# xinjuezou-whi/Open_Duck_Playground

Measured on AMD Instinct MI355X. Metric: env steps/sec (all envs) open_duck_mini_v2 flat, 4096 envs, 1/2/4/8 GPUs, higher is better.
Workload: dtype f32; 1 GPU; C2: flat_terrain, no imitation, 4096 envs per GPU, episode_length 1000 + auto-reset; envs_per_gpu=4096, total_envs=4096, substeps=10, parallelism=env-shard x1, step_kernel=throughput

## Files before the change

open_duck_playground_amd/csrc/duck_env_kernels.h:

```cpp
#pragma once
#include "duck_common.h"
#include "duck_physics.h"
#include "duck_team.h"

enum { SLOT_ACTION_DELAY = 0, SLOT_PUSH_THETA = 1, SLOT_PUSH_MAG = 2, SLOT_GYRO = 3, SLOT_ACCEL = 6,
       SLOT_GRAVITY = 9, SLOT_IMU_IDX = 12, SLOT_QPOS = 13, SLOT_QVEL = 29, SLOT_CMD = 45 };
enum { RSLOT_DXY = 0, RSLOT_YAW = 2, RSLOT_QSCALE = 3, RSLOT_QVEL = 19, RSLOT_CMD = 25, RSLOT_PUSH = 33,
       RSLOT_OBS = 64 };
#define KEY_TAG_ENV 0x5EEDu
#define KEY_TAG_DR 0xD0D0u
#define PI_F 3.14159265358979323846f

struct KArgs {
  int n;
  float* fs;
  int32_t* is;
  const float* dr;
  const float* action;
  float* obs;
  float* priv;
  float* reward;
  float* done;
  float* scratch;
  const uint8_t* mask;
  uint64_t seed;
  int64_t env_offset;
  const float* frames;
  const float* hfield;
  RefMeta ref;
  duck_env_config cfg;
  duck_layout lay;
  duck_dr_layout drl;
  unsigned* err;
};


DK int local_env(int& lane) {
  lane = threadIdx.x % TEAM;
  return threadIdx.x / TEAM;
}

template <class Md, int LAT = 0>
DK lds_float* env_slice(float* lds, int t) {
  return (lds_float*)(lds + t * TLay<Md, LAT>::STRIDE);
}

template <class Md>
DK void phys_step(lds_float* L, int lane, bool integrate, bool want_out, float* aux, int aux_stride, float* scratch,
                  int sstride, const float* hfield) {
  TPhys<Md>::step(L, lane, integrate, want_out, aux, aux_stride, scratch, sstride, hfield);
}

template <class Md>
__device__ __noinline__ void phys_step_dni(lds_float* L, int lane, bool integrate, bool want_out, float* aux,
                                           int aux_stride, float* scratch, int sstride, const float* hfield) {
  phys_step<Md>(L, lane, integrate, want_out, aux, aux_stride, scratch, sstride, hfield);
}

struct Col {
  float* p;
  int n;
  DK float& operator[](int k) const { return p[(size_t)k * n]; }
};
struct LCol {
  lds_float* p;
  DK lds_float& operator[](int k) const { return p[k]; }
};

DK int nearest(const float* g, int n, float v) {
  int best = 0;
  float bd = fabsf(g[0] - v);
  for (int i = 1; i < 16; i++) {
    if (i >= n) break;
    const float d = fabsf(g[i] - v);
    if (d < bd) { bd = d; best = i; }
  }
  return best;
}
DK void reference_motion(const KArgs& A, float dx, float dy, float dth, int i, float* out) {
  const RefMeta& R = A.ref;
  dx = fminf(fmaxf(dx, R.dx_range[0]), R.dx_range[1]);
  dy = fminf(fmaxf(dy, R.dy_range[0]), R.dy_range[1]);
  dth = fminf(fmaxf(dth, R.dtheta_range[0]), R.dtheta_range[1]);
  const int ix = nearest(R.dxs, R.n_dx, dx), iy = nearest(R.dys, R.n_dy, dy), it = nearest(R.dthetas, R.n_dtheta, dth);
  const int nb = R.nb;
  const int ph = ((i % nb) + nb) % nb;
  const float4* f = reinterpret_cast<const float4*>(
      A.frames + ((size_t)((ix * R.n_dy + iy) * R.n_dtheta + it) * nb + ph) * 40);
#pragma unroll
  for (int d = 0; d < 10; d++) {
    const float4 v = f[d];
    out[4 * d] = v.x; out[4 * d + 1] = v.y; out[4 * d + 2] = v.z; out[4 * d + 3] = v.w;
  }
}

DK float nan_to_num(float x) {
  if (isnan(x)) return 0.0f;
  if (isinf(x)) return x > 0 ? 3.4028234663852886e38f : -3.4028234663852886e38f;
  return x;
}

template <class RT>
DK void sample_command(const duck_env_config& c, const RT& r, int slot, float* cmd) {
  const float f = c.head_range_factor;
  cmd[0] = r.uniform(slot + 0, c.lin_vel_x[0], c.lin_vel_x[1]);
  cmd[1] = r.uniform(slot + 1, c.lin_vel_y[0], c.lin_vel_y[1]);
  cmd[2] = r.uniform(slot + 2, c.ang_vel_yaw[0], c.ang_vel_yaw[1]);
  cmd[3] = r.uniform(slot + 3, c.neck_pitch_range[0] * f, c.neck_pitch_range[1] * f);
  cmd[4] = r.uniform(slot + 4, c.head_pitch_range[0] * f, c.head_pitch_range[1] * f);
  cmd[5] = r.uniform(slot + 5, c.head_yaw_range[0] * f, c.head_yaw_range[1] * f);
  cmd[6] = r.uniform(slot + 6, c.head_roll_range[0] * f, c.head_roll_range[1] * f);
  if (r.u(slot + 7) < 0.1f)
    for (int k = 0; k < 7; k++) cmd[k] = 0.0f;
}

template <class Md>
DK void load_dyn(const KArgs& A, int e, lds_float* L) {
  using Ly = Lay<Md>;
  Phys<Md>::set_nominal(L);
  if (A.dr) {
    const duck_dr_layout& D = A.drl;
    const int n = A.n;
#pragma unroll
    for (int k = 0; k < 3; k++) L[Ly::DIPOS + k] = A.dr[(size_t)(D.base_ipos + k) * n + e];
#pragma unroll
    for (int b = 0; b < Md::NB; b++) L[Ly::DMASS + b] = A.dr[(size_t)(D.body_mass + b) * n + e];
#pragma unroll
    for (int a = 0; a < Md::NU; a++) {
      L[Ly::DFRIC + Md::actuator_dof[a]] = A.dr[(size_t)(D.frictionloss + a) * n + e];
      L[Ly::DARM + Md::actuator_dof[a]] = A.dr[(size_t)(D.armature + a) * n + e];
      L[Ly::DQ0 + Md::actuator_qadr[a]] = A.dr[(size_t)(D.qpos0 + a) * n + e];
      L[Ly::DKP + a] = A.dr[(size_t)(D.kp + a) * n + e];
    }
  }
}

template <class Md, int LAT = 0>
DK void load_dyn_team(const KArgs& A, int e, lds_float* L, int lane) {
  using Ly = Lay<Md>;
  using TP = TPhys<Md, LAT>;
  constexpr int NDYN = Md::NB + 3 + 2 * Md::NV + Md::NQ + Md::NU;
  static_assert(Ly::DKP + Md::NU - Ly::DMASS == NDYN, "contiguous per-env model block");
  for (int k = lane; k < NDYN; k += TEAM) L[Ly::DMASS + k] = TP::tf(Md::B_NOM + k);
  if (A.dr) {
    TSYNC();
    const duck_dr_layout& D = A.drl;
    const int n = A.n;
    if (lane < 3) L[Ly::DIPOS + lane] = A.dr[(size_t)(D.base_ipos + lane) * n + e];
    for (int b = lane; b < Md::NB; b += TEAM) L[Ly::DMASS + b] = A.dr[(size_t)(D.body_mass + b) * n + e];
    if (lane < Md::NU) {
      const int a = lane, o = Md::B_ACT + 12 * a, dof = TP::ti(o + 5), qadr = TP::ti(o + 4);
      L[Ly::DFRIC + dof] = A.dr[(size_t)(D.frictionloss + a) * n + e];
      L[Ly::DARM + dof] = A.dr[(size_t)(D.armature + a) * n + e];
      L[Ly::DQ0 + qadr] = A.dr[(size_t)(D.qpos0 + a) * n + e];
      L[Ly::DKP + a] = A.dr[(size_t)(D.kp + a) * n + e];
    }
  }
}

struct SObs {
  lds_float* row;
  DK void operator()(int k, float v) const { row[k] = v; }
};

template <class Md, class FA, class OS, class RT>
DK void write_obs_team(const KArgs& A, int lane, lds_float* L, const FA& F, const OS& out, const RT& r,
                       int slot_base, int imitation_i) {
  using Ly = Lay<Md>;
  const duck_env_config& c = A.cfg;
  const duck_layout& Lo = A.lay;
  constexpr int NU = Md::NU;
  static_assert(NU <= TEAM, "an actuator per lane");
  static_assert(priv_row_max(NU) <= Ly::HSZ + 4 * Ly::NROW, "privileged row must fit in the H/row storage (SObs)");
  const bool joystick = Lo.task == DUCK_TASK_JOYSTICK;
  const float nl = c.noise_level;
  const int OQ = 13, OV = OQ + NU, O1 = OV + NU, O2 = O1 + NU, O3 = O2 + NU, OM = O3 + NU;
  const int OC = joystick ? OM + NU : OM;
  const int P = OC + 2 + (joystick ? 2 : 0);
  const int PQ = P + 15, PV = PQ + NU, PZ = PV + NU, PA = PZ + 1, PC = PA + NU, PF = PC + 2, PT = PF + 6, PR = PT + 2;
  const int PI = PR + (Lo.imitation ? 40 : 0);
  if (lane < 3) {
    const int k = lane;
    const float gyro = L[Ly::SENS + c.sens_gyro + k], acc = L[Ly::SENS + c.sens_accelerometer + k];
    const float grav = -L[Ly::IMUR + k];
    const float ngrav = grav + (2.0f * r.u(slot_base + SLOT_GRAVITY + k) - 1.0f) * nl * c.noise_gravity;
    const float h0 = F[Lo.imu_history + k], h1 = F[Lo.imu_history + 3 + k];
    F[Lo.imu_history + 6 + k] = h1;
    F[Lo.imu_history + 3 + k] = h0;
    F[Lo.imu_history + k] = ngrav;
    out(k, gyro + (2.0f * r.u(slot_base + SLOT_GYRO + k) - 1.0f) * nl * c.noise_gyro);
    out(3 + k, acc + (2.0f * r.u(slot_base + SLOT_ACCEL + k) - 1.0f) * nl * c.noise_accelerometer);
    out(P + k, gyro);
    out(P + 3 + k, acc);
    out(P + 6 + k, grav);
    out(P + 9 + k, L[Ly::SENS + c.sens_local_linvel + k]);
    out(P + 12 + k, L[Ly::SENS + c.sens_global_angvel + k]);
    out(PF + k, L[Ly::SENS + c.sens_left_foot_linvel + k]);
    out(PF + 3 + k, L[Ly::SENS + c.sens_right_foot_linvel + k]);
  }
  if (lane < 7) out(6 + lane, F[Lo.command + lane]);
  if (lane < NU) {
    const int a = lane;
    float ja = L[Ly::QPOS + c.actuator_qposadr[a]];
    if (c.backlash_qposadr[a] >= 0) ja += L[Ly::QPOS + c.backlash_qposadr[a]];
    const float jv = L[Ly::QVEL + c.actuator_qveladr[a]];
    out(OQ + a, ja + (2.0f * r.u(slot_base + SLOT_QPOS + a) - 1.0f) * nl * c.qpos_noise_scale[a] - c.default_actuator[a]);
    out(OV + a, (jv + (2.0f * r.u(slot_base + SLOT_QVEL + a) - 1.0f) * nl * c.noise_joint_vel) * c.dof_vel_scale);
    out(O1 + a, F[Lo.last_act + a]);
    out(O2 + a, F[Lo.last_last_act + a]);
    out(O3 + a, F[Lo.last_last_last_act + a]);
    if (joystick) out(OM + a, F[Lo.motor_targets + a]);
    out(PQ + a, ja - c.default_actuator[a]);
    out(PV + a, jv);
    out(PA + a, L[Ly::AF + a]);
  }
  if (lane < 2) {
    const float con = L[Ly::OCON + lane];
    out(OC + lane, con);
    out(PC + lane, con);
    out(PT + lane, F[Lo.feet_air_time + lane]);
    if (joystick) {
      const float ph = F[Lo.imitation_phase + lane];
      out(OC + 2 + lane, ph);
      out(PI + 1 + lane, ph);
    }
  }
  if (lane == 0) {
    out(PZ, L[Ly::QPOS + 2]);
    if (joystick) out(PI, (float)imitation_i);
  }
  if (Lo.imitation)
    for (int k = lane; k < 40; k += TEAM) out(PR + k, F[Lo.ref_motion + k]);
}

template <class Md>
__global__ void __launch_bounds__(TPB) reset_kernel(KArgs A) {
  using Ly = Lay<Md>;
  {
    extern __shared__ float lds_t[];
    load_model_tables<Md>(lds_t);
  }
  int lane;
  const int t = local_env(lane);
  const int e = blockIdx.x * TEAM_WG + t;
  if (e >= A.n) return;
  if (A.mask && !A.mask[e]) return;
  extern __shared__ float lds[];
  lds_float* const L = env_slice<Md>(lds, t);
  const duck_env_config& c = A.cfg;
  const duck_layout& Lo = A.lay;
  constexpr int NQ = Md::NQ, NV = Md::NV, NU = Md::NU;
  const Col F{A.fs + e, A.n};
  auto iset = [&](int k, int32_t v) { A.is[(size_t)k * A.n + e] = v; };
  for (int k = 0; k < Lo.nfloat; k++) F[k] = 0.0f;
  for (int k = 0; k < Lo.nint; k++) iset(k, 0);
  Rng r;
  derive_key(A.seed, A.env_offset + e, KEY_TAG_ENV, r.k0, r.k1);
  r.ctr = 0;
  load_dyn<Md>(A, e, L);
  for (int i = 0; i < NQ; i++) L[Ly::QPOS + i] = c.init_qpos[i];
  for (int i = 0; i < NV; i++) { L[Ly::QVEL + i] = 0.0f; L[Ly::WARM + i] = 0.0f; }
  L[Ly::QPOS + 0] += r.uniform(RSLOT_DXY + 0, -0.05f, 0.05f);
  L[Ly::QPOS + 1] += r.uniform(RSLOT_DXY + 1, -0.05f, 0.05f);
  {
    const float yaw = r.uniform(RSLOT_YAW, -3.14f, 3.14f);
    float s, co;
    sincosf(0.5f * yaw, &s, &co);
    const float qy[4] = {co, 0.0f, 0.0f, s};
    float q[4] = {L[Ly::QPOS + 3], L[Ly::QPOS + 4], L[Ly::QPOS + 5], L[Ly::QPOS + 6]};
    qmul(q, q, qy);
    for (int k = 0; k < 4; k++) L[Ly::QPOS + 3 + k] = q[k];
  }
  for (int a = 0; a < NU; a++) L[Ly::QPOS + c.actuator_qposadr[a]] *= r.uniform(RSLOT_QSCALE + a, 0.5f, 1.5f);
  const float vr = Lo.task == DUCK_TASK_STANDING ? 0.5f : 0.05f;
  for (int k = 0; k < 6; k++) L[Ly::QVEL + k] = r.uniform(RSLOT_QVEL + k, -vr, vr);
  for (int a = 0; a < NU; a++) L[Ly::CTRL + a] = L[Ly::QPOS + c.actuator_qposadr[a]];
  phys_step<Md>(L, lane, false, true, nullptr, 0, A.scratch ? A.scratch + e : nullptr, A.n, A.hfield);
  float cmd[7];
  sample_command(c, r, RSLOT_CMD, cmd);
  const float push_interval = r.uniform(RSLOT_PUSH, c.push_interval_range[0], c.push_interval_range[1]);
  iset(Lo.push_interval, (int32_t)rintf(push_interval / c.ctrl_dt));
  iset(Lo.rng_key, (int32_t)r.k0);
  iset(Lo.rng_key + 1, (int32_t)r.k1);
  iset(Lo.rng_ctr, 1);
  for (int k = 0; k < 7; k++) F[Lo.command + k] = cmd[k];
  for (int a = 0; a < NU; a++) F[Lo.motor_targets + a] = Lo.task == DUCK_TASK_STANDING ? 0.0f : c.default_actuator[a];
  if (Lo.imitation) {
    float ref[40];
    reference_motion(A, cmd[0], cmd[1], cmd[2], 0, ref);
    for (int k = 0; k < 40; k++) F[Lo.ref_motion + k] = ref[k];
  }
  write_obs_team<Md>(A, lane, L, F, SObs{L + Ly::H}, r, RSLOT_OBS, 0);
  TSYNC();
  float* priv = A.priv + (size_t)e * Lo.priv_size;
  float* obs = A.obs + (size_t)e * Lo.obs_size;
  for (int k = lane; k < Lo.priv_size; k += TEAM) {
    const float v = L[Ly::H + k];
    priv[k] = v;
    F[Lo.first_priv + k] = v;
    if (k < Lo.obs_size) {
      obs[k] = v;
      F[Lo.first_obs + k] = v;
    }
  }
  for (int i = 0; i < NQ; i++) { F[Lo.qpos + i] = L[Ly::QPOS + i]; F[Lo.first_qpos + i] = L[Ly::QPOS + i]; }
  for (int i = 0; i < NV; i++) {
    F[Lo.qvel + i] = L[Ly::QVEL + i]; F[Lo.first_qvel + i] = L[Ly::QVEL + i];
    F[Lo.qacc_warmstart + i] = L[Ly::WARM + i]; F[Lo.first_qacc_warmstart + i] = L[Ly::WARM + i];
  }
  for (int a = 0; a < NU; a++) { F[Lo.ctrl + a] = L[Ly::CTRL + a]; F[Lo.first_ctrl + a] = L[Ly::CTRL + a]; }
}

struct StepPre {
  int32_t step, push_step, push_interval, ep_steps, imitation_i;
  uint32_t k0, k1, ctr;
  float act;
};
template <class Md>
DK StepPre step_prefetch(const KArgs& A, int e, int lane) {
  static_assert(Md::NU <= TEAM, "an actuator per lane");
  const duck_layout& Lo = A.lay;
  const int n = A.n, ec = e < n ? e : 0;
  auto ig = [&](int k) { return A.is[(size_t)k * n + ec]; };
  StepPre P;
  P.step = ig(Lo.step);
  P.push_step = ig(Lo.push_step);
  P.push_interval = ig(Lo.push_interval);
  P.ep_steps = ig(Lo.ep_steps);
  P.imitation_i = ig(Lo.imitation_i);
  P.k0 = (uint32_t)ig(Lo.rng_key);
  P.k1 = (uint32_t)ig(Lo.rng_key + 1);
  P.ctr = (uint32_t)ig(Lo.rng_ctr);
  P.act = A.action[(size_t)ec * Md::NU + (lane < Md::NU ? lane : 0)];
  return P;
}

template <class Md, class FA, class RT, int LAT = 0>
DK void step_env(const KArgs& A, int e, int lane, lds_float* L, const FA& F, const Col& G, const RT& r,
                 const StepPre& P) {
  using Ly = Lay<Md>;
  const duck_env_config& c = A.cfg;
  const duck_layout& Lo = A.lay;
  constexpr int NQ = Md::NQ, NV = Md::NV, NU = Md::NU;
  const int n = A.n;
  STAGE_T0();
  auto iset = [&](int k, int32_t v) { A.is[(size_t)k * n + e] = v; };
  const float dt = c.ctrl_dt;
  const int step_prev = P.step, push_step = P.push_step, push_interval = P.push_interval;
  int ep_steps = P.ep_steps;
  if (c.auto_reset && F[Lo.done] != 0.0f) ep_steps = 0;
  int imitation_i = P.imitation_i;
  if (Lo.imitation) {
    const int nb = A.ref.nb;
    imitation_i = (imitation_i + 1) % nb;
    const float ph = ((float)imitation_i / (float)nb) * 2.0f * PI_F;
    F[Lo.imitation_phase] = cosf(ph);
    F[Lo.imitation_phase + 1] = sinf(ph);
    float ref[40];
    reference_motion(A, F[Lo.command], F[Lo.command + 1], F[Lo.command + 2], imitation_i, ref);
    for (int k = 0; k < 40; k++) F[Lo.ref_motion + k] = ref[k];
  } else {
    imitation_i = 0;
  }
  const int didx = r.randint(SLOT_ACTION_DELAY, c.action_min_delay, c.action_max_delay);
  float arate = 0.0f;
  for (int a = lane; a < NU; a += TEAM) {
    const float act = P.act;
    const float h1 = F[Lo.action_history + a], h2 = F[Lo.action_history + NU + a];
    F[Lo.action_history + a] = act;
    F[Lo.action_history + NU + a] = h1;
    F[Lo.action_history + 2 * NU + a] = h2;
    const float ad = didx == 0 ? act : (didx == 1 ? h1 : h2);
    float mt = c.default_actuator[a] + ad * c.action_scale;
    if (c.use_motor_speed_limits) {
      const float prev = F[Lo.motor_targets + a], lim = c.max_motor_velocity * dt;
      mt = fminf(fmaxf(mt, prev - lim), prev + lim);
    }
    L[Ly::CTRL + a] = mt;
    const float la = F[Lo.last_act + a];
    arate += (act - la) * (act - la);
  }
  const float theta = r.uniform(SLOT_PUSH_THETA, 0.0f, 2.0f * PI_F);
  const float mag = r.uniform(SLOT_PUSH_MAG, c.push_magnitude_range[0], c.push_magnitude_range[1]);
  const float gate = (push_interval != 0 && (push_step + 1) % push_interval == 0) ? 1.0f : 0.0f;
  const float push[2] = {cosf(theta) * gate * (float)c.push_enable, sinf(theta) * gate * (float)c.push_enable};
  arate = tsum(arate);
  team_for<NQ>(lane, [&](int i) { L[Ly::QPOS + i] = F[Lo.qpos + i]; });
  team_for<NV>(lane, [&](int i) {
    L[Ly::QVEL + i] = F[Lo.qvel + i] + (i == 0 ? push[0] * mag : (i == 1 ? push[1] * mag : 0.0f));
    L[Ly::WARM + i] = F[Lo.qacc_warmstart + i];
  });
  load_dyn_team<Md, LAT>(A, e, L, lane);
  TSYNC();
  float* scr = A.scratch ? A.scratch + e : nullptr;
  STAGE_MARK(29);
  if constexpr (LAT) {
    using TPL = TPhys<Md, LAT>;
    (void)scr;
    LAT_T(43, 5);
    for (int s = 0; s < c.n_substeps; s++) {
// ... 59 lines not shown
  const float r_still = nan_to_num(pc + vc) * (cn < 0.01f ? 1.0f : 0.0f);
  float imit = 0.0f;
  if (Lo.imitation) {
    const int R0 = Lo.ref_motion;
    float lxy = 0.0f, axy = 0.0f;
    for (int k = 0; k < 2; k++) {
      const float dv = L[Ly::QVEL + k] - F[R0 + 34 + k], dw = L[Ly::QVEL + 3 + k] - F[R0 + 37 + k];
      lxy += dv * dv;
      axy += dw * dw;
    }
    const float dz = L[Ly::QVEL + 2] - F[R0 + 36], dwz = L[Ly::QVEL + 5] - F[R0 + 39];
    const float lin_xy = expf(-8.0f * lxy), lin_z = expf(-8.0f * dz * dz);
    const float ang_xy = expf(-2.0f * axy) * 0.5f, ang_z = expf(-2.0f * dwz * dwz) * 0.5f;
    float jp = 0.0f, jv = 0.0f;
    for (int k = lane; k < 5; k += TEAM) {
      const float q1 = L[Ly::QPOS + c.actuator_qposadr[k]] - F[R0 + k];
      const float q2 = L[Ly::QPOS + c.actuator_qposadr[NU - 5 + k]] - F[R0 + 11 + k];
      const float v1 = L[Ly::QVEL + c.actuator_qveladr[k]] - F[R0 + 16 + k];
      const float v2 = L[Ly::QVEL + c.actuator_qveladr[NU - 5 + k]] - F[R0 + 27 + k];
      jp += q1 * q1 + q2 * q2;
      jv += v1 * v1 + v2 * v2;
    }
    jp = tsum(jp);
    jv = tsum(jv);
    float contact_r = 0.0f;
    for (int k = 0; k < 2; k++) contact_r += (con[k] == (F[R0 + 32 + k] > 0.5f ? 1.0f : 0.0f)) ? 1.0f : 0.0f;
    float rr = lin_xy + lin_z + ang_xy + ang_z + (-jp * 15.0f) + (-jv * 1e-3f) + contact_r;
    rr *= cn > 0.01f ? 1.0f : 0.0f;
    imit = nan_to_num(rr);
  }
  float terms[7];
  if (standing) {
    lpc = tsum(lpc);
    lvc = tsum(lvc);
    hp = tsum(hp);
    const float ux = L[Ly::SENS + c.sens_upvector], uy = L[Ly::SENS + c.sens_upvector + 1];
    terms[0] = nan_to_num(ux * ux + uy * uy) * c.scale_orientation;
    terms[1] = nan_to_num(torq) * c.scale_torques;
    terms[2] = nan_to_num(arate) * c.scale_action_rate;
    terms[3] = 1.0f * c.scale_alive;
    terms[4] = nan_to_num(lpc + lvc) * (cn < 0.01f ? 1.0f : 0.0f) * c.scale_stand_still;
    terms[5] = nan_to_num(hp) * (cn > 0.01f ? 1.0f : 0.0f) * c.scale_head_pos;
    terms[6] = 0.0f;
  } else {
    terms[0] = r_lin * c.scale_tracking_lin_vel;
    terms[1] = r_ang * c.scale_tracking_ang_vel;
    terms[2] = nan_to_num(torq) * c.scale_torques;
    terms[3] = nan_to_num(arate) * c.scale_action_rate;
    terms[4] = 1.0f * c.scale_alive;
    terms[5] = imit * c.scale_imitation;
    terms[6] = r_still * c.scale_stand_still;
  }
  float sum = 0.0f;
  for (int k = 0; k < 7; k++) sum += terms[k];
  const float reward = fminf(fmaxf(sum * dt, 0.0f), 10000.0f);
  F[Lo.push] = push[0];
  F[Lo.push + 1] = push[1];
  int step = step_prev + 1;
  iset(Lo.push_step, push_step + 1);
  team_for<NU>(lane, [&](int a) {
    F[Lo.last_last_last_act + a] = F[Lo.last_last_act + a];
    F[Lo.last_last_act + a] = F[Lo.last_act + a];
    F[Lo.last_act + a] = F[Lo.action_history + a];
  });
  if (step > 500) {
    float nc[7];
    sample_command(c, r, SLOT_CMD, nc);
    for (int k = 0; k < 7; k++) F[Lo.command + k] = nc[k];
  }
  if (done != 0.0f || step > 500) step = 0;
  iset(Lo.step, step);
  iset(Lo.imitation_i, imitation_i);
  for (int k = 0; k < 2; k++) {
    F[Lo.feet_air_time + k] = F[Lo.feet_air_time + k] * (con[k] != 0.0f ? 0.0f : 1.0f);
    F[Lo.last_contact + k] = con[k];
    F[Lo.swing_peak + k] = F[Lo.swing_peak + k] * (con[k] != 0.0f ? 0.0f : 1.0f);
  }
  const float scales[7] = {standing ? c.scale_orientation : c.scale_tracking_lin_vel,
                           standing ? c.scale_torques : c.scale_tracking_ang_vel,
                           standing ? c.scale_action_rate : c.scale_torques,
                           standing ? c.scale_alive : c.scale_action_rate,
                           standing ? c.scale_stand_still : c.scale_alive,
                           standing ? c.scale_head_pos : c.scale_imitation,
                           standing ? 0.0f : c.scale_stand_still};
  for (int k = 0; k < 7; k++) F[Lo.metrics + k] = scales[k] > 0.0f ? terms[k] : -terms[k];
  F[Lo.metrics + DUCK_M_SWING_PEAK] = 0.5f * (F[Lo.swing_peak] + F[Lo.swing_peak + 1]);
  iset(Lo.rng_ctr, (int32_t)(r.ctr + 1));
  float trunc = 0.0f;
  bool restore = false;
  if (c.auto_reset) {
    ep_steps += 1;
    if (ep_steps >= c.episode_length) { trunc = 1.0f - done; done = 1.0f; }
    restore = done != 0.0f;
    iset(Lo.ep_steps, ep_steps);
  }
  if (restore) {
    for (int i = lane; i < NQ; i += TEAM) F[Lo.qpos + i] = G[Lo.first_qpos + i];
    for (int i = lane; i < NV; i += TEAM) { F[Lo.qvel + i] = G[Lo.first_qvel + i]; F[Lo.qacc_warmstart + i] = G[Lo.first_qacc_warmstart + i]; }
    for (int a = lane; a < NU; a += TEAM) F[Lo.ctrl + a] = G[Lo.first_ctrl + a];
    TSYNC();
    for (int k = lane; k < Lo.priv_size; k += TEAM) L[Ly::H + k] = G[Lo.first_priv + k];
  } else {
    team_for<NQ>(lane, [&](int i) { F[Lo.qpos + i] = L[Ly::QPOS + i]; });
    team_for<NV>(lane, [&](int i) { F[Lo.qvel + i] = L[Ly::QVEL + i]; F[Lo.qacc_warmstart + i] = L[Ly::WARM + i]; });
  }
  F[Lo.reward] = reward;
  F[Lo.done] = done;
  F[Lo.truncation] = trunc;
  A.reward[e] = reward;
  A.done[e] = done;
  STAGE_MARK(31);
  TSYNC();
  float* priv = A.priv + (size_t)e * Lo.priv_size;
  float* obs = A.obs + (size_t)e * Lo.obs_size;
  constexpr int PMAX = priv_row_max(NU);
  constexpr int NKP = (PMAX + TEAM - 1) / TEAM, NKO = (DUCK_OBS_SIZE(NU) + TEAM - 1) / TEAM;
  float pv[NKP];
#pragma unroll
  for (int kk = 0; kk < NKP; kk++) {
    const int k = lane + TEAM * kk;
    pv[kk] = L[Ly::H + (k < PMAX ? k : PMAX - 1)];
  }
#pragma unroll
  for (int kk = 0; kk < NKP; kk++) {
    const int k = lane + TEAM * kk;
    if (k < Lo.priv_size) priv[k] = pv[kk];
  }
#pragma unroll
  for (int kk = 0; kk < NKO; kk++) {
    const int k = lane + TEAM * kk;
    if (k < Lo.obs_size) obs[k] = pv[kk];
  }
  STAGE_MARK(34);
}

DK RngTab step_rng(const StepPre& P, lds_float* tab, int lane) {
  RngTab rt;
  rt.k0 = P.k0;
  rt.k1 = P.k1;
  rt.ctr = P.ctr;
  rt.tab = tab;
  rt.fill(tab, lane);
  return rt;
}

template <class Md>
__global__ void __launch_bounds__(TPB) step_kernel(KArgs A) {
  STAGE_T0();
#ifdef DUCK_ANY_PROF
  const unsigned long long kstart = clock64(), kwall = wall_clock64();
#endif
  using TL = TLay<Md>;
  {
    extern __shared__ float lds_t[];
    load_model_tables<Md>(lds_t);
  }
  STAGE_MARK(14);
  int lane;
  const int t = local_env(lane);
  const int e = blockIdx.x * TEAM_WG + t;
  const int n = A.n;
  extern __shared__ float lds[];
  if constexpr (TL::ES_LDS) {
    const int j = threadIdx.x % TEAM_WG, ej = blockIdx.x * TEAM_WG + j;
    lds_float* esj = (lds_float*)(lds + TL::ES + j * TL::ESTRIDE);
    const StepPre P = step_prefetch<Md>(A, e, lane);
    {
      constexpr int NK = (TL::HOT + TPB / TEAM_WG - 1) / (TPB / TEAM_WG);
      const int ejc = ej < n ? ej : 0;
      float hv[NK];
#pragma unroll
      for (int kk = 0; kk < NK; kk++) {
        const int k = (int)threadIdx.x / TEAM_WG + (TPB / TEAM_WG) * kk;
        hv[kk] = A.fs[(size_t)(k < TL::HOT ? k : TL::HOT - 1) * n + ejc];
      }
#pragma unroll
      for (int kk = 0; kk < NK; kk++) {
        const int k = (int)threadIdx.x / TEAM_WG + (TPB / TEAM_WG) * kk;
        if (ej < n && k < TL::HOT) esj[k] = hv[kk];
      }
    }
    __syncthreads();
    STAGE_MARK(32);
    if (e < n) {
      lds_float* const L = env_slice<Md>(lds, t);
      const Col G{A.fs + e, n};
      lds_float* esp = (lds_float*)(lds + TL::ES + t * TL::ESTRIDE);
      const RngTab rt = step_rng(P, esp + TL::HOT, lane);
      TSYNC();
      STAGE_MARK(33);
      step_env<Md>(A, e, lane, L, LCol{esp}, G, rt, P);
      STAGE_RESET();
    }
    __syncthreads();
    {
      constexpr int NK = (TL::HOT + TPB / TEAM_WG - 1) / (TPB / TEAM_WG);
      float hv[NK];
#pragma unroll
      for (int kk = 0; kk < NK; kk++) {
        const int k = (int)threadIdx.x / TEAM_WG + (TPB / TEAM_WG) * kk;
        hv[kk] = esj[k < TL::HOT ? k : TL::HOT - 1];
      }
#pragma unroll
      for (int kk = 0; kk < NK; kk++) {
        const int k = (int)threadIdx.x / TEAM_WG + (TPB / TEAM_WG) * kk;
        if (ej < n && k < TL::HOT) A.fs[(size_t)k * n + ej] = hv[kk];
      }
    }
  } else {
    if (e >= n) return;
    lds_float* const L = env_slice<Md>(lds, t);
    const Col G{A.fs + e, n};
    const duck_layout& Lo = A.lay;
    Rng r;
    r.k0 = (uint32_t)A.is[(size_t)Lo.rng_key * n + e];
    r.k1 = (uint32_t)A.is[(size_t)(Lo.rng_key + 1) * n + e];
    r.ctr = (uint32_t)A.is[(size_t)Lo.rng_ctr * n + e];
    step_env<Md>(A, e, lane, L, G, G, r, step_prefetch<Md>(A, e, lane));
    STAGE_RESET();
  }
  STAGE_MARK(15);
#ifdef DUCK_ANY_PROF
  if ((threadIdx.x & 63) == 0 && blockIdx.x < 256) {
    const int w = 4 * blockIdx.x + threadIdx.x / 64;
    g_stage_cycles[DUCK_NSTAGE + w] = clock64() - kstart;
    g_stage_cycles[DUCK_NSTAGE + 1024 + w] = kwall;
    g_stage_cycles[DUCK_NSTAGE + 2048 + w] = wall_clock64();
  }
#endif
}

template <class Md, int LAT>
__device__ __forceinline__ void step_lat_body(KArgs A) {
  using TL = TLay<Md, LAT>;
  using TPL = TPhys<Md, LAT>;
  constexpr int WGL = TL::NWG;
  static_assert(TL::TAB_LDS && TL::ES_LDS, "latency mode: the model blob and the hot state in LDS");
  static_assert(TPB == 4 * 64 && WGL * TEAM == 64 * (LAT == 2 ? 2 : 1),
                "latency modes: 4 waves, one set of 4 teams per wave (paired: per pair of waves)");
  extern __shared__ float lds[];
  LAT_T(40, 5);
  TPL::ev_init((int)threadIdx.x);
  load_model_tables<Md, LAT>(lds);
  LAT_T(41, 5);
  const int wave = __builtin_amdgcn_readfirstlane((int)threadIdx.x >> 6);
  const int t = (LAT == 2 ? 4 * (wave >> 1) : 0) + ((int)threadIdx.x & 63) / TEAM, lane = (int)threadIdx.x % TEAM;
  const int e = blockIdx.x * WGL + t;
  const int n = A.n;
  const int j = threadIdx.x % WGL, ej = blockIdx.x * WGL + j;
  lds_float* esj = (lds_float*)(lds + TL::ES + j * TL::ESTRIDE);
  const StepPre P = step_prefetch<Md>(A, e, lane);
  constexpr int NK = (TL::HOT + TPB / WGL - 1) / (TPB / WGL);
  {
    const int ejc = ej < n ? ej : 0;
    float hv[NK];
#pragma unroll
    for (int kk = 0; kk < NK; kk++) {
      const int k = (int)threadIdx.x / WGL + (TPB / WGL) * kk;
      hv[kk] = A.fs[(size_t)(k < TL::HOT ? k : TL::HOT - 1) * n + ejc];
    }
#pragma unroll
    for (int kk = 0; kk < NK; kk++) {
      const int k = (int)threadIdx.x / WGL + (TPB / WGL) * kk;
      if (ej < n && k < TL::HOT) esj[k] = hv[kk];
    }
  }
  __syncthreads();
  LAT_T(42, 5);
  if (e < n) {
    lds_float* const L = env_slice<Md, LAT>(lds, t);
    const int ns = A.cfg.n_substeps;
    float* scr = A.scratch ? A.scratch + e : nullptr;
    auto env_code = [&]() {
      const Col G{A.fs + e, n};
      lds_float* esp = (lds_float*)(lds + TL::ES + t * TL::ESTRIDE);
      const RngTab rt = step_rng(P, esp + TL::HOT, lane);
      TSYNC();
      step_env<Md, LCol, RngTab, LAT>(A, e, lane, L, LCol{esp}, G, rt, P);
      LAT_T(45, 5);
    };
    if constexpr (LAT == 2) {
      if ((wave & 1) == 0) {
        env_code();
      } else {
        for (int s = 0; s < ns; s++) TPL::lat2_b(L, lane, s, true, s == ns - 1, scr, n);
      }
    } else {
      if (wave == 0) {
        env_code();
      } else if (wave == 1) {
        for (int s = 0; s < ns; s++) TPL::lat_r1(L, lane, s, true, s == ns - 1, scr, n);
      } else if (wave == 2) {
        for (int s = 0; s < ns; s++) TPL::lat_r2(L, lane, s, A.hfield);
      } else {
        for (int s = 0; s < ns; s++) TPL::lat_r3(L, lane, s);
      }
    }
  }
  __syncthreads();
  LAT_T(46, 5);
  const bool timed_out = TPL::ev_timed_out(LAT == 2 ? j / LAT_WG : 0);
  if (threadIdx.x == 0 && A.err && (TPL::ev_timed_out(0) || (LAT == 2 && TPL::ev_timed_out(1))))
    __hip_atomic_fetch_or(A.err, (unsigned)DUCK_DEVERR_LAT_TIMEOUT, __ATOMIC_RELAXED, __HIP_MEMORY_SCOPE_SYSTEM);
  {
    float hv[NK];
#pragma unroll
    for (int kk = 0; kk < NK; kk++) {
      const int k = (int)threadIdx.x / WGL + (TPB / WGL) * kk;
      hv[kk] = esj[k < TL::HOT ? k : TL::HOT - 1];
      if (timed_out && k >= A.lay.qpos && k < A.lay.qpos + Md::NQ) hv[kk] = __builtin_nanf("");
    }
#pragma unroll
    for (int kk = 0; kk < NK; kk++) {
      const int k = (int)threadIdx.x / WGL + (TPB / WGL) * kk;
      if (ej < n && k < TL::HOT) A.fs[(size_t)k * n + ej] = hv[kk];
    }
  }
}

template <class Md, int LAT>
__global__ void __launch_bounds__(TPB) step_kernel_lat(KArgs A) {
  step_lat_body<Md, LAT>(A);
}

constexpr int LAT_X2 = 5;
template <class Md>
struct LatX2 {
  static_assert(TLay<Md, LAT_X2>::LDS_FLOATS == TLay<Md, 1>::LDS_FLOATS && TLay<Md, LAT_X2>::NWG == LAT_WG,
                "LAT_X2 is the LAT = 1 layout");
  static constexpr bool PAYS = TLay<Md, 1>::FITS && 2 * (size_t)TLay<Md, 1>::LDS_FLOATS * 4 <= 160 * 1024 &&
                               Md::FLOOR_TYPE == 0 && Md::NV <= 20;
};
template <class Md>
__global__ void __launch_bounds__(TPB) __attribute__((amdgpu_waves_per_eu(2, 2))) step_kernel_lat_x2(KArgs A) {
  if constexpr (LatX2<Md>::PAYS) step_lat_body<Md, LAT_X2>(A);
}

template <class Md>
__global__ void __launch_bounds__(TPB) physics_kernel(KArgs A, float* qpos_g, float* qvel_g, float* warm_g,
                                                     const float* ctrl_g, int nsub, float* aux) {
  using Ly = Lay<Md>;
  {
    extern __shared__ float lds_t[];
    load_model_tables<Md>(lds_t);
  }
  int lane;
  const int t = local_env(lane);
  const int e = blockIdx.x * TEAM_WG + t;
  const int n = A.n;
  if (e >= n) return;
  extern __shared__ float lds[];
  lds_float* const L = env_slice<Md>(lds, t);
  for (int i = 0; i < Md::NQ; i++) L[Ly::QPOS + i] = qpos_g[(size_t)i * n + e];
  for (int i = 0; i < Md::NV; i++) { L[Ly::QVEL + i] = qvel_g[(size_t)i * n + e]; L[Ly::WARM + i] = warm_g[(size_t)i * n + e]; }
  for (int a = 0; a < Md::NU; a++) L[Ly::CTRL + a] = ctrl_g[(size_t)a * n + e];
  load_dyn<Md>(A, e, L);
  float* ax = aux ? aux + e : nullptr;
  float* scr = A.scratch ? A.scratch + e : nullptr;
  const int ns = nsub > 0 ? nsub : 1;
  for (int s = 0; s < ns; s++) phys_step_dni<Md>(L, lane, nsub > 0, s == ns - 1, ax, n, scr, n, A.hfield);
  for (int i = 0; i < Md::NQ; i++) qpos_g[(size_t)i * n + e] = L[Ly::QPOS + i];
  for (int i = 0; i < Md::NV; i++) { qvel_g[(size_t)i * n + e] = L[Ly::QVEL + i]; warm_g[(size_t)i * n + e] = L[Ly::WARM + i]; }
}

template <class Md>
__global__ void randomize_kernel(int n, float* dr, duck_dr_layout D, uint64_t seed, int64_t env_offset) {
  const int e = blockIdx.x * blockDim.x + threadIdx.x;
  if (e >= n) return;
  Rng r;
  derive_key(seed, env_offset + e, KEY_TAG_DR, r.k0, r.k1);
  r.ctr = 0;
  int slot = 0;
  auto W = [&](int k, float v) { dr[(size_t)k * n + e] = v; };
  W(D.floor_friction, r.uniform(slot++, 0.5f, 1.0f));
  float fl[Md::NU], arm[Md::NU], ip[3], ms[Md::NB], q0[Md::NU], kp[Md::NU];
  for (int a = 0; a < Md::NU; a++) fl[a] = r.uniform(slot++, 0.9f, 1.1f);
  for (int a = 0; a < Md::NU; a++) arm[a] = r.uniform(slot++, 1.0f, 1.05f);
  for (int k = 0; k < 3; k++) ip[k] = r.uniform(slot++, -0.05f, 0.05f);
  for (int b = 0; b < Md::NB; b++) ms[b] = r.uniform(slot++, 0.9f, 1.1f);
  const float dmass = r.uniform(slot++, -0.1f, 0.1f);
  for (int a = 0; a < Md::NU; a++) q0[a] = r.uniform(slot++, -0.03f, 0.03f);
  for (int a = 0; a < Md::NU; a++) kp[a] = r.uniform(slot++, 0.9f, 1.1f);
  for (int a = 0; a < Md::NU; a++) {
    W(D.frictionloss + a, fl[a] * Md::dof_frictionloss[Md::actuator_dof[a]]);
    W(D.armature + a, arm[a] * Md::dof_armature[Md::actuator_dof[a]]);
    W(D.qpos0 + a, q0[a] + Md::qpos0[Md::actuator_qadr[a]]);
    W(D.kp + a, kp[a] * Md::actuator_kp[a]);
  }
  for (int k = 0; k < 3; k++) W(D.base_ipos + k, ip[k] + Md::body_ipos[1][k]);
  for (int b = 0; b < Md::NB; b++) W(D.body_mass + b, ms[b] * Md::body_mass[b] + (b == 1 ? dmass : 0.0f));
}

template <class Md>
static bool matches(const duck_model_desc* m) {
  return duck_model_fingerprint(m) == Md::FINGERPRINT;
}

template <class Md>
static size_t lds_bytes() {
  return (size_t)TLay<Md>::LDS_FLOATS * sizeof(float);
}
template <class Md>
static size_t lds_bytes_lat() {
  return TLay<Md, 1>::FITS ? (size_t)TLay<Md, 1>::LDS_FLOATS * sizeof(float) : 0;
}
template <class Md>
static size_t lds_bytes_lat2() {
  return TLay<Md, 2>::FITS ? (size_t)TLay<Md, 2>::LDS_FLOATS * sizeof(float) : 0;
}
template <class Md>
static size_t lds_bytes_lat_x2() {
  return LatX2<Md>::PAYS ? (size_t)TLay<Md, 1>::LDS_FLOATS * sizeof(float) : 0;
}

template <class Md>
static int aux_size_of() {
  return aux_size<Md>();
}

static KArgs make_args(duck_sim* s, int n) {
  KArgs A;
  memset(&A, 0, sizeof(A));
  A.n = n;
  A.cfg = s->cfg;
  A.lay = s->lay;
  A.drl = s->drl;
  A.ref = s->ref;
  A.frames = s->frames_d;
  A.hfield = s->hfield_d;
  A.err = s->err_d;
  return A;
}

template <class Md>
static int launch_reset(duck_sim* s, int n, float* fs, int32_t* is, const uint8_t* mask, uint64_t seed,
                        int64_t env_offset, const float* dr, float* obs, float* priv, hipStream_t st) {
  KArgs A = make_args(s, n);
  A.fs = fs; A.is = is; A.mask = mask; A.seed = seed; A.env_offset = env_offset; A.dr = dr;
  A.obs = obs; A.priv = priv;
  const dim3 grid((A.n + TEAM_WG - 1) / TEAM_WG), block(TPB);
  hipLaunchKernelGGL((reset_kernel<Md>), grid, block, lds_bytes<Md>(), st, A);
  HIPCHECK(hipGetLastError());
  return DUCK_OK;
}

template <class Md>
static int launch_step(duck_sim* s, int n, float* fs, int32_t* is, const float* dr, const float* action, float* obs,
                       float* priv, float* reward, float* done, float* scratch, hipStream_t st) {
  KArgs A = make_args(s, n);
  A.fs = fs; A.is = is; A.dr = dr; A.action = action; A.obs = obs; A.priv = priv;
  A.reward = reward; A.done = done; A.scratch = scratch;
  if (s->lay.first_qpos != TLay<Md>::HOT) return duck_fail(DUCK_EINVAL, "state layout does not match the kernel's hot-state size");
  static_assert(LAT_WG == LAT_WG_HOST, "latency workgroup size");
  const int k = step_kernel_choice(s, n);
  if (k == DUCK_STEP_LATENCY || k == DUCK_STEP_PAIRED || k == DUCK_STEP_LATENCY_X2) {
    const int wgl = k == DUCK_STEP_PAIRED ? 2 * LAT_WG : LAT_WG;
    const dim3 grid((A.n + wgl - 1) / wgl), block(TPB);
    if (k == DUCK_STEP_LATENCY_X2) {
      if constexpr (LatX2<Md>::PAYS)
        hipLaunchKernelGGL((step_kernel_lat_x2<Md>), grid, block, lds_bytes_lat_x2<Md>(), st, A);
      else
        return duck_fail(DUCK_EUNSUPPORTED, "the two-workgroups-per-CU latency kernel is not compiled for this model");
    } else if (k == DUCK_STEP_PAIRED) {
      if constexpr (TLay<Md, 2>::FITS)
        hipLaunchKernelGGL((step_kernel_lat<Md, 2>), grid, block, lds_bytes_lat2<Md>(), st, A);
      else
        return duck_fail(DUCK_EUNSUPPORTED, "the paired latency kernel does not fit this model in LDS");
    } else {
      if constexpr (TLay<Md, 1>::FITS)
        hipLaunchKernelGGL((step_kernel_lat<Md, 1>), grid, block, lds_bytes_lat<Md>(), st, A);
      else
        return duck_fail(DUCK_EUNSUPPORTED, "the latency kernel does not fit this model in LDS");
    }
    HIPCHECK(hipGetLastError());
    return DUCK_OK;
  }
  const dim3 grid((A.n + TEAM_WG - 1) / TEAM_WG), block(TPB);
  hipLaunchKernelGGL((step_kernel<Md>), grid, block, lds_bytes<Md>(), st, A);
  HIPCHECK(hipGetLastError());
  return DUCK_OK;
}

template <class Md>
static int launch_randomize(duck_sim* s, int n, float* dr, uint64_t seed, int64_t env_offset, hipStream_t st) {
  const dim3 grid((n + 255) / 256), block(256);
  hipLaunchKernelGGL((randomize_kernel<Md>), grid, block, 0, st, n, dr, s->drl, seed, env_offset);
  HIPCHECK(hipGetLastError());
  return DUCK_OK;
}

template <class Md>
static int launch_physics(duck_sim* s, int n, float* qpos, float* qvel, float* warm, const float* ctrl, const float* dr,
                          int nsub, float* aux, float* scratch, hipStream_t st) {
  const dim3 grid((n + TEAM_WG - 1) / TEAM_WG), block(TPB);
  KArgs A = make_args(s, n);
  A.dr = dr;
  A.scratch = scratch;
  hipLaunchKernelGGL((physics_kernel<Md>), grid, block, lds_bytes<Md>(), st, A, qpos, qvel, warm, ctrl, nsub, aux);
  HIPCHECK(hipGetLastError());
  return DUCK_OK;
}

static int lat_timeouts_of(unsigned* out, int reset) {
  hipError_t e = hipMemcpyFromSymbol(out, HIP_SYMBOL(g_lat_timeouts), sizeof(unsigned));
  if (e == hipSuccess && reset) {
    const unsigned z = 0;
    e = hipMemcpyToSymbol(HIP_SYMBOL(g_lat_timeouts), &z, sizeof(unsigned));
  }
  return e == hipSuccess ? DUCK_OK : duck_fail(DUCK_EHIP, hipGetErrorString(e));
}

static int stage_cycles_of(unsigned long long* out, int reset) {
#ifdef DUCK_ANY_PROF
  hipError_t e = hipMemcpyFromSymbol(out, HIP_SYMBOL(g_stage_cycles), sizeof(unsigned long long) * (DUCK_NSTAGE + 3 * 1024));
  static unsigned long long wg[DUCK_NSTAGE * 256];
  if (e == hipSuccess) e = hipMemcpyFromSymbol(wg, HIP_SYMBOL(g_stage_wg), sizeof(wg));
  for (int k = 0; k < DUCK_NSTAGE && e == hipSuccess; k++)
    for (int b = 0; b < 256; b++) out[k] += wg[k * 256 + b];
  if (e == hipSuccess && reset) {
    static unsigned long long z[DUCK_NSTAGE * 256 > DUCK_NSTAGE + 3 * 1024 ? DUCK_NSTAGE * 256 : DUCK_NSTAGE + 3 * 1024] = {0};
    e = hipMemcpyToSymbol(HIP_SYMBOL(g_stage_cycles), z, sizeof(unsigned long long) * (DUCK_NSTAGE + 3 * 1024));
    if (e == hipSuccess) e = hipMemcpyToSymbol(HIP_SYMBOL(g_stage_wg), z, sizeof(wg));
  }
  return e == hipSuccess ? 0 : DUCK_EHIP;
#else
  (void)out;
  (void)reset;
  return DUCK_EUNSUPPORTED;
#endif
}

#define DUCK_DEFINE_VARIANT(NAME, MODEL)                                                        \
  const VariantOps* duck_variant_##NAME() {                                                     \
    static const VariantOps ops = {#NAME,               matches<MODEL>,         aux_size_of<MODEL>, \
                                   lds_bytes<MODEL>,    MODEL::FLOOR_TYPE,      launch_reset<MODEL>, \
                                   launch_step<MODEL>,  launch_randomize<MODEL>, launch_physics<MODEL>, \
                                   stage_cycles_of,     lat_timeouts_of,        lds_bytes_lat<MODEL>, \
                                   lds_bytes_lat2<MODEL>, lds_bytes_lat_x2<MODEL>};                     \
    return &ops;                                                                                \
  }
```

open_duck_playground_amd/csrc/duck_physics.h:

```cpp
#pragma once
#include "../../include/duck_env.h"
#include "duck_math.h"

#define DNI __device__ __noinline__
#define SCHED_FENCE() asm volatile("" ::: "memory")

typedef __attribute__((address_space(3))) float lds_float;

#if defined(DUCK_STAGE_PROF) || defined(DUCK_WAVE_PROF) || defined(DUCK_LAT_PROF)
#define DUCK_ANY_PROF 1
#endif
#ifdef DUCK_ANY_PROF
#define DUCK_NSTAGE 60
static __device__ unsigned long long g_stage_cycles[DUCK_NSTAGE + 3 * 1024];
static __device__ unsigned long long g_stage_wg[DUCK_NSTAGE * 256];
#define STAGE_ADD(k, v) atomicAdd(&g_stage_wg[(k) * 256 + (blockIdx.x & 255)], (v))
#endif
#ifdef DUCK_STAGE_PROF
#define STAGE_T0() unsigned long long _t0 = wall_clock64(), _c0 = clock64()
#define STAGE_RESET() (_c0 = clock64())
#define STAGE_MARK(k)                                                             \
  do {                                                                            \
    asm volatile("s_waitcnt lgkmcnt(0)" ::: "memory");                            \
    const unsigned long long _c1 = clock64();                                     \
    if (threadIdx.x == 0) STAGE_ADD(k, _c1 - _c0);                                \
    _c0 = _c1;                                                                    \
    (void)_t0;                                                                    \
  } while (0)
#elif defined(DUCK_LAT_PROF)
#define STAGE_T0() unsigned long long _c0 = clock64()
#define STAGE_RESET() (_c0 = clock64())
#define STAGE_MARK(k)                                                                  \
  do {                                                                                 \
    asm volatile("s_waitcnt lgkmcnt(0)" ::: "memory");                                 \
    const unsigned long long _c1 = clock64();                                          \
    if (blockIdx.x == 0 && ((int)threadIdx.x & 63) == 0) g_stage_cycles[DUCK_NSTAGE + 64 + (k)] += _c1 - _c0; \
    _c0 = _c1;                                                                         \
  } while (0)
#elif defined(DUCK_ASM_MARKS)
#define STAGE_T0() \
  do {             \
  } while (0)
#define STAGE_MARK(k) asm volatile("; STAGE_MARK " #k ::: "memory")
#define STAGE_RESET() \
  do {                \
  } while (0)
#else
#define STAGE_T0() \
  do {             \
  } while (0)
#define STAGE_MARK(k) \
  do {                \
  } while (0)
#define STAGE_RESET() \
  do {                \
  } while (0)
#endif

constexpr int priv_row_max(int nu) { return DUCK_OBS_SIZE(nu) + 15 + 3 * nu + 1 + 2 + 6 + 2 + 40 + 1 + 2; }

template <class Md>
struct Lay {
  static constexpr int NB = Md::NB, NV = Md::NV, NQ = Md::NQ, NU = Md::NU;
  static constexpr int NCON = 4 * Md::NPAIR;
  static constexpr int R_LIM = Md::NFRIC, R_CON = Md::NFRIC + Md::NLIM;
  static constexpr int NROW = R_CON + 4 * NCON;
  static constexpr int QPOS = 0, QVEL = QPOS + NQ, WARM = QVEL + NV, CTRL = WARM + NV, QACC = CTRL + NU;
  static constexpr int QSM = QACC + NV, FSM = QSM + NV, SRCH = FSM + NV, GRAD = SRCH + NV, MA = GRAD + NV;
  static constexpr int DMASS = MA + NV, DIPOS = DMASS + NB, DARM = DIPOS + 3, DFRIC = DARM + NV;
  static constexpr int DQ0 = DFRIC + NV, DKP = DQ0 + NQ;
  static constexpr int XPOS = DKP + NU, XQ = XPOS + 3 * NB, XMAT = XQ + 4 * NB, CIN = XMAT + 9 * NB;
  static constexpr int CVEL = CIN + 10 * NB, COM = CVEL + 6 * NB;
  static constexpr int CDOF = COM + 3, CDD1 = CDOF + 6 * NV;
  static constexpr int M = CDD1 + 18, MZERO = M + Md::NM, H = MZERO + 1;
  static constexpr int SCR_TREE = 12 * NB + 6 * NV, SCR_SAT = 6 * (Md::NHE + Md::NHF);
  static constexpr int SCR_HF = Md::FLOOR_TYPE == 1 ? 3 + 28 * 16 : 0, SCR_OBS = priv_row_max(NU);
  static constexpr int cmax(int a, int b) { return a > b ? a : b; }
  static constexpr int SCR_NEED = cmax(cmax(SCR_TREE, SCR_SAT), cmax(SCR_HF, SCR_OBS));
  static constexpr int HSZ = ((cmax(SCR_NEED - 4 * NROW - Md::NLIM, 0) + 3) / 4) * 4;
  static constexpr int JA = H + HSZ, JV = JA + NROW, RD = JV + NROW, AREF = RD + NROW;
  static constexpr int LSGN = AREF + NROW;
  static constexpr int CR = LSGN + Md::NLIM, CFR = CR + 3 * NCON, CDIST = CFR + 9 * NCON;
  static constexpr int KL = CIN, KR = KL + 21, KLR = KR + 21, FL = KLR + 36, FR = FL + 6;
  static_assert(FR + 6 <= CIN + 10 * NB, "Newton blocks must fit in CIN");
  static constexpr int AF = CDIST + NCON, SENS = AF + NU, OCON = SENS + Md::NSENSORDATA, IMUR = OCON + 2,
                       FOOTZ = IMUR + 3, FLAGS = FOOTZ + 2;
  static constexpr int TOTAL = FLAGS + 2;
};

DK void kbi(const float* solref, const float* solimp, float pos, float dt, float& k, float& b, float& imp) {
  const float timeconst = fmaxf(solref[0], 2.0f * dt);
  const float dampratio = solref[1];
  const float dmin = fminf(fmaxf(solimp[0], 0.0001f), 0.9999f), dmax = fminf(fmaxf(solimp[1], 0.0001f), 0.9999f);
  const float width = fmaxf(1e-15f, solimp[2]), mid = fminf(fmaxf(solimp[3], 0.0001f), 0.9999f);
  const float power = fmaxf(1.0f, solimp[4]);
  k = 1.0f / (dmax * dmax * timeconst * timeconst * dampratio * dampratio);
  b = 2.0f / (dmax * timeconst);
  const float x = fabsf(pos) / width;
  float y;
  if (power == 2.0f) {
    const float ya = (1.0f / mid) * x * x;
    const float yb = 1.0f - (1.0f / (1.0f - mid)) * (1.0f - x) * (1.0f - x);
    y = x < mid ? ya : yb;
  } else {
    const float ya = (1.0f / powf(mid, power - 1.0f)) * powf(x, power);
    const float yb = 1.0f - (1.0f / powf(1.0f - mid, power - 1.0f)) * powf(1.0f - x, power);
    y = x < mid ? ya : yb;
  }
  float im = dmin + y * (dmax - dmin);
  im = fminf(fmaxf(im, dmin), dmax);
  imp = x > 1.0f ? dmax : im;
}

template <int N>
DK int argmax_tol(const float* v, float tol) {
  float mx = v[0];
#pragma unroll
  for (int i = 1; i < N; i++) mx = fmaxf(mx, v[i]);
  int r = N - 1;
#pragma unroll
  for (int i = N - 1; i >= 0; i--) r = (v[i] >= mx - tol) ? i : r;
  return r;
}
#define MANIFOLD_TOL 2e-8f

template <int N>
DK void pick3(const float (*P)[3], int k, float* out) {
  out[0] = P[0][0]; out[1] = P[0][1]; out[2] = P[0][2];
#pragma unroll
  for (int i = 1; i < N; i++) {
    const bool s = (i == k);
    out[0] = s ? P[i][0] : out[0];
    out[1] = s ? P[i][1] : out[1];
    out[2] = s ? P[i][2] : out[2];
  }
}
template <int N>
DK float pick1(const float* P, int k) {
  float o = P[0];
#pragma unroll
  for (int i = 1; i < N; i++) o = (i == k) ? P[i] : o;
  return o;
}

template <int N>
DK void manifold_points(const float (*poly)[3], const bool* mask, const float* nrm, int idx[4]) {
  float dm[N], s[N], s2[2 * N];
#pragma unroll
  for (int k = 0; k < N; k++) dm[k] = mask[k] ? 0.0f : -1e6f;
  const int a = argmax_tol<N>(dm, 0.0f);
  float pa[3];
  pick3<N>(poly, a, pa);
#pragma unroll
  for (int k = 0; k < N; k++) {
    const float dx = pa[0] - poly[k][0], dy = pa[1] - poly[k][1], dz = pa[2] - poly[k][2];
    s[k] = dx * dx + dy * dy + dz * dz + dm[k];
  }
  const int b = argmax_tol<N>(s, MANIFOLD_TOL);
  float pb[3];
  pick3<N>(poly, b, pb);
  float amb[3] = {pa[0] - pb[0], pa[1] - pb[1], pa[2] - pb[2]}, ab[3];
  cross3(ab, nrm, amb);
#pragma unroll
  for (int k = 0; k < N; k++) {
    const float ap[3] = {pa[0] - poly[k][0], pa[1] - poly[k][1], pa[2] - poly[k][2]};
    s[k] = fabsf(dot3(ap, ab)) + dm[k];
  }
  const int c = argmax_tol<N>(s, MANIFOLD_TOL);
  float pc[3];
  pick3<N>(poly, c, pc);
  float amc[3] = {pa[0] - pc[0], pa[1] - pc[1], pa[2] - pc[2]};
  float bmc[3] = {pb[0] - pc[0], pb[1] - pc[1], pb[2] - pc[2]};
  float ac[3], bc[3];
  cross3(ac, nrm, amc);
  cross3(bc, nrm, bmc);
#pragma unroll
  for (int k = 0; k < N; k++) {
    const float bp[3] = {pb[0] - poly[k][0], pb[1] - poly[k][1], pb[2] - poly[k][2]};
    const float ap[3] = {pa[0] - poly[k][0], pa[1] - poly[k][1], pa[2] - poly[k][2]};
    s2[k] = fabsf(dot3(bp, bc)) + dm[k];
    s2[N + k] = fabsf(dot3(ap, ac)) + dm[k];
  }
  int d = argmax_tol<2 * N>(s2, MANIFOLD_TOL);
  d = d >= N ? d - N : d;
  idx[0] = a; idx[1] = b; idx[2] = c; idx[3] = d;
}

DK void make_frame(float* fr, const float* nin) {
  float n[3] = {nin[0], nin[1], nin[2]};
  const float nn = sqrtf(dot3(n, n));
  if (nn > 1e-15f) { n[0] /= nn; n[1] /= nn; n[2] /= nn; }
  float b[3];
  const bool y = (-0.5f < n[1]) && (n[1] < 0.5f);
  b[0] = 0.0f; b[1] = y ? 1.0f : 0.0f; b[2] = y ? 0.0f : 1.0f;
  const float nb = dot3(n, b);
  b[0] -= n[0] * nb; b[1] -= n[1] * nb; b[2] -= n[2] * nb;
  const float bn = sqrtf(dot3(b, b));
  if (bn > 1e-15f) { b[0] /= bn; b[1] /= bn; b[2] /= bn; }
  float c[3];
  cross3(c, n, b);
  fr[0] = n[0]; fr[1] = n[1]; fr[2] = n[2];
  fr[3] = b[0]; fr[4] = b[1]; fr[5] = b[2];
  fr[6] = c[0]; fr[7] = c[1]; fr[8] = c[2];
}

template <class Md>
DK constexpr int cgeom_slot(int g) {
  return g == Md::FLOOR_GEOM ? 0 : (g == Md::LFOOT_GEOM ? 1 : 2);
}

template <class Md>
struct Phys {
  using Ly = Lay<Md>;
  static constexpr int NV = Md::NV, NB = Md::NB, NQ = Md::NQ, NU = Md::NU;
  static constexpr int NCON = Ly::NCON;

  static DK void set_nominal(lds_float* L) {
#pragma unroll
    for (int b = 0; b < NB; b++) L[Ly::DMASS + b] = Md::body_mass[b];
#pragma unroll
    for (int k = 0; k < 3; k++) L[Ly::DIPOS + k] = Md::body_ipos[1][k];
#pragma unroll
    for (int i = 0; i < NV; i++) { L[Ly::DARM + i] = Md::dof_armature[i]; L[Ly::DFRIC + i] = Md::dof_frictionloss[i]; }
#pragma unroll
    for (int i = 0; i < NQ; i++) L[Ly::DQ0 + i] = Md::qpos0[i];
#pragma unroll
    for (int a = 0; a < NU; a++) L[Ly::DKP + a] = Md::actuator_kp[a];
  }

  static DK void geom_frame(lds_float* L, int g, float* gp, float* gR) {
    const int b = Md::cgeom_body[g];
    if (Md::body_weldid[b] == 0) {
      float bq[4] = {Md::body_quat[b][0], Md::body_quat[b][1], Md::body_quat[b][2], Md::body_quat[b][3]}, BR[9], t[3];
      q2m(BR, bq);
      mulmv3(t, BR, Md::geom_pos[g]);
#pragma unroll
      for (int k = 0; k < 3; k++) gp[k] = Md::body_pos[b][k] + t[k];
      mulmm3(gR, BR, Md::geom_mat[g]);
    } else {
      float R[9], t[3];
#pragma unroll
      for (int k = 0; k < 9; k++) R[k] = L[Ly::XMAT + 9 * b + k];
      mulmv3(t, R, Md::geom_pos[g]);
#pragma unroll
      for (int k = 0; k < 3; k++) gp[k] = L[Ly::XPOS + 3 * b + k] + t[k];
      mulmm3(gR, R, Md::geom_mat[g]);
    }
  }

  static DK void store_contact(lds_float* L, int slot, float dist, const float* pos, const float* fr) {
    L[Ly::CDIST + slot] = dist;
#pragma unroll
    for (int a = 0; a < 3; a++) L[Ly::CR + 3 * slot + a] = pos[a] - L[Ly::COM + a];
#pragma unroll
    for (int a = 0; a < 9; a++) L[Ly::CFR + 9 * slot + a] = fr[a];
  }

  static DK void contact_vel(const float* Sp, const float* r, float* v) {
    float t[3];
    cross3(t, Sp, r);
    v[0] = Sp[3] + t[0]; v[1] = Sp[4] + t[1]; v[2] = Sp[5] + t[2];
  }

  static DNI void write_aux(lds_float* L, float* aux, int stride) {
    int o = 0;
    for (int i = 0; i < NV; i++) aux[(o++) * stride] = L[Ly::QACC + i];
    for (int i = 0; i < NV; i++) aux[(o++) * stride] = L[Ly::QSM + i];
    for (int i = 0; i < NV; i++) aux[(o++) * stride] = L[Ly::QVEL + i];
    for (int i = 0; i < NV; i++) aux[(o++) * stride] = L[Ly::FSM + i];
    for (int a = 0; a < NU; a++) aux[(o++) * stride] = L[Ly::AF + a];
    for (int k = 0; k < Md::NSENSORDATA; k++) aux[(o++) * stride] = L[Ly::SENS + k];
    for (int s = 0; s < NCON; s++) aux[(o++) * stride] = L[Ly::CDIST + s];
    for (int s = 0; s < NCON; s++)
      for (int a = 0; a < 3; a++) aux[(o++) * stride] = L[Ly::CR + 3 * s + a] + L[Ly::COM + a];
    for (int s = 0; s < NCON; s++)
      for (int a = 0; a < 3; a++) aux[(o++) * stride] = L[Ly::CFR + 9 * s + a];
    for (int k = 0; k < Md::NM; k++) aux[(o++) * stride] = L[Ly::M + k];
#ifdef DUCK_AUX_LDS
    for (int k = 0; k < Ly::TOTAL + 12 * Md::MAXCHAIN + 24; k++) aux[(o++) * stride] = L[k];
#endif
  }
};

template <class Md>
constexpr int aux_size() {
  return 4 * Md::NV + Md::NU + Md::NSENSORDATA + 7 * Lay<Md>::NCON + Md::NM
#ifdef DUCK_AUX_LDS
         + Lay<Md>::TOTAL + 12 * Md::MAXCHAIN + 24
#endif
      ;
}
```

open_duck_playground_amd/csrc/duck_team.h:

```cpp
#pragma once
#include <utility>

#include "duck_physics.h"

constexpr int TEAM = 16;
constexpr int TEAM_WG = 16;
constexpr int TPB = TEAM * TEAM_WG;
typedef __attribute__((address_space(3))) int lds_int;
typedef float f4v __attribute__((ext_vector_type(4)));
typedef __attribute__((address_space(3))) f4v lds_f4;

DK float frcp(float x) { return __builtin_amdgcn_rcpf(x); }
DK float vsel(unsigned long long m, float t, float f) {
  float r;
  asm("v_cndmask_b32_e64 %0, %1, %2, %3" : "=v"(r) : "v"(f), "v"(t), "s"(m));
  return r;
}

DK float imp_of(const float* solimp, float pos) {
  const float dmin = fminf(fmaxf(solimp[0], 0.0001f), 0.9999f), dmax = fminf(fmaxf(solimp[1], 0.0001f), 0.9999f);
  const float width = fmaxf(1e-15f, solimp[2]), mid = fminf(fmaxf(solimp[3], 0.0001f), 0.9999f);
  const float power = fmaxf(1.0f, solimp[4]);
  const float x = fabsf(pos) * frcp(width);
  float y;
// ... 45 lines not shown
  for (int s = 0; s < (N - B0 + TEAM - 1) / TEAM; s++) {
    const int i = B0 + lane + TEAM * s;
    if (B0 + TEAM * (s + 1) <= N || i < N) f(i);
  }
}
DK float tmaxf(float v) {
  v = fmaxf(v, dppf<0xB1>(v));
  v = fmaxf(v, dppf<0x4E>(v));
  v = fmaxf(v, dppf<0x141>(v));
  v = fmaxf(v, dppf<0x140>(v));
  return v;
}
DK int tmini(int v) {
  v = min(v, dppi<0xB1>(v));
  v = min(v, dppi<0x4E>(v));
  v = min(v, dppi<0x141>(v));
  v = min(v, dppi<0x140>(v));
  return v;
}
DK float hsum8(float v) {
  v += dppf<0xB1>(v);
  v += dppf<0x4E>(v);
  v += dppf<0x141>(v);
  return v;
}
DK float hmax8(float v) {
  v = fmaxf(v, dppf<0xB1>(v));
  v = fmaxf(v, dppf<0x4E>(v));
  v = fmaxf(v, dppf<0x141>(v));
  return v;
}
DK float hmax8_nc(float v) {
  v = fmax_nc(v, dppf<0xB1>(v));
  v = fmax_nc(v, dppf<0x4E>(v));
  v = fmax_nc(v, dppf<0x141>(v));
  return v;
}
DK int hmin8i(int v) {
  v = min(v, dppi<0xB1>(v));
  v = min(v, dppi<0x4E>(v));
  v = min(v, dppi<0x141>(v));
  return v;
}

template <int B, int E, class F>
DK void static_for(F&& f) {
  if constexpr (B < E) {
    f(std::integral_constant<int, B>{});
    static_for<B + 1, E>(f);
  }
}
constexpr int fbits(float v) { return __builtin_bit_cast(int, v); }
template <int C0, int C1, int C2>
DK float cdot(const float* x) {
  float r;
  asm("v_mul_f32_e32 %0, %1, %2" : "=v"(r) : "i"(C0), "v"(x[0]));
  asm("v_fmac_f32_e32 %0, %1, %2" : "+v"(r) : "i"(C1), "v"(x[1]));
  asm("v_fmac_f32_e32 %0, %1, %2" : "+v"(r) : "i"(C2), "v"(x[2]));
  return r;
}
template <int C0, int C1, int C2, int OFF>
DK void cdot3v_off(const float* x, const float* y, const float* z, float* r) {
  asm("v_mul_f32_e32 %0, %3, %7\n\tv_mul_f32_e32 %1, %3, %10\n\tv_mul_f32_e32 %2, %3, %13\n\t"
      "v_fmac_f32_e32 %0, %4, %8\n\tv_fmac_f32_e32 %1, %4, %11\n\tv_fmac_f32_e32 %2, %4, %14\n\t"
      "v_fmac_f32_e32 %0, %5, %9\n\tv_fmac_f32_e32 %1, %5, %12\n\tv_fmac_f32_e32 %2, %5, %15\n\t"
      "v_sub_f32_e32 %0, %6, %0\n\tv_sub_f32_e32 %1, %6, %1\n\tv_sub_f32_e32 %2, %6, %2"
      : "=&v"(r[0]), "=&v"(r[1]), "=&v"(r[2])
      : "i"(C0), "i"(C1), "i"(C2), "i"(OFF), "v"(x[0]), "v"(x[1]), "v"(x[2]), "v"(y[0]), "v"(y[1]), "v"(y[2]),
        "v"(z[0]), "v"(z[1]), "v"(z[2]));
}
template <int C0, int C1, int C2>
DK void cdot4v(const float* x, const float* y, const float* z, const float* u, float* r) {
  asm("v_mul_f32_e32 %0, %4, %7\n\tv_mul_f32_e32 %1, %4, %10\n\tv_mul_f32_e32 %2, %4, %13\n\t"
      "v_mul_f32_e32 %3, %4, %16\n\t"
      "v_fmac_f32_e32 %0, %5, %8\n\tv_fmac_f32_e32 %1, %5, %11\n\tv_fmac_f32_e32 %2, %5, %14\n\t"
      "v_fmac_f32_e32 %3, %5, %17\n\t"
      "v_fmac_f32_e32 %0, %6, %9\n\tv_fmac_f32_e32 %1, %6, %12\n\tv_fmac_f32_e32 %2, %6, %15\n\t"
      "v_fmac_f32_e32 %3, %6, %18"
      : "=&v"(r[0]), "=&v"(r[1]), "=&v"(r[2]), "=&v"(r[3])
      : "i"(C0), "i"(C1), "i"(C2), "v"(x[0]), "v"(x[1]), "v"(x[2]), "v"(y[0]), "v"(y[1]), "v"(y[2]),
        "v"(z[0]), "v"(z[1]), "v"(z[2]), "v"(u[0]), "v"(u[1]), "v"(u[2]));
}
template <int C0, int C1, int C2>
DK void cdot5v(const float* x, const float* y, const float* z, const float* u, const float* w, float* r) {
  asm("v_mul_f32_e32 %0, %5, %8\n\tv_mul_f32_e32 %1, %5, %11\n\tv_mul_f32_e32 %2, %5, %14\n\t"
      "v_mul_f32_e32 %3, %5, %17\n\tv_mul_f32_e32 %4, %5, %20\n\t"
      "v_fmac_f32_e32 %0, %6, %9\n\tv_fmac_f32_e32 %1, %6, %12\n\tv_fmac_f32_e32 %2, %6, %15\n\t"
      "v_fmac_f32_e32 %3, %6, %18\n\tv_fmac_f32_e32 %4, %6, %21\n\t"
      "v_fmac_f32_e32 %0, %7, %10\n\tv_fmac_f32_e32 %1, %7, %13\n\tv_fmac_f32_e32 %2, %7, %16\n\t"
      "v_fmac_f32_e32 %3, %7, %19\n\tv_fmac_f32_e32 %4, %7, %22"
      : "=&v"(r[0]), "=&v"(r[1]), "=&v"(r[2]), "=&v"(r[3]), "=&v"(r[4])
      : "i"(C0), "i"(C1), "i"(C2), "v"(x[0]), "v"(x[1]), "v"(x[2]), "v"(y[0]), "v"(y[1]), "v"(y[2]),
        "v"(z[0]), "v"(z[1]), "v"(z[2]), "v"(u[0]), "v"(u[1]), "v"(u[2]), "v"(w[0]), "v"(w[1]), "v"(w[2]));
}
template <int C0, int C1, int C2>
DK void cdot5v_noff(const float* x, const float* y, const float* z, const float* u, const float* w, const float* o,
                    float* r) {
  asm("v_fmamk_f32 %0, %8, %5, %23\n\tv_fmamk_f32 %1, %11, %5, %24\n\tv_fmamk_f32 %2, %14, %5, %25\n\t"
      "v_fmamk_f32 %3, %17, %5, %26\n\tv_fmamk_f32 %4, %20, %5, %27\n\t"
      "v_fmac_f32_e32 %0, %6, %9\n\tv_fmac_f32_e32 %1, %6, %12\n\tv_fmac_f32_e32 %2, %6, %15\n\t"
      "v_fmac_f32_e32 %3, %6, %18\n\tv_fmac_f32_e32 %4, %6, %21\n\t"
      "v_fmac_f32_e32 %0, %7, %10\n\tv_fmac_f32_e32 %1, %7, %13\n\tv_fmac_f32_e32 %2, %7, %16\n\t"
      "v_fmac_f32_e32 %3, %7, %19\n\tv_fmac_f32_e32 %4, %7, %22"
      : "=&v"(r[0]), "=&v"(r[1]), "=&v"(r[2]), "=&v"(r[3]), "=&v"(r[4])
      : "i"(C0 ^ (int)0x80000000), "i"(C1 ^ (int)0x80000000), "i"(C2 ^ (int)0x80000000), "v"(x[0]), "v"(x[1]),
        "v"(x[2]), "v"(y[0]), "v"(y[1]), "v"(y[2]), "v"(z[0]), "v"(z[1]), "v"(z[2]), "v"(u[0]), "v"(u[1]), "v"(u[2]),
        "v"(w[0]), "v"(w[1]), "v"(w[2]), "v"(o[0]), "v"(o[1]), "v"(o[2]), "v"(o[3]), "v"(o[4]));
}
template <int A0, int A1, int A2, int B0, int B1, int B2>
DK void cdot2c(const float* x, float& ra, float& rb) {
  asm("v_mul_f32_e32 %0, %2, %8\n\tv_mul_f32_e32 %1, %5, %8\n\t"
      "v_fmac_f32_e32 %0, %3, %9\n\tv_fmac_f32_e32 %1, %6, %9\n\t"
      "v_fmac_f32_e32 %0, %4, %10\n\tv_fmac_f32_e32 %1, %7, %10"
      : "=&v"(ra), "=&v"(rb)
      : "i"(A0), "i"(A1), "i"(A2), "i"(B0), "i"(B1), "i"(B2), "v"(x[0]), "v"(x[1]), "v"(x[2]));
}
template <int C>
DK float cfma(float x, float a) {
  asm("v_fmac_f32_e32 %0, %1, %2" : "+v"(a) : "i"(C), "v"(x));
  return a;
}

constexpr float HF_WITNESS_BAND = 1e-3f;
constexpr float HF_DEPTH_TIE = 1e-6f;

#ifndef DUCK_LS_DFLOOR
#define DUCK_LS_DFLOOR 1e-6f
#endif

constexpr int LAT_WG = 4;
static __device__ unsigned int g_lat_timeouts;
#ifdef DUCK_LAT_PROF
#define LAT_T(k, s)                                                                                         \
  do {                                                                                                      \
    if (blockIdx.x == 0 && ((int)threadIdx.x & 63) == 0 && (s) == 5) g_stage_cycles[DUCK_NSTAGE + (k)] = clock64(); \
  } while (0)
#define LAT2_T(k, s)               \
  do {                             \
    if (threadIdx.x < 128) LAT_T(k, s); \
  } while (0)
#else
#define LAT_T(k, s) \
  do {              \
  } while (0)
#define LAT2_T(k, s) \
  do {               \
  } while (0)
#endif

template <class Md, int LAT = 0>
struct TLay {
  using Ly = Lay<Md>;
  static constexpr int KC = Ly::TOTAL;
#ifdef DUCK_LS_DUMP
  static constexpr int USED0 = KC + 136;
#else
  static constexpr int USED0 = KC + 2 * TEAM;
#endif
  static constexpr int HF_SLF = (1 + Md::HF_SILCAP + 3) & ~3;
  static constexpr int HF_SLSZ = HF_SLF + 4 * Md::HF_SILCAP;
  static constexpr int XRNE = LAT ? ((USED0 + 3) & ~3) : Ly::H;
  static constexpr int RCA = XRNE, CFRC = XRNE + 6 * Md::NB, RFB = XRNE + 12 * Md::NB;
  static constexpr int XCIN = LAT ? XRNE + 18 * Md::NB : Ly::CIN;
  static constexpr int XDUM0 = LAT ? XCIN + 10 * Md::NB : 0, XDUM1 = LAT ? XDUM0 + 10 * Md::NB : 0;
  static constexpr int XSIL = LAT ? ((XDUM1 + 6 * Md::NB + 3) & ~3) : ((Ly::CIN + 3) & ~3);
  static constexpr int XDIR = LAT ? ((XSIL + (Md::FLOOR_TYPE == 1 ? 2 * HF_SLSZ : 0) + 3) & ~3) : 0;
  static constexpr int USED = LAT ? XDIR + Md::NV + 4 : USED0;
  static constexpr int STRIDE = ((USED + 15) / 32) * 32 + 16;
  static constexpr int NWG = LAT == 2 ? 2 * LAT_WG : (LAT ? LAT_WG : TEAM_WG);
  static_assert(STRIDE >= USED && STRIDE % 32 == 16, "stride");
  static constexpr int SINK = KC;
  static constexpr int TMP = Ly::H;
  static constexpr int KLOC = TMP;
  static_assert(7 * Md::NB <= Ly::HSZ + 4 * Ly::NROW, "tree scratch must fit in H + rows");
  static constexpr int TAB = STRIDE * NWG;
  static constexpr int HOT = Md::NQ + 2 * Md::NV + 8 * Md::NU + 77;
  static constexpr int ESTRIDE = (HOT + 64) | 1;
  static constexpr int ES_FLOATS = ESTRIDE * NWG;
  static constexpr int NEV_G = LAT ? 10 : 0;
  static constexpr int NEV = LAT == 2 ? 2 * NEV_G : NEV_G;
  static constexpr size_t LDS_MAX = 160 * 1024 / 4 - 4 * NEV;
  static constexpr bool TAB_LDS = (size_t)(TAB + Md::NBLOB) <= LDS_MAX;
  static constexpr int NHT = Md::B_HEND > Md::B_HFACE ? Md::B_HEND - Md::B_HFACE : 0;
  static constexpr bool HT_LDS = !TAB_LDS && NHT > 0 && (size_t)(TAB + NHT) <= LDS_MAX;
  static constexpr int ES = TAB + (TAB_LDS ? Md::NBLOB : (HT_LDS ? NHT : 0));
  static constexpr bool ES_LDS = (size_t)(ES + ES_FLOATS) <= LDS_MAX;
  static constexpr int EV = ES + (ES_LDS ? ES_FLOATS : 0);
  static constexpr int LDS_FLOATS = EV + 4 * NEV;
  static constexpr bool FITS = (size_t)LDS_FLOATS * 4 <= 160 * 1024 && (LAT == 0 || (TAB_LDS && ES_LDS));
  static_assert(LAT || FITS, "LDS budget");
  static_assert(6 * Md::NV <= 4 * Ly::NROW, "crb scratch must fit in the row storage");
  static_assert(LAT || 18 * Md::NB <= Ly::HSZ + 4 * Ly::NROW, "rne scratch must fit in H + rows");
  static_assert(LAT || Md::FLOOR_TYPE != 1 || XSIL + 2 * HF_SLSZ <= Ly::CIN + 10 * Md::NB,
                "the silhouette lists must fit in the composite inertias' storage");
};

template <class Md, int LAT = 0>
DK void load_model_tables(float* lds) {
  using TLy = TLay<Md, LAT>;
  if constexpr (TLy::TAB_LDS) {
    int* dst = (int*)(lds + TLy::TAB);
    constexpr int NK = (Md::NBLOB + TPB - 1) / TPB;
    int w[NK];
#pragma unroll
    for (int kk = 0; kk < NK; kk++) {
      const int i = (int)threadIdx.x + TPB * kk;
      w[kk] = Md::t_blob()[i < Md::NBLOB ? i : Md::NBLOB - 1];
    }
#pragma unroll
    for (int kk = 0; kk < NK; kk++) {
      const int i = (int)threadIdx.x + TPB * kk;
      if (i < Md::NBLOB) dst[i] = w[kk];
    }
    __syncthreads();
  } else if constexpr (TLy::HT_LDS) {
    int* dst = (int*)(lds + TLy::TAB);
    constexpr int N = TLy::NHT, NK = (N + TPB - 1) / TPB;
    int w[NK];
#pragma unroll
    for (int kk = 0; kk < NK; kk++) {
      const int i = (int)threadIdx.x + TPB * kk;
      w[kk] = Md::t_blob()[Md::B_HFACE + (i < N ? i : N - 1)];
    }
#pragma unroll
    for (int kk = 0; kk < NK; kk++) {
      const int i = (int)threadIdx.x + TPB * kk;
      if (i < N) dst[i] = w[kk];
    }
    __syncthreads();
  }
}

template <class Md>
struct HullFaceOrder {
  int f[Md::NHF];
  constexpr HullFaceOrder() : f{} {
    bool used[Md::NHF] = {};
    int n = 0;
    for (int c = 0; c < 6 && c < Md::NHF; c++) {
      const int ax = c < 2 ? 2 : (c < 4 ? 0 : 1);
      const float sg = (c == 0 || c == 3 || c == 5) ? -1.0f : 1.0f;
      int best = -1;
      for (int i = 0; i < Md::NHF; i++)
        if (!used[i] && (best < 0 || sg * Md::hull_face_normal[i][ax] > sg * Md::hull_face_normal[best][ax])) best = i;
      used[best] = true;
      f[n++] = best;
    }
    for (int i = 0; i < Md::NHF; i++)
      if (!used[i]) f[n++] = i;
  }
};

template <class Md, int LAT = 0>
struct TPhys {
  using Ly = Lay<Md>;
  using TL = TLay<Md, LAT>;
  using Ph = Phys<Md>;
  typedef lds_float* LP;
  static constexpr int NV = Md::NV, NB = Md::NB, NQ = Md::NQ, NU = Md::NU, NJ = Md::NJ;
  static constexpr int NCON = Ly::NCON, NFRIC = Md::NFRIC, NLIM = Md::NLIM, NROW = Ly::NROW;
  static constexpr int R_LIM = Ly::R_LIM, R_CON = Ly::R_CON;
  static DK int ti(int off) {
    if constexpr (TL::TAB_LDS) {
      extern __shared__ float lds_dyn[];
      return ((lds_int*)(lds_dyn + TL::TAB))[off];
    } else {
      return Md::t_blob()[off];
    }
  }
  static DK float tf(int off) { return __int_as_float(ti(off)); }
  static DK float th(int off) {
    if constexpr (!TL::TAB_LDS && TL::HT_LDS) {
      extern __shared__ float lds_dyn[];
      return ((lds_float*)(lds_dyn + TL::TAB))[off - Md::B_HFACE];
    } else {
      return tf(off);
    }
  }
  static DK f4v ht4(int off) {
    extern __shared__ __attribute__((aligned(16))) float lds_dyn[];
    static_assert(Md::FLOOR_TYPE != 1 || TL::TAB_LDS || TL::HT_LDS, "the hull SAT tables must be in LDS");
    return *(const lds_f4*)((lds_float*)lds_dyn + TL::TAB + (TL::TAB_LDS ? off : off - Md::B_HFACE));
  }
  static constexpr int LIMW = 13, PAIRW = 13;
  static DK int fric_dof(int r) {
    if constexpr (Md::B_FRIC0 >= 0) return Md::B_FRIC0 + r;
    else return ti(Md::B_FRIC + 3 * r);
  }
  static DK int lim_dof(int r) {
    if constexpr (Md::B_LIM0 >= 0) return Md::B_LIM0 + r;
    else return ti(Md::B_LIM + LIMW * r);
  }
  static DK int dof_fric(int c) {
    if constexpr (Md::B_FRIC0 >= 0) return (c >= Md::B_FRIC0 && c < Md::B_FRIC0 + NFRIC) ? c - Md::B_FRIC0 : -1;
    else return ti(Md::B_DOF2FRIC + c);
  }
  static DK int dof_lim(int c) {
    if constexpr (Md::B_LIM0 >= 0) return (c >= Md::B_LIM0 && c < Md::B_LIM0 + NLIM) ? c - Md::B_LIM0 : -1;
    else return ti(Md::B_DOF2LIM + c);
  }
  static DK int madr(int i, int j) { return ti(Md::B_MADR + NV * i + j); }
  static constexpr bool FREE0 = Md::jnt_type[0] == 0 && Md::body_dofadr[1] == 0 && Md::body_dofnum[1] == 6;
  static constexpr unsigned long long moving_mask() {
    unsigned long long msk = 0;
    for (int b = 0; b < Md::NB; b++)
      if (Md::body_weldid[b] != 0) msk |= 1ull << b;
    return msk;
  }
  static DK bool moving(int b) { return (moving_mask() >> b) & 1ull; }
  static DK int limb_body(int lane, int d) { return ti(Md::B_BR + Md::T_BRLEN * (lane < Md::T_NBR ? lane : 0) + d); }
  static DK int limb_dof(int lane, int k) { return ti(Md::B_BRDOF + 2 * Md::T_BRLEN * (lane < Md::T_NBR ? lane : 0) + k); }
  static DK int dof_body(int i) {
    if constexpr (Md::B_DBD > -1000) return i < Md::B_DBN ? Md::B_DB0 : i + Md::B_DBD;
    else return ti(Md::B_DOFREC + 4 * i);
  }
  static DK int act_dof(int a) {
    if constexpr (Md::B_ACTD0 >= 0) return Md::B_ACTD0 + a;
    else return ti(Md::B_ACT + 12 * a + 5);
  }
  static DK int act_qadr(int a) {
    if constexpr (Md::B_ACTQ0 >= 0) return Md::B_ACTQ0 + a;
    else return ti(Md::B_ACT + 12 * a + 4);
  }
  static DK int lim_qadr(int r) {
    if constexpr (Md::B_LIMQ0 >= 0) return Md::B_LIMQ0 + r;
    else return ti(Md::B_LIM + LIMW * r + 1);
  }

  static_assert(NFRIC <= TEAM, "one friction row per lane");
  static_assert(NCON <= TEAM, "one contact slot per lane");
  static_assert(NU <= TEAM, "one actuator per lane");

  static DK void body_pose(LP L, int b, const float* pp, const float* pR, const float* pq, float* p, float* q,
                           float* R) {
    const float bq[4] = {Md::body_quat[b][0], Md::body_quat[b][1], Md::body_quat[b][2], Md::body_quat[b][3]};
    const float bp[3] = {Md::body_pos[b][0], Md::body_pos[b][1], Md::body_pos[b][2]};
    float t[3];
    mulmv3(t, pR, bp);
    for (int k = 0; k < 3; k++) p[k] = pp[k] + t[k];
    qmul(q, pq, bq);
    const int nj = Md::body_jntnum[b], j0 = Md::body_jntadr[b];
#pragma unroll
    for (int jj = 0; jj < 2; jj++) {
      if (jj < nj) {
        const int j = j0 + jj, a = Md::jnt_qposadr[j];
        float sn, cs;
        sincosf(0.5f * (L[Ly::QPOS + a] - L[Ly::DQ0 + a]), &sn, &cs);
        const float ql[4] = {cs, Md::jnt_axis[j][0] * sn, Md::jnt_axis[j][1] * sn, Md::jnt_axis[j][2] * sn};
        qmul(q, q, ql);
      }
    }
    qnormalize(q);
    q2m(R, q);
  }
  static DK void store_pose(LP L, int b, const float* p, const float* q, const float* R) {
    for (int k = 0; k < 3; k++) L[Ly::XPOS + 3 * b + k] = p[k];
    for (int k = 0; k < 4; k++) L[Ly::XQ + 4 * b + k] = q[k];
    for (int k = 0; k < 9; k++) L[Ly::XMAT + 9 * b + k] = R[k];
  }

  static DK void kinematics(LP L, int lane) {
#pragma clang fp reassociate(on)
    STAGE_T0();
    team_for<NB, 2>(lane, [&](int b) {
      if (!moving(b)) return;
      const int o = Md::B_BKIN + 17 * b;
      float q[4] = {tf(o), tf(o + 1), tf(o + 2), tf(o + 3)};
      const int nj = ti(o + 7);
#pragma unroll
      for (int jj = 0; jj < 2; jj++) {
        if (jj < nj) {
          const int oj = o + 8 + 4 * jj, a = ti(oj);
          float sn, cs;
          __sincosf(0.5f * (L[Ly::QPOS + a] - L[Ly::DQ0 + a]), &sn, &cs);
          const float ql[4] = {cs, tf(oj + 1) * sn, tf(oj + 2) * sn, tf(oj + 3) * sn};
          qmul(q, q, ql);
        }
      }
      for (int k = 0; k < 4; k++) L[TL::KLOC + 7 * b + k] = q[k];
      for (int k = 0; k < 3; k++) L[TL::KLOC + 7 * b + 4 + k] = tf(o + 4 + k);
    });
    TSYNC();
    STAGE_MARK(24);
    float p[3], q[4], R[9];
    for (int k = 0; k < 3; k++) p[k] = L[Ly::QPOS + k];
    for (int k = 0; k < 4; k++) q[k] = L[Ly::QPOS + 3 + k];
    qnormalize(q);
    q2m(R, q);
    if (lane == 0) store_pose(L, 1, p, q, R);
    auto compose = [&](int b) {
      float ql[4], pl[3], t[3], qn[4];
      for (int k = 0; k < 4; k++) ql[k] = L[TL::KLOC + 7 * b + k];
      for (int k = 0; k < 3; k++) pl[k] = L[TL::KLOC + 7 * b + 4 + k];
      mulmv3(t, R, pl);
      for (int k = 0; k < 3; k++) p[k] += t[k];
      qmul(qn, q, ql);
      qnormalize(qn);
      for (int k = 0; k < 4; k++) q[k] = qn[k];
      q2m(R, q);
    };
#pragma unroll
    for (int r = 1; r < Md::T_NROOT; r++) {
      compose(Md::T_ROOT[r]);
      if (lane == 0) store_pose(L, Md::T_ROOT[r], p, q, R);
    }
    if (lane < Md::T_NBR) {
      constexpr int BL = Md::T_BRLEN;
      int bb[BL];
      float kl[BL][7];
#pragma unroll
      for (int d = 0; d < BL; d++) bb[d] = limb_body(lane, d);
#pragma unroll
      for (int d = 0; d < BL; d++) {
        const int bc = bb[d] >= 0 ? bb[d] : 1;
        for (int k = 0; k < 7; k++) kl[d][k] = L[TL::KLOC + 7 * bc + k];
      }
#pragma unroll
      for (int d = 0; d < BL; d++) {
        if (bb[d] < 0) break;
        float t[3], qn[4];
        mulmv3(t, R, &kl[d][4]);
        for (int k = 0; k < 3; k++) p[k] += t[k];
        qmul(qn, q, kl[d]);
        qnormalize(qn);
        for (int k = 0; k < 4; k++) q[k] = qn[k];
        q2m(R, q);
        store_pose(L, bb[d], p, q, R);
      }
    }
    TSYNC();
  }

  static DK void com_pos(LP L, int lane) {
#pragma clang fp reassociate(on)
    static_assert((moving_mask() >> (1 + TEAM)) == 0, "a moving body per lane");
    float xi[3] = {0, 0, 0}, rot[9] = {0, 0, 0, 0, 0, 0, 0, 0, 0}, m = 0.0f;
    const int b = 1 + lane;
    const bool mv = b < NB && moving(b);
    if (mv) {
      const int ob = Md::B_BINERT + 17 * b;
      float R[9], t[3], ip[3], Ri[9], Bi[9];
      for (int k = 0; k < 9; k++) R[k] = L[Ly::XMAT + 9 * b + k];
      for (int k = 0; k < 3; k++) ip[k] = (b == 1) ? L[Ly::DIPOS + k] : tf(ob + k);
      for (int k = 0; k < 9; k++) Bi[k] = tf(ob + 3 + k);
      mulmv3(t, R, ip);
      mulmm3(Ri, R, Bi);
      const float I[3] = {tf(ob + 12), tf(ob + 13), tf(ob + 14)};
      for (int a = 0; a < 3; a++)
        for (int c = 0; c < 3; c++)
          rot[3 * a + c] = Ri[3 * a] * I[0] * Ri[3 * c] + Ri[3 * a + 1] * I[1] * Ri[3 * c + 1] + Ri[3 * a + 2] * I[2] * Ri[3 * c + 2];
      for (int k = 0; k < 3; k++) xi[k] = L[Ly::XPOS + 3 * b + k] + t[k];
      m = L[Ly::DMASS + b];
    }
    const float ms = tsum(m);
    const float inv = frcp(ms);
    const float com[3] = {tsum(m * xi[0]) * inv, tsum(m * xi[1]) * inv, tsum(m * xi[2]) * inv};
    if (lane == 0)
      for (int k = 0; k < 3; k++) L[Ly::COM + k] = com[k];
    if (mv) {
      const float d[3] = {xi[0] - com[0], xi[1] - com[1], xi[2] - com[2]};
      const float dd = dot3(d, d);
      const int o = Ly::CIN + 10 * b;
      L[o + 0] = rot[0] + m * (dd - d[0] * d[0]);
      L[o + 1] = rot[4] + m * (dd - d[1] * d[1]);
      L[o + 2] = rot[8] + m * (dd - d[2] * d[2]);
      L[o + 3] = rot[1] - m * d[0] * d[1];
      L[o + 4] = rot[2] - m * d[0] * d[2];
      L[o + 5] = rot[5] - m * d[1] * d[2];
      L[o + 6] = m * d[0]; L[o + 7] = m * d[1]; L[o + 8] = m * d[2];
      L[o + 9] = m;
    }
    team_for<NJ>(lane, [&](int j) {
      const int oj = Md::B_JREC + 9 * j;
      const bool jh = Md::B_JAFF && j >= Md::B_JN0;
      const int b = jh ? j + Md::B_JBD : ti(oj), da = jh ? j + Md::B_JDD : ti(oj + 1);
      const float off[3] = {com[0] - L[Ly::XPOS + 3 * b], com[1] - L[Ly::XPOS + 3 * b + 1], com[2] - L[Ly::XPOS + 3 * b + 2]};
      if (!jh && ti(oj + 3) == 0) {
        for (int k = 0; k < 3; k++)
          for (int q = 0; q < 6; q++) L[Ly::CDOF + 6 * (da + k) + q] = (q == 3 + k) ? 1.0f : 0.0f;
        for (int k = 0; k < 3; k++) {
          const float ax[3] = {L[Ly::XMAT + 9 * b + k], L[Ly::XMAT + 9 * b + 3 + k], L[Ly::XMAT + 9 * b + 6 + k]};
          float t[3];
          cross3(t, ax, off);
          const int o = Ly::CDOF + 6 * (da + 3 + k);
          L[o] = ax[0]; L[o + 1] = ax[1]; L[o + 2] = ax[2]; L[o + 3] = t[0]; L[o + 4] = t[1]; L[o + 5] = t[2];
        }
      } else {
        float R[9], ax[3], t[3];
        const float ja[3] = {tf(oj + 4), tf(oj + 5), tf(oj + 6)};
        for (int k = 0; k < 9; k++) R[k] = L[Ly::XMAT + 9 * b + k];
        mulmv3(ax, R, ja);
        cross3(t, ax, off);
        const int o = Ly::CDOF + 6 * da;
        L[o] = ax[0]; L[o + 1] = ax[1]; L[o + 2] = ax[2]; L[o + 3] = t[0]; L[o + 4] = t[1]; L[o + 5] = t[2];
      }
    });
    TSYNC();
  }

  static constexpr int RCA = TL::RCA, RFB = TL::RFB;

  static DK void root_motion(LP L, int lane, int b, float* cv, float* ca) {
    const int da = Md::body_dofadr[b], nd = Md::body_dofnum[b];
    if (nd == 6) {
      for (int i = 0; i < 3; i++) cv[3 + i] += L[Ly::QVEL + da + i];
      float cvt[6];
      for (int k = 0; k < 6; k++) cvt[k] = cv[k];
      for (int i = 3; i < 6; i++) {
        float cd[6], cdd[6];
        for (int k = 0; k < 6; k++) cd[k] = L[Ly::CDOF + 6 * (da + i) + k];
        cross_motion(cdd, cvt, cd);
        if (lane == i - 3)
          for (int k = 0; k < 6; k++) L[Ly::CDD1 + 6 * (i - 3) + k] = cdd[k];
        const float v = L[Ly::QVEL + da + i];
        for (int k = 0; k < 6; k++) { ca[k] += cdd[k] * v; cv[k] += cd[k] * v; }
      }
    } else {
      for (int jj = 0; jj < nd; jj++) {
        float cd[6], cdd[6];
        for (int k = 0; k < 6; k++) cd[k] = L[Ly::CDOF + 6 * (da + jj) + k];
        cross_motion(cdd, cv, cd);
        const float v = L[Ly::QVEL + da + jj];
        for (int k = 0; k < 6; k++) { ca[k] += cdd[k] * v; cv[k] += cd[k] * v; }
      }
    }
  }

  static DK void rne(LP L, int lane) {
    rne_vel(L, lane);
    rne_rest<0>(L, lane);
  }
  static DK void rne_vel(LP L, int lane) {
#pragma clang fp reassociate(on)
    STAGE_T0();
    constexpr int NR = Md::T_NROOT, BL = Md::T_BRLEN, MD = Md::T_BRMD;
    static_assert(Md::T_NBR <= TEAM, "a limb per lane");
    float cv[6], ca[6];
    for (int k = 0; k < 6; k++) { cv[k] = 0.0f; ca[k] = (k >= 3) ? -Md::gravity[k - 3] : 0.0f; }
#pragma unroll
    for (int r = 0; r < NR; r++) {
      const int b = Md::T_ROOT[r];
      root_motion(L, lane, b, cv, ca);
      if (lane == 0)
        for (int k = 0; k < 6; k++) { L[Ly::CVEL + 6 * b + k] = cv[k]; L[RCA + 6 * b + k] = ca[k]; }
    }
    const bool limb = lane < Md::T_NBR;
    int bb[BL];
#pragma unroll
    for (int d = 0; d < BL; d++) bb[d] = limb_body(lane, d);
    {
      float cd[BL][MD][6], qv[BL][MD];
      int dof[BL][MD];
#pragma unroll
      for (int d = 0; d < BL; d++)
#pragma unroll
        for (int jj = 0; jj < MD; jj++) dof[d][jj] = limb_dof(lane, 2 * d + jj);
#pragma unroll
      for (int d = 0; d < BL; d++)
#pragma unroll
        for (int jj = 0; jj < MD; jj++) {
          const int i = dof[d][jj] >= 0 ? dof[d][jj] : 0;
          for (int k = 0; k < 6; k++) cd[d][jj][k] = L[Ly::CDOF + 6 * i + k];
          const float q = L[Ly::QVEL + i];
          qv[d][jj] = dof[d][jj] >= 0 ? q : 0.0f;
        }
#pragma unroll
      for (int d = 0; d < BL; d++) {
#pragma unroll
        for (int jj = 0; jj < MD; jj++) {
          float cdd[6];
          cross_motion(cdd, cv, cd[d][jj]);
          const float v = qv[d][jj];
          for (int k = 0; k < 6; k++) { ca[k] += cdd[k] * v; cv[k] += cd[d][jj][k] * v; }
        }
        if (limb && bb[d] >= 0)
          for (int k = 0; k < 6; k++) { L[Ly::CVEL + 6 * bb[d] + k] = cv[k]; L[RCA + 6 * bb[d] + k] = ca[k]; }
      }
    }
    TSYNC();
    STAGE_MARK(21);
  }
  template <int PART>
  static DK void rne_rest(LP L, int lane) {
#pragma clang fp reassociate(on)
    STAGE_T0();
    team_for<NB, 1>(lane, [&](int b) {
      if (!moving(b)) return;
      float I[10], v6[6], a6[6], f[6], t1[6], t2[6];
      for (int k = 0; k < 10; k++) I[k] = L[Ly::CIN + 10 * b + k];
      for (int k = 0; k < 6; k++) { v6[k] = L[Ly::CVEL + 6 * b + k]; a6[k] = L[RCA + 6 * b + k]; }
      mul_inert_vec(f, I, a6);
      mul_inert_vec(t1, I, v6);
      cross_force(t2, v6, t1);
      for (int k = 0; k < 6; k++) L[RFB + 6 * b + k] = f[k] + t2[k];
    });
    TSYNC();
    STAGE_MARK(22);
    subtree_sums<PART>(L, lane);
    team_for<NV>(lane, [&](int i) {
      const int b = dof_body(i);
      float s = 0.0f;
      for (int k = 0; k < 6; k++) s += L[Ly::CDOF + 6 * i + k] * L[TL::CFRC + 6 * b + k];
      L[Ly::FSM + i] = -s;
    });
    TSYNC();
  }
  static constexpr bool bodies_distinct() {
    for (int m = 0; m < Md::T_NBR; m++)
      for (int d = 0; d < Md::T_BRLEN; d++) {
        const int b = Md::T_BRB[m][d];
        if (b < 0) continue;
        for (int m2 = 0; m2 < Md::T_NBR; m2++)
          for (int d2 = 0; d2 < Md::T_BRLEN; d2++)
            if ((m2 != m || d2 != d) && Md::T_BRB[m2][d2] == b) return false;
        for (int r = 0; r < Md::T_NROOT; r++)
          if (Md::T_ROOT[r] == b) return false;
      }
    for (int r = 0; r < Md::T_NROOT; r++)
      for (int r2 = r + 1; r2 < Md::T_NROOT; r2++)
        if (Md::T_ROOT[r] == Md::T_ROOT[r2]) return false;
    return true;
  }
  template <int PART>
  static DK void subtree_sums(LP L, int lane) {
#pragma clang fp reassociate(on)
    STAGE_T0();
    constexpr int NR = Md::T_NROOT, BL = Md::T_BRLEN;
    static_assert(TEAM == 6 + 10, "a force or inertia component per lane");
    {
      int lk = lane;
      asm volatile("" : "+v"(lk));
      const bool fk = lk < 6;
      const int fsrc = PART == 2 ? Ly::CIN + lk : RFB + lk, fdst = PART == 2 ? TL::XDUM1 + lk : TL::CFRC + lk;
      const int idst = PART == 1 ? TL::XDUM0 + (lk - 6) : TL::XCIN + (lk - 6);
      const int src = fk ? fsrc : Ly::CIN + (lk - 6), dst = fk ? fdst : idst;
      const int st = fk ? 6 : 10;
      static_assert(bodies_distinct(), "limb and root bodies must be distinct");
      float xb[Md::T_NBR][BL], xr[NR];
#pragma unroll
      for (int m = 0; m < Md::T_NBR; m++)
#pragma unroll
        for (int d = 0; d < BL; d++) {
          const int b = Md::T_BRB[m][d];
// ... 333 lines not shown
      }
    }
  }

  static DK void smooth_acc(LP L, int lane, const float (*Mc)[NV]) {
    Fac F;
#pragma unroll
    for (int s = 0; s < NC; s++)
#pragma unroll
      for (int r = 0; r < NV; r++) F.col[s][r] = Mc[s][r];
    float x[NC];
#pragma unroll
    for (int s = 0; s < NC; s++) {
      const int c = TEAM * s + lane;
      const float v = L[Ly::FSM + (c < NV ? c : 0)];
      x[s] = c < NV ? v : 0.0f;
    }
    factor_solve(F, x, lane);
#pragma unroll
    for (int s = 0; s < NC; s++) {
      const int c = TEAM * s + lane;
      if (c < NV) L[Ly::QSM + c] = x[s];
    }
    TSYNC();
  }
  static DK void smooth_factor(Fac& F, int lane, const float (*Mc)[NV]) {
#pragma unroll
    for (int s = 0; s < NC; s++)
#pragma unroll
      for (int r = 0; r < NV; r++) F.col[s][r] = Mc[s][r];
    factor(F, lane);
  }
  static DK void smooth_solve(LP L, int lane, const Fac& F) {
    float x[NC];
#pragma unroll
    for (int s = 0; s < NC; s++) {
      const int c = TEAM * s + lane;
      const float v = L[Ly::FSM + (c < NV ? c : 0)];
      x[s] = c < NV ? v : 0.0f;
    }
    solve_factored(F, x, lane);
#pragma unroll
    for (int s = 0; s < NC; s++) {
      const int c = TEAM * s + lane;
      if (c < NV) L[Ly::QSM + c] = x[s];
    }
    TSYNC();
  }

  template <int... R>
  static DK void mul_acc(const float (*Mc)[NV], const float* x, float* y, std::integer_sequence<int, R...>) {
#pragma unroll
    for (int s = 0; s < NC; s++) ((y[s] += Mc[s][R] * bc<R % TEAM>(x[R / TEAM])), ...);
  }
  static DK void mul_cols(LP L, int lane, const float (*Mc)[NV], const float* x, int Y) {
    float y[NC];
#pragma unroll
    for (int s = 0; s < NC; s++) y[s] = 0.0f;
    mul_acc(Mc, x, y, std::make_integer_sequence<int, NV>{});
#pragma unroll
    for (int s = 0; s < NC; s++) {
      const int c = TEAM * s + lane;
      if (c < NV) L[Y + c] = y[s];
    }
  }
  static DK void lane_vec(LP L, int lane, int X, float* x) {
#pragma unroll
    for (int s = 0; s < NC; s++) {
      const int c = TEAM * s + lane;
      x[s] = L[X + (c < NV ? c : 0)];
    }
  }

  static constexpr unsigned chain_mask(int b) {
    unsigned msk = 0;
    for (int q = 0; q < Md::chain_len[b]; q++) msk |= 1u << Md::chain[b][q];
    return msk;
  }

  template <int R>
  static DK void jdj_row(Fac& F, const float (*kc)[6], const float (*cdc)[6], const bool* in, unsigned msk) {
    if (!((msk >> R) & 1u)) return;
#pragma unroll
    for (int s = 0; s < NC; s++) {
      if (R < TEAM * s) continue;
      if (FREE0 && R < 3) { F.col[s][R] += kc[s][3 + R]; continue; }
      float h = 0.0f;
      for (int k = 0; k < 6; k++) h += bc<R % TEAM>(kc[R / TEAM][k]) * cdc[s][k];
      F.col[s][R] += in[s] ? h : 0.0f;
    }
  }
  template <int... R>
  static DK void jdj_rows(Fac& F, const float (*kc)[6], const float (*cdc)[6], const bool* in, unsigned msk,
                          std::integer_sequence<int, R...>) {
    (jdj_row<R>(F, kc, cdc, in, msk), ...);
  }

  template <bool FF, int OUT = Ly::SRCH>
  static DK bool newton_fused(LP L, int lane, const float (*Mc)[NV]) {
    STAGE_T0();
    if constexpr (!FF) {
      if (Md::FOOT_PAIR >= 0) {
        const int row = R_CON + 16 * Md::FOOT_PAIR + lane;
        const float act = (L[Ly::JA + row] < 0.0f && L[Ly::RD + row] != 0.0f) ? 1.0f : 0.0f;
        if (tsum(act) > 0.0f) return false;
      }
    }
    Fac F;
    float g[NC];
#pragma unroll
    for (int s = 0; s < NC; s++) {
      const int c = TEAM * s + lane, cc = c < NV ? c : 0;
      const bool valid = c < NV;
      float gr = L[Ly::MA + cc] - L[Ly::FSM + cc], diag = 0.0f;
      const int fr = dof_fric(cc), frc = fr >= 0 ? fr : 0;
      {
        const float D = L[Ly::RD + frc], x = L[Ly::JA + frc], f = L[Ly::DFRIC + cc], rf = f * frcp(D);
        const float force = x <= -rf ? f : (x >= rf ? -f : -D * x);
        const bool quad = x > -rf && x < rf;
        gr -= fr >= 0 ? force : 0.0f;
        diag += (fr >= 0 && quad) ? D : 0.0f;
      }
      const int lr = dof_lim(cc), lrc = lr >= 0 ? lr : 0;
      {
        const float D = L[Ly::RD + R_LIM + lrc], x = L[Ly::JA + R_LIM + lrc], sg = L[Ly::LSGN + lrc];
        const bool act = lr >= 0 && x < 0.0f;
        gr -= act ? sg * (-D * x) : 0.0f;
        diag += act ? D : 0.0f;
      }
      g[s] = valid ? gr : 0.0f;
#pragma unroll
      for (int r = 0; r < NV; r++) F.col[s][r] = r >= TEAM * s ? Mc[s][r] + (r == c ? diag : 0.0f) : 0.0f;
    }
    STAGE_MARK(16);
    float Kh[21], Fh[6];
    {
      const int hs = lane >> 3, l8 = lane & 7;
      const int p = hs == 0 ? Md::PLANE_PAIR[0] : Md::PLANE_PAIR[1];
      const float mu = tf(Md::B_PAIR + PAIRW * p + 2);
#pragma unroll
      for (int k = 0; k < 21; k++) Kh[k] = 0.0f;
#pragma unroll
      for (int k = 0; k < 6; k++) Fh[k] = 0.0f;
#pragma unroll
      for (int h2 = 0; h2 < 2; h2++) {
        const int j = l8 + 8 * h2, slot = 4 * p + (j >> 2), e = j & 3, row = R_CON + 4 * slot + e;
        const float D = L[Ly::RD + row], x = L[Ly::JA + row];
        const float w = (x < 0.0f && D != 0.0f) ? D : 0.0f;
        const float force = -w * x;
        const int t = 1 + (e >> 1);
        const float sg = (e & 1) ? -mu : mu;
        float u[3], r3[3], a[6];
        for (int q = 0; q < 3; q++) {
          u[q] = L[Ly::CFR + 9 * slot + q] + sg * L[Ly::CFR + 9 * slot + 3 * t + q];
          r3[q] = L[Ly::CR + 3 * slot + q];
        }
        cross3(a, r3, u);
        a[3] = u[0]; a[4] = u[1]; a[5] = u[2];
        int o = 0;
        for (int q = 0; q < 6; q++)
          for (int kk = q; kk < 6; kk++) { Kh[o] += w * a[q] * a[kk]; o++; }
        for (int q = 0; q < 6; q++) Fh[q] += force * a[q];
      }
#pragma unroll
      for (int k = 0; k < 21; k++) Kh[k] = hsum8(Kh[k]);
#pragma unroll
      for (int k = 0; k < 6; k++) Fh[k] = hsum8(Fh[k]);
    }
#pragma unroll
    for (int side = 0; side < 2; side++) {
      const int p = Md::PLANE_PAIR[side];
      const int foot = cgeom_slot<Md>(Md::pair_geom2[p]);
      float K[21], Fv[6];
#pragma unroll
      for (int k = 0; k < 21; k++) K[k] = side == 0 ? bc<0>(Kh[k]) : bc<8>(Kh[k]);
#pragma unroll
      for (int k = 0; k < 6; k++) Fv[k] = side == 0 ? bc<0>(Fh[k]) : bc<8>(Fh[k]);
      constexpr unsigned MASKL = chain_mask(Md::LFOOT_BODY), MASKR = chain_mask(Md::RFOOT_BODY);
      const unsigned msk = foot == 1 ? MASKL : MASKR;
      float cdc[NC][6], kc[NC][6];
      bool in[NC];
#pragma unroll
      for (int s = 0; s < NC; s++) {
        const int c = TEAM * s + lane, cc = c < NV ? c : 0;
        in[s] = c < NV && ((msk >> cc) & 1u);
        for (int k = 0; k < 6; k++) cdc[s][k] = L[Ly::CDOF + 6 * cc + k];
        float gf = 0.0f;
        for (int q = 0; q < 6; q++) {
          float sacc = 0.0f;
          for (int k = 0; k < 6; k++) sacc += K[kidx(q, k)] * cdc[s][k];
          kc[s][q] = in[s] ? sacc : 0.0f;
          gf += cdc[s][q] * Fv[q];
        }
        g[s] -= in[s] ? gf : 0.0f;
      }
      jdj_rows(F, kc, cdc, in, msk, std::make_integer_sequence<int, NV>{});
    }
    if constexpr (FF) {
      if constexpr (Md::FOOT_PAIR >= 0) {
        constexpr int p = Md::FOOT_PAIR;
        constexpr int g1 = cgeom_slot<Md>(Md::pair_geom1[p]), g2 = cgeom_slot<Md>(Md::pair_geom2[p]);
        constexpr unsigned M1 = chain_mask(g1 == 1 ? Md::LFOOT_BODY : Md::RFOOT_BODY);
        constexpr unsigned M2 = chain_mask(g2 == 1 ? Md::LFOOT_BODY : Md::RFOOT_BODY);
        const float mu = tf(Md::B_PAIR + PAIRW * p + 2);
        const int slot = 4 * p + (lane >> 2), e = lane & 3, row = R_CON + 4 * slot + e;
        const float D = L[Ly::RD + row], x = L[Ly::JA + row];
        const float w = (x < 0.0f && D != 0.0f) ? D : 0.0f;
        const float force = -w * x;
        const int t = 1 + (e >> 1);
        const float sg = (e & 1) ? -mu : mu;
        float u[3], r3[3], a[6];
        for (int q = 0; q < 3; q++) {
          u[q] = L[Ly::CFR + 9 * slot + q] + sg * L[Ly::CFR + 9 * slot + 3 * t + q];
          r3[q] = L[Ly::CR + 3 * slot + q];
        }
        cross3(a, r3, u);
        a[3] = u[0]; a[4] = u[1]; a[5] = u[2];
        float K[21], Fv[6];
        {
          int o = 0;
          for (int q = 0; q < 6; q++)
            for (int kk = q; kk < 6; kk++) { K[o] = tsum(w * a[q] * a[kk]); o++; }
          for (int q = 0; q < 6; q++) Fv[q] = tsum(force * a[q]);
        }
#pragma unroll
        for (int s = 0; s < NC; s++) {
          const int c = TEAM * s + lane, cc = c < NV ? c : 0;
          const float sc = c < NV ? (float)((int)((M2 >> cc) & 1u) - (int)((M1 >> cc) & 1u)) : 0.0f;
          float cdc[6], kc[6];
          for (int k = 0; k < 6; k++) cdc[k] = sc * L[Ly::CDOF + 6 * cc + k];
          float gf = 0.0f;
          for (int q = 0; q < 6; q++) {
            float sacc = 0.0f;
            for (int k = 0; k < 6; k++) sacc += K[kidx(q, k)] * cdc[k];
            kc[q] = sacc;
            gf += cdc[q] * Fv[q];
          }
          g[s] -= gf;
#pragma unroll
          for (int r = 0; r < NV; r++) {
            const int sr = (int)((M2 >> r) & 1u) - (int)((M1 >> r) & 1u);
            if (sr == 0 || r < TEAM * s) continue;
            float h = 0.0f;
            for (int k = 0; k < 6; k++) h += L[Ly::CDOF + 6 * r + k] * kc[k];
            F.col[s][r] += sr > 0 ? h : -h;
          }
        }
      }
    }
    STAGE_MARK(17);
    if constexpr (FF) factor_solve_dense(F, g, lane);
    else factor_solve(F, g, lane);
    STAGE_MARK(18);
#pragma unroll
    for (int s = 0; s < NC; s++) {
      const int c = TEAM * s + lane;
      if (c < NV) L[OUT + c] = -g[s];
    }
    TSYNC();
    return true;
  }

  static DK void cgeom_frame(LP L, int gs, float* gp, float* gR) {
    const int o = Md::B_CGEOM + 16 * gs, b = ti(o);
    float R[9], t[3], gpos[3], gm[9];
    for (int k = 0; k < 9; k++) { R[k] = L[Ly::XMAT + 9 * b + k]; gm[k] = tf(o + 4 + k); }
    for (int k = 0; k < 3; k++) gpos[k] = tf(o + 1 + k);
    mulmv3(t, R, gpos);
    for (int k = 0; k < 3; k++) gp[k] = L[Ly::XPOS + 3 * b + k] + t[k];
    mulmm3(gR, R, gm);
  }

  static DK void collide_planes(LP L, int lane) {
    constexpr int NH = Md::NHV;
    const int h = lane >> 3, sub = lane & 7;
    const int p = Md::PLANE_PAIR[0] * (1 - h) + Md::PLANE_PAIR[1] * h;
    const int gs = cgeom_slot<Md>(Md::pair_geom2[p]);
    float pp[3], PR[9], cp[3], CR[9];
    Ph::geom_frame(L, 0, pp, PR);
    cgeom_frame(L, gs, cp, CR);
    const float n[3] = {PR[2], PR[5], PR[8]};
    const float dif[3] = {pp[0] - cp[0], pp[1] - cp[1], pp[2] - cp[2]};
    float pl[3], nl[3];
    mulmtv3(pl, CR, dif);
    mulmtv3(nl, CR, n);
    auto HVf = [&](int k, int q) { return tf(Md::B_HULL + 3 * k + q); };
    constexpr int R = (NH + 7) / 8;
    float sup[R], vx[R], vy[R], vz[R];
    float smax = -1e30f;
    for (int r = 0; r < R; r++) {
      const int k = sub + 8 * r;
      const bool ok = k < NH;
      vx[r] = ok ? HVf(k, 0) : 0.0f; vy[r] = ok ? HVf(k, 1) : 0.0f; vz[r] = ok ? HVf(k, 2) : 0.0f;
      sup[r] = ok ? (pl[0] - vx[r]) * nl[0] + (pl[1] - vy[r]) * nl[1] + (pl[2] - vz[r]) * nl[2] : -1e30f;
      smax = fmaxf(smax, sup[r]);
    }
    smax = hmax8(smax);
    const float thr = fmaxf(smax - 1e-3f, 0.0f);
    float dm[R];
    for (int r = 0; r < R; r++) dm[r] = (sub + 8 * r < NH) ? (sup[r] > thr ? 0.0f : -1e6f) : -1e30f;
    auto argmax = [&](const float* v, float tol) -> int {
      float mx = -1e30f;
      for (int r = 0; r < R; r++) mx = fmaxf(mx, v[r]);
      mx = hmax8(mx);
      int best = 1 << 20;
      for (int r = 0; r < R; r++) {
        const int k = sub + 8 * r;
        if (k < NH && v[r] >= mx - tol) best = min(best, k);
      }
      best = hmin8i(best);
      return best < NH ? best : NH - 1;
    };
    auto vert = [&](int k, float* o) { o[0] = HVf(k, 0); o[1] = HVf(k, 1); o[2] = HVf(k, 2); };
    float s[R];
    const int a = argmax(dm, 0.0f);
    float pa[3];
    vert(a, pa);
    for (int r = 0; r < R; r++) {
      const float dx = pa[0] - vx[r], dy = pa[1] - vy[r], dz = pa[2] - vz[r];
      s[r] = dx * dx + dy * dy + dz * dz + dm[r];
    }
    const int b = argmax(s, MANIFOLD_TOL);
    float pb[3];
    vert(b, pb);
    float amb[3] = {pa[0] - pb[0], pa[1] - pb[1], pa[2] - pb[2]}, ab[3];
    cross3(ab, nl, amb);
    for (int r = 0; r < R; r++) {
      const float ap[3] = {pa[0] - vx[r], pa[1] - vy[r], pa[2] - vz[r]};
      s[r] = fabsf(dot3(ap, ab)) + dm[r];
    }
    const int c = argmax(s, MANIFOLD_TOL);
    float pc[3];
    vert(c, pc);
    float amc[3] = {pa[0] - pc[0], pa[1] - pc[1], pa[2] - pc[2]};
    float bmc[3] = {pb[0] - pc[0], pb[1] - pc[1], pb[2] - pc[2]};
    float ac[3], bc[3];
    cross3(ac, nl, amc);
    cross3(bc, nl, bmc);
    int d;
    {
      float s1[R], s2[R];
      float mx = -1e30f;
      for (int r = 0; r < R; r++) {
        const float bp[3] = {pb[0] - vx[r], pb[1] - vy[r], pb[2] - vz[r]};
        const float ap[3] = {pa[0] - vx[r], pa[1] - vy[r], pa[2] - vz[r]};
        s1[r] = fabsf(dot3(bp, bc)) + dm[r];
        s2[r] = fabsf(dot3(ap, ac)) + dm[r];
        mx = fmaxf(mx, fmaxf(s1[r], s2[r]));
      }
      mx = hmax8(mx);
      int best = 1 << 20;
      for (int r = 0; r < R; r++) {
        const int k = sub + 8 * r;
        if (k < NH && s1[r] >= mx - MANIFOLD_TOL) best = min(best, k);
        if (k < NH && s2[r] >= mx - MANIFOLD_TOL) best = min(best, NH + k);
      }
      d = hmin8i(best);
      d = d < 2 * NH ? d : 2 * NH - 1;
      d = d >= NH ? d - NH : d;
    }
    if (sub < 4) {
      const int idx[4] = {a, b, c, d};
      const int me = idx[sub];
      bool unique = true;
      for (int e = 0; e < 4; e++) unique = unique && !(e < sub && idx[e] == me);
      float v[3], vw[3], pos[3], nw[3], fr[9];
      vert(me, v);
      mulmv3(vw, CR, v);
      const float sp = (pl[0] - v[0]) * nl[0] + (pl[1] - v[1]) * nl[1] + (pl[2] - v[2]) * nl[2];
      nw[0] = n[0]; nw[1] = n[1]; nw[2] = n[2];
      for (int q = 0; q < 3; q++) vw[q] += cp[q];
      const float dist = unique ? -sp : 1.0f;
      for (int q = 0; q < 3; q++) pos[q] = vw[q] - 0.5f * dist * nw[q];
      make_frame(fr, nw);
      Ph::store_contact(L, 4 * p + sub, dist, pos, fr);
    }
  }

  static DK float hmin8f(float v) { return -hmax8_nc(-v); }
  static DK unsigned half_bits(unsigned long long b, int lane) {
    const int base = ((int)threadIdx.x & 63) & ~7;
    (void)lane;
    return (unsigned)(b >> base) & 0xFFu;
  }
  template <int F>
  static DK float nf_dot(const float* x) {
    return cdot<fbits(Md::hull_face_normal[F][0]), fbits(Md::hull_face_normal[F][1]), fbits(Md::hull_face_normal[F][2])>(x);
  }
  template <int K>
  static DK float hv_dot(const float* x) {
    return cdot<fbits(Md::hull_vert[K][0]), fbits(Md::hull_vert[K][1]), fbits(Md::hull_vert[K][2])>(x);
  }
  template <int E>
  static DK float dxc_dot(const float* x) {
    return cdot<fbits(Md::hull_edge_dxc[E][0]), fbits(Md::hull_edge_dxc[E][1]), fbits(Md::hull_edge_dxc[E][2])>(x);
  }
#define DUCK_C3(A) fbits(A[0]), fbits(A[1]), fbits(A[2])
  template <int F>
  static DK void nf_off_dot3(const float* x, const float* y, const float* z, float* r) {
    cdot3v_off<DUCK_C3(Md::hull_face_normal[F]), fbits(Md::hull_face_offset[F])>(x, y, z, r);
  }
  template <int F>
  static DK void nf_dot4(const float* x, const float* y, const float* z, const float* u, float* r) {
    cdot4v<DUCK_C3(Md::hull_face_normal[F])>(x, y, z, u, r);
  }
  template <int K>
  static DK void hv_dot5(const float* x, const float* y, const float* z, const float* u, const float* w, float* r) {
    cdot5v<DUCK_C3(Md::hull_vert[K])>(x, y, z, u, w, r);
  }
  template <int K>
  static DK void hv_noff5(const float* x, const float* y, const float* z, const float* u, const float* w, const float* o,
                          float* r) {
    cdot5v_noff<DUCK_C3(Md::hull_vert[K])>(x, y, z, u, w, o, r);
  }
  template <int K>
  static DK void hv_dot2(const float* x, float& ra, float& rb) {
    cdot2c<DUCK_C3(Md::hull_vert[K]), DUCK_C3(Md::hull_vert[K + 1])>(x, ra, rb);
  }
  template <int F>
  static DK void nf_dot2(const float* x, float& ra, float& rb) {
    cdot2c<DUCK_C3(Md::hull_face_normal[F]), DUCK_C3(Md::hull_face_normal[F + 1])>(x, ra, rb);
  }
// ... 971 lines not shown
      float a[3], b[3], ab[3], sd[3];
      vtx(ref1, FV[bi][i], a);
      vtx(ref1, FV[bi][i + 1 < nr ? i + 1 : 0], b);
      for (int q = 0; q < 3; q++) ab[q] = b[q] - a[q];
      cross3(sd, ab, fn);
      int nt = 0;
      for (int j = 0; j < np; j++) {
        const int jn = j + 1 < np ? j + 1 : 0;
        const float P[3] = {L[src + 3 * j], L[src + 3 * j + 1], L[src + 3 * j + 2]};
        const float Q[3] = {L[src + 3 * jn], L[src + 3 * jn + 1], L[src + 3 * jn + 2]};
        const float dp = sd[0] * (P[0] - a[0]) + sd[1] * (P[1] - a[1]) + sd[2] * (P[2] - a[2]);
        const float dq = sd[0] * (Q[0] - a[0]) + sd[1] * (Q[1] - a[1]) + sd[2] * (Q[2] - a[2]);
        if (dp <= 0.0f && nt < CLIPMAX) {
          for (int q = 0; q < 3; q++) L[dst + 3 * nt + q] = P[q];
          nt++;
        }
        if ((dp <= 0.0f) != (dq <= 0.0f) && nt < CLIPMAX) {
          const float tt = dp / (dp - dq);
          for (int q = 0; q < 3; q++) L[dst + 3 * nt + q] = P[q] + tt * (Q[q] - P[q]);
          nt++;
        }
      }
      TSYNC();
      np = nt;
      const int sw = src;
      src = dst;
      dst = sw;
    }
    float poly[CLIPMAX][3], depth[CLIPMAX];
    bool mask[CLIPMAX], any = false;
#pragma unroll
    for (int k = 0; k < CLIPMAX; k++) {
      const bool ok = k < np;
      for (int q = 0; q < 3; q++) poly[k][q] = ok ? L[src + 3 * k + q] : 0.0f;
      depth[k] = off - dot3(fn, poly[k]);
      mask[k] = ok && depth[k] > 0.0f;
      any = any || mask[k];
    }
    if (!any) return;
    int idx[4];
    manifold_points<CLIPMAX>(poly, mask, fn, idx);
    if (lane < 4) {
      const int c = lane;
      bool unique = true;
      for (int e = 0; e < 4; e++) unique = unique && !(e < c && idx[e] == idx[c]);
      const float dist = unique ? -pick1<CLIPMAX>(depth, idx[c]) : 1.0f;
      float v[3], pos[3];
      pick3<CLIPMAX>(poly, idx[c], v);
      for (int a = 0; a < 3; a++) pos[a] = v[a] - 0.5f * dist * fn[a];
      Ph::store_contact(L, slot0 + c, dist, pos, fr);
    }
  }

  static DNI void collide_hulls_rare(LP L, int lane) {
    constexpr int p = Md::FOOT_PAIR < 0 ? 0 : Md::FOOT_PAIR;
    const int s1 = cgeom_slot<Md>(Md::pair_geom1[p]), s2 = cgeom_slot<Md>(Md::pair_geom2[p]);
    float p1[3], R1[9], p2[3], R2[9], t[3], c1[3], c2[3];
    Ph::geom_frame(L, s1, p1, R1);
    Ph::geom_frame(L, s2, p2, R2);
    const float hc[3] = {Md::hull_center[0], Md::hull_center[1], Md::hull_center[2]};
    mulmv3(t, R1, hc);
    for (int a = 0; a < 3; a++) c1[a] = p1[a] + t[a];
    mulmv3(t, R2, hc);
    for (int a = 0; a < 3; a++) c2[a] = p2[a] + t[a];
    const float cc[3] = {c2[0] - c1[0], c2[1] - c1[1], c2[2] - c1[2]};
    collide_hulls_team(L, lane, 4 * p, p1, R1, p2, R2, cc);
  }

  static DK void collision(LP L, int lane, const float* hf) {
    STAGE_T0();
    if constexpr (Md::FLOOR_TYPE == 1) collide_hfield(L, lane, hf);
    else collide_planes(L, lane);
    STAGE_MARK(26);
    if (Md::FOOT_PAIR >= 0) {
      constexpr int p = Md::FOOT_PAIR;
      const int s1 = cgeom_slot<Md>(Md::pair_geom1[p]), s2 = cgeom_slot<Md>(Md::pair_geom2[p]);
      float p1[3], R1[9], p2[3], R2[9], t[3];
      Ph::geom_frame(L, s1, p1, R1);
      Ph::geom_frame(L, s2, p2, R2);
      float c1[3], c2[3];
      const float hc[3] = {Md::hull_center[0], Md::hull_center[1], Md::hull_center[2]};
      mulmv3(t, R1, hc);
      for (int a = 0; a < 3; a++) c1[a] = p1[a] + t[a];
      mulmv3(t, R2, hc);
      for (int a = 0; a < 3; a++) c2[a] = p2[a] + t[a];
      const float cc[3] = {c2[0] - c1[0], c2[1] - c1[1], c2[2] - c1[2]};
      if (dot3(cc, cc) > 4.0f * Md::hull_radius * Md::hull_radius || boxes_separated(p1, R1, p2, R2)) {
        if (lane < 4) {
          const float nofr[9] = {0, 0, 1, 0, 1, 0, -1, 0, 0};
          const float zero[3] = {L[Ly::COM], L[Ly::COM + 1], L[Ly::COM + 2]};
          Ph::store_contact(L, 4 * p + lane, 1.0f, zero, nofr);
        }
      } else {
        TSYNC();
#ifdef DUCK_STAGE_PROF
        if (lane == 0) STAGE_ADD(27, 1ull);
#endif
#ifndef DUCK_DIAG_NO_RARE_CALLS
        collide_hulls_rare(L, lane);
#endif
      }
    }
    TSYNC();
  }

  static DK void make_rows(LP L, int lane) {
    if (lane < NFRIC) {
      const int r = lane, i = fric_dof(r);
      L[Ly::RD + r] = tf(Md::B_FRIC + 3 * r + 1);
      L[Ly::AREF + r] = -tf(Md::B_FRIC + 3 * r + 2) * L[Ly::QVEL + i];
    }
    team_for<NLIM>(lane, [&](int r) {
      const int o = Md::B_LIM + LIMW * r;
      const int i = lim_dof(r), qa = lim_qadr(r);
      const float q = L[Ly::QPOS + qa];
      const float dlo = q - tf(o + 2), dhi = tf(o + 3) - q;
      const float pos = fminf(dlo, dhi) - tf(o + 4);
      const float sgn = dlo < dhi ? 1.0f : -1.0f;
      const float k = tf(o + 5), b = tf(o + 6);
      const float si[5] = {tf(o + 8), tf(o + 9), tf(o + 10), tf(o + 11), tf(o + 12)};
      const float imp = imp_of(si, pos);
      const float R = fmaxf(tf(o + 7) * (1.0f - imp) * frcp(imp), 1e-15f);
      const bool active = pos < 0.0f;
      L[Ly::RD + R_LIM + r] = active ? frcp(R) : 0.0f;
      L[Ly::AREF + R_LIM + r] = active ? (-b * sgn * L[Ly::QVEL + i] - k * imp * pos) : 0.0f;
      L[Ly::LSGN + r] = sgn;
    });
    if (lane < NCON) {
      const int slot = lane, p = slot >> 2, o = Md::B_PAIR + PAIRW * p;
      float SL[6], SR[6];
      for (int k = 0; k < 6; k++) { SL[k] = L[Ly::CVEL + 6 * Md::LFOOT_BODY + k]; SR[k] = L[Ly::CVEL + 6 * Md::RFOOT_BODY + k]; }
      const float pos = L[Ly::CDIST + slot] - tf(o + 4);
      const bool active = pos < 0.0f;
      const float k = tf(o + 5), b = tf(o + 6);
      const float si[5] = {tf(o + 8), tf(o + 9), tf(o + 10), tf(o + 11), tf(o + 12)};
      const float imp = imp_of(si, pos);
      const float R = fmaxf(tf(o + 3) * (1.0f - imp) * frcp(imp), 1e-15f);
      float vel[4];
      contact_jx(L, p, slot, SL, SR, vel);
      for (int e = 0; e < 4; e++) {
        const int row = R_CON + 4 * slot + e;
        L[Ly::RD + row] = active ? frcp(R) : 0.0f;
        L[Ly::AREF + row] = active ? (-b * vel[e] - k * imp * pos) : 0.0f;
      }
    }
    TSYNC();
  }

  static DK void contact_jx(LP L, int p, int slot, const float* SL, const float* SR, float* out4) {
#pragma clang fp contract(on)
    const int o = Md::B_PAIR + PAIRW * p;
    const int s1 = ti(o), s2 = ti(o + 1);
    const float mu = tf(o + 2);
    const float r[3] = {L[Ly::CR + 3 * slot], L[Ly::CR + 3 * slot + 1], L[Ly::CR + 3 * slot + 2]};
    float v[3] = {0.0f, 0.0f, 0.0f}, t[3];
    if (s2 != 0) { Ph::contact_vel(s2 == 1 ? SL : SR, r, t); v[0] += t[0]; v[1] += t[1]; v[2] += t[2]; }
    if (s1 != 0) { Ph::contact_vel(s1 == 1 ? SL : SR, r, t); v[0] -= t[0]; v[1] -= t[1]; v[2] -= t[2]; }
    float jr[3];
    for (int q = 0; q < 3; q++)
      jr[q] = L[Ly::CFR + 9 * slot + 3 * q] * v[0] + L[Ly::CFR + 9 * slot + 3 * q + 1] * v[1] +
              L[Ly::CFR + 9 * slot + 3 * q + 2] * v[2];
    out4[0] = jr[0] + mu * jr[1];
    out4[1] = jr[0] - mu * jr[1];
    out4[2] = jr[0] + mu * jr[2];
    out4[3] = jr[0] - mu * jr[2];
  }

  static DK constexpr int kidx(int q, int k) {
    return q <= k ? (q * 6 - (q * (q - 1)) / 2 + (k - q)) : (k * 6 - (k * (k - 1)) / 2 + (q - k));
  }

  struct Pt { float alpha, q0p, q1, q2, d0, d1; };

  static DK void spatial2(LP L, int lane, int X, int X2, float& so, float& so2) {
    so = 0.0f;
    so2 = 0.0f;
    if (lane < 12) {
      int lo = lane;
      asm volatile("" : "+v"(lo));
      const bool left = lo < 6;
      const int k = left ? lo : lo - 6;
      float s = 0.0f, s2 = 0.0f;
#pragma unroll
      for (int c = 0; c < Md::MAXCHAIN; c++) {
        const int iL = Md::chain[Md::LFOOT_BODY][c], iR = Md::chain[Md::RFOOT_BODY][c];
        if (iL < 0 && iR < 0) continue;
        const bool ok = left ? iL >= 0 : iR >= 0;
        const int ic = left ? (iL >= 0 ? iL : 0) : (iR >= 0 ? iR : 0);
        if (FREE0 && iL == iR && iL >= 0 && iL < 3) {
          const float x = L[X + iL];
          s += k == 3 + iL ? x : 0.0f;
          if (X2 >= 0) {
            const float x2 = L[X2 + iL];
            s2 += k == 3 + iL ? x2 : 0.0f;
          }
          continue;
        }
        const float cv = L[Ly::CDOF + 6 * ic + k];
        const float cd = ok ? cv : 0.0f;
        s += cd * L[X + ic];
        if (X2 >= 0) s2 += cd * L[X2 + ic];
      }
      so = s;
      so2 = s2;
    }
  }

  static DK void sp_bcast(float v, float* SL, float* SR) {
    SL[0] = bc<0>(v); SL[1] = bc<1>(v); SL[2] = bc<2>(v); SL[3] = bc<3>(v); SL[4] = bc<4>(v); SL[5] = bc<5>(v);
    SR[0] = bc<6>(v); SR[1] = bc<7>(v); SR[2] = bc<8>(v); SR[3] = bc<9>(v); SR[4] = bc<10>(v); SR[5] = bc<11>(v);
  }

  static DK float fric_cost(float D, float x, float f) {
    const float rf = f * frcp(D);
    const float lo = -f * x - 0.5f * rf * f, hi = f * x - 0.5f * rf * f, qd = 0.5f * D * x * x;
    const float r = x >= rf ? hi : qd;
    return x <= -rf ? lo : r;
  }

  static constexpr int NLR = (NLIM + TEAM - 1) / TEAM;
  struct Rows2 {
    float fja, fv, frf, flin0, ffja, ffv, fQ0, fQ1, fQ2;
    float ja[NLR + 4], v[NLR + 4], Q0[NLR + 4], Q1[NLR + 4], Q2[NLR + 4];
  };
  static DK void set_fric(Rows2& R, float D, float ja, float v, float f) {
    const float rf = f * frcp(D);
    R.fja = ja; R.fv = v; R.frf = rf;
    R.flin0 = -0.5f * rf * f; R.ffja = f * ja; R.ffv = f * v;
    R.fQ0 = 0.5f * D * ja * ja; R.fQ1 = D * v * ja; R.fQ2 = 0.5f * D * v * v;
  }
  static DK void set_row(Rows2& R, int k, float D, float ja, float v) {
    R.ja[k] = ja; R.v[k] = v;
    R.Q0[k] = 0.5f * D * ja * ja; R.Q1[k] = D * v * ja; R.Q2[k] = 0.5f * D * v * v;
  }

  static DK void quad2(const Rows2& R, float alpha, float& q0, float& q1, float& q2) {
    {
      const float x = R.fja + alpha * R.fv;
      const bool lo = x <= -R.frf, hi = x >= R.frf, quad = !(lo || hi);
      const float sg = lo ? -1.0f : 1.0f;
      q0 += quad ? R.fQ0 : R.flin0 + sg * R.ffja;
      q1 += quad ? R.fQ1 : sg * R.ffv;
      q2 += quad ? R.fQ2 : 0.0f;
    }
#pragma unroll
    for (int k = 0; k < NLR + 4; k++) {
      const float on = (R.ja[k] + alpha * R.v[k] < 0.0f) ? 1.0f : 0.0f;
      q0 = fmaf(on, R.Q0[k], q0);
      q1 = fmaf(on, R.Q1[k], q1);
      q2 = fmaf(on, R.Q2[k], q2);
    }
  }

  static DK void solve(LP L, int lane, float* scratch, int stride, const float (*Mc)[NV]) {
    STAGE_T0();
    const float g0 = warm_start(L, lane, Mc);
#if defined(DUCK_DOUBLE) && DUCK_DOUBLE == 21
    (void)warm_start(L, lane, Mc);
#endif
    newton(L, lane, scratch, stride, Mc, g0);
  }
  static DK void warm_start_a0(LP L, int lane, const float (*Mc)[NV], float* SL, float* SR) {
    float sw, ss;
    spatial2(L, lane, Ly::WARM, -1, sw, ss);
    {
      float xw[NC];
      lane_vec(L, lane, Ly::WARM, xw);
      mul_cols(L, lane, Mc, xw, Ly::MA);
    }
    sp_bcast(sw, SL, SR);
  }
  static DK void warm_start_a1(LP L, int lane, const float* SL, const float* SR, float& cwp) {
    cwp = 0.0f;
    {
      const bool fr = lane < NFRIC;
      const int r = fr ? lane : 0, i = fric_dof(r);
      const float D = L[Ly::RD + r], f = L[Ly::DFRIC + i], ar = L[Ly::AREF + r];
      const float jw = L[Ly::WARM + i] - ar;
      cwp += fr ? fric_cost(D, jw, f) : 0.0f;
      L[fr ? Ly::JA + r : TL::SINK + lane] = jw;
    }
    team_for<NLIM>(lane, [&](int r) {
      const int i = lim_dof(r), row = R_LIM + r;
      const float D = L[Ly::RD + row], sg = L[Ly::LSGN + r], ar = L[Ly::AREF + row];
      const float jw = sg * L[Ly::WARM + i] - ar;
      cwp += jw < 0.0f ? 0.5f * D * jw * jw : 0.0f;
      L[Ly::JA + row] = jw;
    });
    if (lane < NCON) {
      float vw[4];
      contact_jx(L, lane >> 2, lane, SL, SR, vw);
      for (int e = 0; e < 4; e++) {
        const int row = R_CON + 4 * lane + e;
        const float D = L[Ly::RD + row], ar = L[Ly::AREF + row];
        const float jw = vw[e] - ar;
        cwp += jw < 0.0f ? 0.5f * D * jw * jw : 0.0f;
        L[Ly::JA + row] = jw;
      }
    }
  }
  static DK float warm_start_b(LP L, int lane, float cwp, bool& warm) {
    float ss, s2;
    spatial2(L, lane, Ly::QSM, -1, ss, s2);
    TSYNC();
    float SL2[6], SR2[6];
    sp_bcast(ss, SL2, SR2);
    float csp = 0.0f, gwp = 0.0f;
    {
      const bool fr = lane < NFRIC;
      const int r = fr ? lane : 0, i = fric_dof(r);
      const float D = L[Ly::RD + r], f = L[Ly::DFRIC + i], ar = L[Ly::AREF + r];
      const float js = L[Ly::QSM + i] - ar;
      csp += fr ? fric_cost(D, js, f) : 0.0f;
      L[fr ? Ly::JV + r : TL::SINK + TEAM + lane] = js;
// ... 167 lines not shown
      const unsigned long long ex = __builtin_amdgcn_read_exec();
      L[TL::KC + 88 + lane] = __int_as_float((int)(ex & 0xffffffffull));
      L[TL::KC + 104 + lane] = __int_as_float((int)(ex >> 32));
      L[TL::KC + 120 + lane] = L[Ly::SRCH + lane];
    }
#endif
    team_for<NV>(lane, [&](int i) {
      const float sv = L[Ly::SRCH + i];
      sn += sv * sv;
      sMa += sv * L[Ly::MA + i];
      sf += sv * L[Ly::FSM + i];
      sMv += sv * L[Ly::GRAD + i];
    });
#ifdef DUCK_LS_DUMP
    L[TL::KC + 56 + lane] = (float)lane;
    L[TL::KC + 72 + lane] = sn;
#endif
    sn = tsum(sn); sMa = tsum(sMa); sf = tsum(sf); sMv = tsum(sMv);
    STAGE_MARK(12);
    const float gtol = Md::tolerance * Md::ls_tolerance * sqrtf(sn) * Md::meaninertia * (float)(NV > 1 ? NV : 1);
    const float G0 = g0, G1 = sMa - sf, G2 = 0.5f * sMv;
    auto mk = [&](float alpha, float q0, float q1, float q2) {
      q1 = tsum(q1) + G1; q2 = tsum(q2) + G2;
      Pt p;
      p.alpha = alpha;
      p.q0p = q0;
      p.q1 = q1;
      p.q2 = q2;
      p.d0 = 2.0f * alpha * q2 + q1;
      p.d1 = 2.0f * q2;
      return p;
    };
    auto cost = [&](const Pt& p) { return p.alpha * p.alpha * p.q2 + p.alpha * p.q1 + (tsum(p.q0p) + G0); };
    Pt p0;
    {
      float q0 = 0, q1 = 0, q2 = 0;
      quad2(R, 0.0f, q0, q1, q2);
#ifdef DUCK_LS_DUMP
      L[TL::KC + 8 + 3 * lane] = q0; L[TL::KC + 9 + 3 * lane] = q1; L[TL::KC + 10 + 3 * lane] = q2;
      if (lane == 0) { L[TL::KC] = G0; L[TL::KC + 1] = G1; L[TL::KC + 2] = G2; L[TL::KC + 3] = gtol; L[TL::KC + 4] = sn; }
#endif
      p0 = mk(0.0f, q0, q1, q2);
    }
    Pt lo;
    {
      const float a1 = p0.alpha - p0.d0 * frcp(p0.d1);
      float q0 = 0, q1 = 0, q2 = 0;
      quad2(R, a1, q0, q1, q2);
      lo = mk(a1, q0, q1, q2);
    }
    Pt hi;
    if (lo.d0 < p0.d0) { hi = p0; } else { hi = lo; lo = p0; }
    bool swap = true;
    const float gtol_ls = fmaxf(gtol, DUCK_LS_DFLOOR * fabsf(p0.d0));
#ifdef DUCK_LS_NOBREAK
    bool stop = false;
#pragma unroll
    for (int it = 0; it < Md::ls_iterations; it++) {
      bool done = stop || !swap;
      done = done || ((lo.d0 < 0.0f) && (lo.d0 > -gtol_ls));
      done = done || ((hi.d0 > 0.0f) && (hi.d0 < gtol_ls));
      stop = done;
#else
#ifdef DUCK_STAGE_PROF
    int its = 0;
#endif
    for (int it = 0; it < Md::ls_iterations; it++) {
      bool done = !swap;
      done = done || ((lo.d0 < 0.0f) && (lo.d0 > -gtol_ls));
      done = done || ((hi.d0 > 0.0f) && (hi.d0 < gtol_ls));
      if (done) break;
#ifdef DUCK_STAGE_PROF
      its = it + 1;
      if (threadIdx.x < 64 && (int)threadIdx.x == __ffsll((long long)__ballot(1)) - 1) STAGE_ADD(56, 1ull);
#endif
#endif
      const float al = lo.alpha - lo.d0 / lo.d1, ah = hi.alpha - hi.d0 / hi.d1, am = 0.5f * (lo.alpha + hi.alpha);
      float a0 = 0, a1 = 0, a2 = 0, b0 = 0, b1 = 0, b2 = 0, c0 = 0, c1 = 0, c2 = 0;
      quad2(R, al, a0, a1, a2);
      quad2(R, ah, b0, b1, b2);
      quad2(R, am, c0, c1, c2);
      const Pt lo_next = mk(al, a0, a1, a2), hi_next = mk(ah, b0, b1, b2), mid = mk(am, c0, c1, c2);
#ifdef DUCK_LS_NOBREAK
      const bool s1 = !done && ((lo.d0 > 0.0f) || (lo.d0 < lo_next.d0));
      if (s1) lo = lo_next;
      const bool s2 = !done && (mid.d0 < 0.0f) && (lo.d0 < mid.d0);
      if (s2) lo = mid;
      const bool s3 = !done && ((hi.d0 < 0.0f) || (hi.d0 > hi_next.d0));
      if (s3) hi = hi_next;
      const bool s4 = !done && (mid.d0 > 0.0f) && (hi.d0 > mid.d0);
      if (s4) hi = mid;
      swap = done ? swap : (s1 || s2 || s3 || s4);
#else
      const bool s1 = (lo.d0 > 0.0f) || (lo.d0 < lo_next.d0);
      if (s1) lo = lo_next;
      const bool s2 = (mid.d0 < 0.0f) && (lo.d0 < mid.d0);
      if (s2) lo = mid;
      const bool s3 = (hi.d0 < 0.0f) || (hi.d0 > hi_next.d0);
      if (s3) hi = hi_next;
      const bool s4 = (mid.d0 > 0.0f) && (hi.d0 > mid.d0);
      if (s4) hi = mid;
      swap = s1 || s2 || s3 || s4;
#endif
    }
#if defined(DUCK_STAGE_PROF) && !defined(DUCK_LS_NOBREAK)
    if (threadIdx.x < 64 && (lane & 15) == 0) { STAGE_ADD(57, (unsigned long long)its); STAGE_ADD(58, 1ull); }
#endif
    const float lo_cost = cost(lo), hi_cost = cost(hi), p0_cost = cost(p0);
    const bool improved = (lo_cost < p0_cost) || (hi_cost < p0_cost);
    const float alpha = lo_cost < hi_cost ? lo.alpha : hi.alpha;
    if (improved)
      team_for<NV>(lane, [&](int i) { L[Ly::QACC + i] += L[Ly::SRCH + i] * alpha; });
    TSYNC();
    STAGE_MARK(13);
    if constexpr (Md::iterations <= 1) {
      break;
    } else {
      if (++newton_it >= Md::iterations) break;
      const float a = improved ? alpha : 0.0f;
      const float cnew = improved ? (lo_cost < hi_cost ? lo_cost : hi_cost) : p0_cost;
      g0 = G0 + a * G1 + a * a * G2;
      team_for<NV>(lane, [&](int i) { L[Ly::MA + i] += a * L[Ly::GRAD + i]; });
      if (lane < NFRIC) L[Ly::JA + lane] = R.fja + a * R.fv;
#pragma unroll
      for (int m = 0; m < NLR; m++) {
        const int r = lane + TEAM * m;
        if (r < NLIM) L[Ly::JA + R_LIM + r] = R.ja[m] + a * R.v[m];
      }
      if (lane < NCON)
        for (int e = 0; e < 4; e++) L[Ly::JA + R_CON + 4 * lane + e] = R.ja[NLR + e] + a * R.v[NLR + e];
      TSYNC();
      const float scale = 1.0f / (Md::meaninertia * (float)(NV > 1 ? NV : 1));
      if (scale * (p0_cost - cnew) < Md::tolerance) break;
    }
    }
  }

  static DK void sensors(LP L, int lane) {
    const float com[3] = {L[Ly::COM], L[Ly::COM + 1], L[Ly::COM + 2]};
    float cacc1[6];
    for (int k = 0; k < 6; k++) cacc1[k] = (k >= 3) ? -Md::gravity[k - 3] : 0.0f;
    for (int i = 0; i < 6; i++) {
      const float v = L[Ly::QVEL + i], a = L[Ly::QACC + i];
      for (int k = 0; k < 6; k++) {
        const float cdd = i >= 3 ? L[Ly::CDD1 + 6 * (i - 3) + k] : 0.0f;
        cacc1[k] += cdd * v + L[Ly::CDOF + 6 * i + k] * a;
      }
    }
    for (int s = lane; s < Md::NSENSOR; s += TEAM) {
      const int os = Md::B_SENS + 20 * s;
      const int typ = ti(os), site = ti(os + 1), adr = ti(os + 2), b = ti(os + 3);
      float R[9], sp[3], sR[9], t[3], SM[9];
      const float spos[3] = {tf(os + 4), tf(os + 5), tf(os + 6)};
      for (int k = 0; k < 9; k++) { R[k] = L[Ly::XMAT + 9 * b + k]; SM[k] = tf(os + 7 + k); }
      mulmv3(t, R, spos);
      for (int k = 0; k < 3; k++) sp[k] = L[Ly::XPOS + 3 * b + k] + t[k];
      mulmm3(sR, R, SM);
      const float off[3] = {sp[0] - com[0], sp[1] - com[1], sp[2] - com[2]};
      float ang[3] = {L[Ly::CVEL + 6 * b], L[Ly::CVEL + 6 * b + 1], L[Ly::CVEL + 6 * b + 2]}, lin[3];
      cross3(t, ang, off);
      for (int k = 0; k < 3; k++) lin[k] = L[Ly::CVEL + 6 * b + 3 + k] + t[k];
      float o[4] = {0.0f, 0.0f, 0.0f, 0.0f};
      if (typ == 0) mulmtv3(o, sR, ang);
      else if (typ == 1) mulmtv3(o, sR, lin);
      else if (typ == 2) {
        float acc[3];
        cross3(t, cacc1, off);
        for (int k = 0; k < 3; k++) acc[k] = cacc1[3 + k] + t[k];
        cross3(t, ang, lin);
        for (int k = 0; k < 3; k++) acc[k] += t[k];
        mulmtv3(o, sR, acc);
      } else if (typ == 3) { o[0] = sR[2]; o[1] = sR[5]; o[2] = sR[8]; }
      else if (typ == 4) { o[0] = sR[0]; o[1] = sR[3]; o[2] = sR[6]; }
      else if (typ == 5) { o[0] = lin[0]; o[1] = lin[1]; o[2] = lin[2]; }
      else if (typ == 6) { o[0] = ang[0]; o[1] = ang[1]; o[2] = ang[2]; }
      else if (typ == 7) { o[0] = sp[0]; o[1] = sp[1]; o[2] = sp[2]; }
      else if (typ == 8) {
        const float bq[4] = {L[Ly::XQ + 4 * b], L[Ly::XQ + 4 * b + 1], L[Ly::XQ + 4 * b + 2], L[Ly::XQ + 4 * b + 3]};
        const float sq[4] = {tf(os + 16), tf(os + 17), tf(os + 18), tf(os + 19)};
        qmul(o, bq, sq);
        qnormalize(o);
      }
      const int dim = typ == 8 ? 4 : 3;
      for (int k = 0; k < dim; k++) L[Ly::SENS + adr + k] = o[k];
      if (typ == 0 && site == Md::IMU_SITE) { L[Ly::IMUR] = sR[6]; L[Ly::IMUR + 1] = sR[7]; L[Ly::IMUR + 2] = sR[8]; }
      if (typ == 7 && site == Md::LFOOT_SITE) L[Ly::FOOTZ] = sp[2];
      if (typ == 7 && site == Md::RFOOT_SITE) L[Ly::FOOTZ + 1] = sp[2];
    }
    if (lane < 2) {
      constexpr int p0 = Md::PLANE_PAIR[0], p1 = Md::PLANE_PAIR[1];
      constexpr int s20 = cgeom_slot<Md>(Md::pair_geom2[p0]), s21 = cgeom_slot<Md>(Md::pair_geom2[p1]);
      const int p = lane == 0 ? p0 : p1, s2 = lane == 0 ? s20 : s21;
      float mn = 1e4f;
      for (int c = 0; c < 4; c++) mn = fminf(mn, L[Ly::CDIST + 4 * p + c]);
      L[Ly::OCON + s2 - 1] = mn < 0.0f ? 1.0f : 0.0f;
    }
    TSYNC();
  }

  static DK void euler(LP L, int lane) {
    const float dt = Md::timestep;
    team_for<NV>(lane, [&](int i) {
      L[Ly::WARM + i] = L[Ly::QACC + i];
      L[Ly::QVEL + i] += dt * L[Ly::QACC + i];
    });
    TSYNC();
    if (lane == 0) {
      for (int k = 0; k < 3; k++) L[Ly::QPOS + k] += dt * L[Ly::QVEL + k];
      const float v[3] = {L[Ly::QVEL + 3], L[Ly::QVEL + 4], L[Ly::QVEL + 5]};
      const float nvv = sqrtf(dot3(v, v));
      float ax[3] = {1.0f, 0.0f, 0.0f};
      if (nvv > 1e-15f) { ax[0] = v[0] / nvv; ax[1] = v[1] / nvv; ax[2] = v[2] / nvv; }
      float s, c;
      __sincosf(0.5f * dt * nvv, &s, &c);
      const float qr[4] = {c, ax[0] * s, ax[1] * s, ax[2] * s};
      float q[4] = {L[Ly::QPOS + 3], L[Ly::QPOS + 4], L[Ly::QPOS + 5], L[Ly::QPOS + 6]};
      qmul(q, q, qr);
      qnormalize(q);
      for (int k = 0; k < 4; k++) L[Ly::QPOS + 3 + k] = q[k];
    }
    team_for<NJ, 1>(lane, [&](int j) {
      const int oj = Md::B_JREC + 9 * j;
      const bool jh = Md::B_JAFF && j >= Md::B_JN0;
      const int qa = jh ? j + Md::B_JQD : ti(oj + 2), da = jh ? j + Md::B_JDD : ti(oj + 1);
      L[Ly::QPOS + qa] += dt * L[Ly::QVEL + da];
    });
    TSYNC();
  }

  static DK void step(LP L, int lane, bool integrate, bool want_out, float* aux, int aux_stride, float* scratch,
                      int sstride, const float* hf) {
    STAGE_T0();
    kinematics(L, lane);
#if defined(DUCK_DOUBLE) && DUCK_DOUBLE == 6
    kinematics(L, lane);
#endif
    STAGE_MARK(0);
    com_pos(L, lane);
#if defined(DUCK_DOUBLE) && DUCK_DOUBLE == 7
    com_pos(L, lane);
#endif
    STAGE_MARK(1);
    rne(L, lane);
    STAGE_MARK(2);
    crb(L, lane);
#if defined(DUCK_DOUBLE) && DUCK_DOUBLE == 1
    crb(L, lane);
#endif
    STAGE_MARK(3);
    smooth(L, lane);
#if defined(DUCK_DOUBLE) && DUCK_DOUBLE == 8
    rne(L, lane);
    smooth(L, lane);
#endif
    STAGE_MARK(28);
    collision(L, lane, hf);
#if defined(DUCK_DOUBLE) && DUCK_DOUBLE == 2
    collision(L, lane, hf);
#endif
    STAGE_MARK(5);
    make_rows(L, lane);
#if defined(DUCK_DOUBLE) && DUCK_DOUBLE == 3
    make_rows(L, lane);
#endif
    STAGE_MARK(6);
    {
      float Mc[NC][NV];
      load_cols(L, lane, Mc, false);
      STAGE_MARK(20);
      smooth_acc(L, lane, Mc);
#if defined(DUCK_DOUBLE) && DUCK_DOUBLE == 4
      smooth_acc(L, lane, Mc);
#endif
      STAGE_MARK(4);
      solve(L, lane, scratch, sstride, Mc);
#if defined(DUCK_DOUBLE) && DUCK_DOUBLE == 5
      solve(L, lane, scratch, sstride, Mc);
#endif
    }
    STAGE_MARK(7);
    if (want_out) {
      sensors(L, lane);
      if (aux) {
        if (lane == 0) Ph::write_aux(L, aux, aux_stride);
      }
    }
    if (integrate) {
      euler(L, lane);
    } else {
      team_for<NV>(lane, [&](int i) { L[Ly::WARM + i] = L[Ly::QACC + i]; });
      TSYNC();
    }
    STAGE_MARK(8);
  }

  enum { EV_KIN = 0, EV_VEL = 1, EV_FSM = 2, EV_ROWS = 3, EV_EULER = 4, EV_M = 5, EV_QSM = 6, EV_WA = 7, EV_DIR = 8,
         EV_TIMEOUT = 9 };
  static_assert(EV_TIMEOUT < TL::NEV_G || !LAT, "event slots");
  static DK lds_int* ev_ptr(int k) {
    extern __shared__ float lds_dyn[];
    const int g = LAT == 2 ? __builtin_amdgcn_readfirstlane((int)threadIdx.x >> 7) : 0;
    return (lds_int*)(lds_dyn + TL::EV) + 4 * (k + TL::NEV_G * g);
  }
  static DK void ev_init(int tid) {
    extern __shared__ float lds_dyn[];
    if (tid < TL::NEV) ((lds_int*)(lds_dyn + TL::EV))[4 * tid] = 0;
  }
  static DK void ev_signal(int k, int v) {
    __hip_atomic_store(ev_ptr(k), v, __ATOMIC_RELEASE, __HIP_MEMORY_SCOPE_WORKGROUP);
  }
  static DK void ev_wait(int k, int v) {
#ifdef DUCK_LAT_FORCE_TIMEOUT
    const bool forced = blockIdx.x == 1 && k == EV_M;
    const int LIMIT = forced ? 1 << 6 : 1 << 20;
    if (forced) v += 1 << 24;
#else
    constexpr int LIMIT = 1 << 20;
#endif
    for (int it = 0; __hip_atomic_load(ev_ptr(k), __ATOMIC_ACQUIRE, __HIP_MEMORY_SCOPE_WORKGROUP) < v; it++) {
      if (it > LIMIT) {
        if ((threadIdx.x & 63) == 0) atomicAdd(&g_lat_timeouts, 1u);
        __hip_atomic_store(ev_ptr(EV_TIMEOUT), 1, __ATOMIC_RELAXED, __HIP_MEMORY_SCOPE_WORKGROUP);
        break;
      }
      __builtin_amdgcn_s_sleep(1);
    }
  }
  static DK bool ev_timed_out(int g) {
    extern __shared__ float lds_dyn[];
    return ((lds_int*)(lds_dyn + TL::EV))[4 * (EV_TIMEOUT + TL::NEV_G * g)] != 0;
  }
  static DK void lat_r0(LP L, int lane, int s) {
    ev_wait(EV_EULER, s);
    LAT_T(0, s);
    kinematics(L, lane);
    com_pos(L, lane);
    ev_signal(EV_KIN, s + 1);
    LAT_T(1, s);
    rne_vel(L, lane);
    ev_signal(EV_VEL, s + 1);
    LAT_T(2, s);
    rne_rest<1>(L, lane);
    smooth(L, lane);
    ev_signal(EV_FSM, s + 1);
    LAT_T(3, s);
  }
  static DK void lat_r1(LP L, int lane, int s, bool integrate, bool want_out, float* scratch, int sstride) {
    ev_wait(EV_KIN, s + 1);
    LAT_T(10, s);
    subtree_sums<2>(L, lane);
    crb(L, lane);
    ev_signal(EV_M, s + 1);
    LAT_T(11, s);
    {
      float Mc[NC][NV];
      load_cols(L, lane, Mc, false);
      LAT_T(12, s);
      float SL[6], SR[6], cwp;
      warm_start_a0(L, lane, Mc, SL, SR);
      ev_wait(EV_ROWS, s + 1);
      LAT_T(13, s);
      warm_start_a1(L, lane, SL, SR, cwp);
      ev_signal(EV_WA, s + 1);
      LAT_T(14, s);
      ev_wait(EV_QSM, s + 1);
      LAT_T(15, s);
      bool warm;
      const float g0 = warm_start_b(L, lane, cwp, warm);
      LAT_T(16, s);
      bool pre = false;
      if (__ballot(!warm) == 0ull) {
        ev_wait(EV_DIR, s + 1);
        pre = L[TL::XDIR + NV] != 0.0f;
      }
      LAT_T(19, s);
      newton(L, lane, scratch, sstride, Mc, g0, pre);
      LAT_T(17, s);
    }
    if (want_out) sensors(L, lane);
    if (integrate) {
      euler(L, lane);
    } else {
      team_for<NV>(lane, [&](int i) { L[Ly::WARM + i] = L[Ly::QACC + i]; });
      TSYNC();
    }
    ev_signal(EV_EULER, s + 1);
    LAT_T(18, s);
  }
  static DK void lat_r2(LP L, int lane, int s, const float* hf) {
    ev_wait(EV_KIN, s + 1);
    LAT_T(20, s);
    collision(L, lane, hf);
    LAT_T(21, s);
    ev_wait(EV_VEL, s + 1);
    LAT_T(22, s);
    make_rows(L, lane);
    ev_signal(EV_ROWS, s + 1);
    LAT_T(23, s);
  }
  static DK void lat_r3(LP L, int lane, int s) {
    ev_wait(EV_M, s + 1);
    LAT_T(30, s);
    float Mc[NC][NV];
    load_cols(L, lane, Mc, false);
    Fac F;
    smooth_factor(F, lane, Mc);
    LAT_T(31, s);
    ev_wait(EV_FSM, s + 1);
    LAT_T(32, s);
    smooth_solve(L, lane, F);
    ev_signal(EV_QSM, s + 1);
    LAT_T(33, s);
    ev_wait(EV_WA, s + 1);
    LAT_T(34, s);
    const bool ok = newton_fused<false, TL::XDIR>(L, lane, Mc);
    if (lane == 0) L[TL::XDIR + NV] = ok ? 1.0f : 0.0f;
    TSYNC();
    ev_signal(EV_DIR, s + 1);
    LAT_T(35, s);
  }

  static DK void lat2_a(LP L, int lane, int s, const float* hf) {
    ev_wait(EV_EULER, s);
    LAT2_T(0, s);
    kinematics(L, lane);
    com_pos(L, lane);
    ev_signal(EV_KIN, s + 1);
    LAT2_T(1, s);
    rne_vel(L, lane);
    LAT2_T(2, s);
    rne_rest<1>(L, lane);
    smooth(L, lane);
    ev_signal(EV_FSM, s + 1);
    LAT2_T(3, s);
    collision(L, lane, hf);
    LAT2_T(4, s);
    make_rows(L, lane);
    ev_signal(EV_ROWS, s + 1);
    LAT2_T(5, s);
    ev_wait(EV_M, s + 1);
    LAT2_T(6, s);
    float Mc[NC][NV];
    load_cols(L, lane, Mc, false);
    ev_wait(EV_WA, s + 1);
    LAT2_T(7, s);
    const bool ok = newton_fused<false, TL::XDIR>(L, lane, Mc);
    if (lane == 0) L[TL::XDIR + NV] = ok ? 1.0f : 0.0f;
    TSYNC();
    ev_signal(EV_DIR, s + 1);
    LAT2_T(8, s);
  }
  static DK void lat2_b(LP L, int lane, int s, bool integrate, bool want_out, float* scratch, int sstride) {
    ev_wait(EV_KIN, s + 1);
    LAT2_T(10, s);
    subtree_sums<2>(L, lane);
    crb(L, lane);
    ev_signal(EV_M, s + 1);
    LAT2_T(11, s);
    {
      float Mc[NC][NV];
      load_cols(L, lane, Mc, false);
      LAT2_T(12, s);
      float SL[6], SR[6], cwp;
      warm_start_a0(L, lane, Mc, SL, SR);
      LAT2_T(13, s);
      {
        Fac F;
        smooth_factor(F, lane, Mc);
        LAT2_T(14, s);
        ev_wait(EV_FSM, s + 1);
        LAT2_T(15, s);
        smooth_solve(L, lane, F);
        LAT2_T(16, s);
      }
      ev_wait(EV_ROWS, s + 1);
      LAT2_T(17, s);
      warm_start_a1(L, lane, SL, SR, cwp);
      ev_signal(EV_WA, s + 1);
      LAT2_T(18, s);
      bool warm;
      const float g0 = warm_start_b(L, lane, cwp, warm);
      LAT2_T(19, s);
// ... 21 lines not shown
```

Before: 20.70 million env-steps/s.

## Realign per-env LDS layout to 16-byte fields and pad records for wide loads

Reorders the per-env LDS slice so matrix and vector fields start at 16-byte (or 8-byte) boundaries, and pads per-body records (xpos to 4, xmat to 10, contact r/frame to 4/10) so the compiler can emit ds_read_b128/b64. The LDS base and slice pointers are marked aligned via attributes and __builtin_assume. The alignment level is chosen at compile time so that whatever the scene already kept in LDS still fits. Padding raises the slice footprint and changes bank patterns, and it relies on the compiler actually merging the accesses.

```diff
diff --git a/open_duck_playground_amd/csrc/duck_env_kernels.h b/open_duck_playground_amd/csrc/duck_env_kernels.h
--- a/open_duck_playground_amd/csrc/duck_env_kernels.h
+++ b/open_duck_playground_amd/csrc/duck_env_kernels.h
@@ -42,7 +42,8 @@
 
 template <class Md, int LAT = 0>
 DK lds_float* env_slice(float* lds, int t) {
-  return (lds_float*)(lds + t * TLay<Md, LAT>::STRIDE);
+  static_assert(TLay<Md, LAT>::STRIDE % 4 == 0, "an env slice starts 16-byte aligned");
+  return lds_assume16((lds_float*)(lds + t * TLay<Md, LAT>::STRIDE));
 }
 
 template <class Md>
@@ -237,7 +238,7 @@
 __global__ void __launch_bounds__(TPB) reset_kernel(KArgs A) {
   using Ly = Lay<Md>;
   {
-    extern __shared__ float lds_t[];
+    extern __shared__ LDS_ALIGNED float lds_t[];
     load_model_tables<Md>(lds_t);
   }
   int lane;
@@ -245,7 +246,7 @@
   const int e = blockIdx.x * TEAM_WG + t;
   if (e >= A.n) return;
   if (A.mask && !A.mask[e]) return;
-  extern __shared__ float lds[];
+  extern __shared__ LDS_ALIGNED float lds[];
   lds_float* const L = env_slice<Md>(lds, t);
   const duck_env_config& c = A.cfg;
   const duck_layout& Lo = A.lay;
@@ -611,7 +612,7 @@
 #endif
   using TL = TLay<Md>;
   {
-    extern __shared__ float lds_t[];
+    extern __shared__ LDS_ALIGNED float lds_t[];
     load_model_tables<Md>(lds_t);
   }
   STAGE_MARK(14);
@@ -619,7 +620,7 @@
   const int t = local_env(lane);
   const int e = blockIdx.x * TEAM_WG + t;
   const int n = A.n;
-  extern __shared__ float lds[];
+  extern __shared__ LDS_ALIGNED float lds[];
   if constexpr (TL::ES_LDS) {
     const int j = threadIdx.x % TEAM_WG, ej = blockIdx.x * TEAM_WG + j;
     lds_float* esj = (lds_float*)(lds + TL::ES + j * TL::ESTRIDE);
@@ -697,7 +698,7 @@
   static_assert(TL::TAB_LDS && TL::ES_LDS, "latency mode: the model blob and the hot state in LDS");
   static_assert(TPB == 4 * 64 && WGL * TEAM == 64 * (LAT == 2 ? 2 : 1),
                 "latency modes: 4 waves, one set of 4 teams per wave (paired: per pair of waves)");
-  extern __shared__ float lds[];
+  extern __shared__ LDS_ALIGNED float lds[];
   LAT_T(40, 5);
   TPL::ev_init((int)threadIdx.x);
   load_model_tables<Md, LAT>(lds);
@@ -800,7 +801,7 @@
                                                      const float* ctrl_g, int nsub, float* aux) {
   using Ly = Lay<Md>;
   {
-    extern __shared__ float lds_t[];
+    extern __shared__ LDS_ALIGNED float lds_t[];
     load_model_tables<Md>(lds_t);
   }
   int lane;
@@ -808,7 +809,7 @@
   const int e = blockIdx.x * TEAM_WG + t;
   const int n = A.n;
   if (e >= n) return;
-  extern __shared__ float lds[];
+  extern __shared__ LDS_ALIGNED float lds[];
   lds_float* const L = env_slice<Md>(lds, t);
   for (int i = 0; i < Md::NQ; i++) L[Ly::QPOS + i] = qpos_g[(size_t)i * n + e];
   for (int i = 0; i < Md::NV; i++) { L[Ly::QVEL + i] = qvel_g[(size_t)i * n + e]; L[Ly::WARM + i] = warm_g[(size_t)i * n + e]; }
@@ -989,7 +990,27 @@
 #endif
 }
 
+constexpr bool name_is(const char* a, const char* b) {
+  for (; *a && *a == *b; a++, b++) {}
+  return *a == *b;
+}
+template <class Md>
+constexpr bool lds_budget_kept(const char* name) {
+  const bool flat = name_is(name, "flat"), rough = name_is(name, "rough");
+  if (!flat && !rough && !name_is(name, "backlash") && !name_is(name, "rough_backlash")) return true;
+  return TLay<Md>::TAB_LDS && TLay<Md, 1>::FITS && TLay<Md, 2>::FITS && (!(flat || rough) || TLay<Md>::ES_LDS) &&
+         (!flat || LatX2<Md>::PAYS);
+}
+template <class Md>
+constexpr bool slices_aligned() {
+  return TLay<Md>::STRIDE % 4 == 0 && TLay<Md>::TAB % 4 == 0 && TLay<Md, 1>::STRIDE % 4 == 0 && TLay<Md, 1>::TAB % 4 == 0 &&
+         TLay<Md, 2>::STRIDE % 4 == 0 && TLay<Md, 2>::TAB % 4 == 0 && TLay<Md, LAT_X2>::STRIDE % 4 == 0 &&
+         TLay<Md, LAT_X2>::TAB % 4 == 0;
+}
+
 #define DUCK_DEFINE_VARIANT(NAME, MODEL)                                                        \
+  static_assert(lds_budget_kept<MODEL>(#NAME), "scene " #NAME " no longer keeps in LDS what it kept"); \
+  static_assert(slices_aligned<MODEL>(), "16-byte env slices and model blob in every step mode");  \
   const VariantOps* duck_variant_##NAME() {                                                     \
     static const VariantOps ops = {#NAME,               matches<MODEL>,         aux_size_of<MODEL>, \
                                    lds_bytes<MODEL>,    MODEL::FLOOR_TYPE,      launch_reset<MODEL>, \
diff --git a/open_duck_playground_amd/csrc/duck_physics.h b/open_duck_playground_amd/csrc/duck_physics.h
--- a/open_duck_playground_amd/csrc/duck_physics.h
+++ b/open_duck_playground_amd/csrc/duck_physics.h
@@ -6,6 +6,11 @@
 #define SCHED_FENCE() asm volatile("" ::: "memory")
 
 typedef __attribute__((address_space(3))) float lds_float;
+#define LDS_ALIGNED __attribute__((aligned(16)))
+DK lds_float* lds_assume16(lds_float* p) {
+  __builtin_assume(((unsigned)(__SIZE_TYPE__)p & 15u) == 0u);
+  return p;
+}
 
 #if defined(DUCK_STAGE_PROF) || defined(DUCK_WAVE_PROF) || defined(DUCK_LAT_PROF)
 #define DUCK_ANY_PROF 1
@@ -59,34 +64,86 @@
 
 constexpr int priv_row_max(int nu) { return DUCK_OBS_SIZE(nu) + 15 + 3 * nu + 1 + 2 + 6 + 2 + 40 + 1 + 2; }
 
-template <class Md>
-struct Lay {
+constexpr int LDS_WORDS = 160 * 1024 / 4;
+constexpr int SLICES_WG = 16;
+#ifdef DUCK_LS_DUMP
+constexpr int SINK_WORDS = 136;
+#else
+constexpr int SINK_WORDS = 32;
+#endif
+constexpr int slice_stride(int used) { return ((used + 15) / 32) * 32 + 16; }
+template <class Md>
+constexpr int hot_words() { return Md::NQ + 2 * Md::NV + 8 * Md::NU + 77; }
+constexpr int hot_stride(int hot) { return (hot + 64) | 1; }
+template <class Md>
+constexpr int lay_keeps(int total) {
+  const int tab = SLICES_WG * slice_stride(total + SINK_WORDS);
+  const int nht = Md::B_HEND > Md::B_HFACE ? Md::B_HEND - Md::B_HFACE : 0;
+  const bool tabl = tab + Md::NBLOB <= LDS_WORDS, htl = !tabl && nht > 0 && tab + nht <= LDS_WORDS;
+  const int es = tab + (tabl ? Md::NBLOB : (htl ? nht : 0));
+  const bool esl = es + SLICES_WG * hot_stride(hot_words<Md>()) <= LDS_WORDS;
+  return es > LDS_WORDS ? -1 : tabl + 2 * htl + 4 * esl;
+}
+
+#ifndef DUCK_LAY_WIDE
+#define DUCK_LAY_WIDE 1
+#endif
+template <class Md, int AL, bool WIDE>
+struct LayT {
+  static constexpr int ALIGN = AL, WIDE_RECORDS = WIDE;
   static constexpr int NB = Md::NB, NV = Md::NV, NQ = Md::NQ, NU = Md::NU;
   static constexpr int NCON = 4 * Md::NPAIR;
   static constexpr int R_LIM = Md::NFRIC, R_CON = Md::NFRIC + Md::NLIM;
   static constexpr int NROW = R_CON + 4 * NCON;
-  static constexpr int QPOS = 0, QVEL = QPOS + NQ, WARM = QVEL + NV, CTRL = WARM + NV, QACC = CTRL + NU;
-  static constexpr int QSM = QACC + NV, FSM = QSM + NV, SRCH = FSM + NV, GRAD = SRCH + NV, MA = GRAD + NV;
-  static constexpr int DMASS = MA + NV, DIPOS = DMASS + NB, DARM = DIPOS + 3, DFRIC = DARM + NV;
-  static constexpr int DQ0 = DFRIC + NV, DKP = DQ0 + NQ;
-  static constexpr int XPOS = DKP + NU, XQ = XPOS + 3 * NB, XMAT = XQ + 4 * NB, CIN = XMAT + 9 * NB;
-  static constexpr int CVEL = CIN + 10 * NB, COM = CVEL + 6 * NB;
-  static constexpr int CDOF = COM + 3, CDD1 = CDOF + 6 * NV;
-  static constexpr int M = CDD1 + 18, MZERO = M + Md::NM, H = MZERO + 1;
+  static constexpr int up(int x, int a) { return (x + a - 1) / a * a; }
+  static constexpr int a4(int x) { return up(x, AL < 4 ? AL : 4); }
+  static constexpr int a2(int x) { return up(x, AL < 2 ? AL : 2); }
+  static constexpr int arow(int x) { return a4(x + R_CON) - R_CON; }
+  static constexpr int XPS = WIDE ? 4 : 3, XMS = WIDE ? 10 : 9, CRS = WIDE ? 4 : 3, CFS = WIDE ? 10 : 9;
+  static constexpr int XQ = 0, XMAT = XQ + 4 * NB, XPOS = a4(XMAT + XMS * NB), CIN = a4(XPOS + XPS * NB);
+  static constexpr int CVEL = a4(CIN + 10 * NB), CDOF = a4(CVEL + 6 * NB);
+  static constexpr int M = a4(CDOF + 6 * NV), MZERO = M + Md::NM, CDD1 = a2(MZERO + 1);
+  static constexpr int COM = a4(CDD1 + 18), IMUR = COM + 3, OCON = IMUR + 3, FOOTZ = OCON + 2, FLAGS = FOOTZ + 2;
+  static constexpr int H = a4(FLAGS + 2);
   static constexpr int SCR_TREE = 12 * NB + 6 * NV, SCR_SAT = 6 * (Md::NHE + Md::NHF);
   static constexpr int SCR_HF = Md::FLOOR_TYPE == 1 ? 3 + 28 * 16 : 0, SCR_OBS = priv_row_max(NU);
   static constexpr int cmax(int a, int b) { return a > b ? a : b; }
   static constexpr int SCR_NEED = cmax(cmax(SCR_TREE, SCR_SAT), cmax(SCR_HF, SCR_OBS));
   static constexpr int HSZ = ((cmax(SCR_NEED - 4 * NROW - Md::NLIM, 0) + 3) / 4) * 4;
-  static constexpr int JA = H + HSZ, JV = JA + NROW, RD = JV + NROW, AREF = RD + NROW;
-  static constexpr int LSGN = AREF + NROW;
-  static constexpr int CR = LSGN + Md::NLIM, CFR = CR + 3 * NCON, CDIST = CFR + 9 * NCON;
-  static constexpr int KL = CIN, KR = KL + 21, KLR = KR + 21, FL = KLR + 36, FR = FL + 6;
+  static constexpr int JA = arow(H + HSZ), JV = arow(JA + NROW), RD = arow(JV + NROW), AREF = arow(RD + NROW);
+  static constexpr int LSGN = a2(AREF + NROW);
+  static constexpr int CR = a4(LSGN + Md::NLIM), CFR = a4(CR + CRS * NCON), CDIST = a4(CFR + CFS * NCON);
+  static_assert(CR - H >= SCR_NEED, "H + rows must cover the scratch users");
+  static constexpr int KL = CIN, KR = a2(KL + 21), KLR = a2(KR + 21), FL = KLR + 36, FR = FL + 6;
   static_assert(FR + 6 <= CIN + 10 * NB, "Newton blocks must fit in CIN");
-  static constexpr int AF = CDIST + NCON, SENS = AF + NU, OCON = SENS + Md::NSENSORDATA, IMUR = OCON + 2,
-                       FOOTZ = IMUR + 3, FLAGS = FOOTZ + 2;
-  static constexpr int TOTAL = FLAGS + 2;
+  static constexpr int AF = a2(CDIST + NCON), SENS = a2(AF + NU);
+  static constexpr int QPOS = SENS + Md::NSENSORDATA, QVEL = QPOS + NQ, WARM = QVEL + NV, CTRL = WARM + NV;
+  static constexpr int QACC = CTRL + NU;
+  static constexpr int QSM = QACC + NV, FSM = QSM + NV, SRCH = FSM + NV, GRAD = SRCH + NV, MA = GRAD + NV;
+  static constexpr int DMASS = MA + NV, DIPOS = DMASS + NB, DARM = DIPOS + 3, DFRIC = DARM + NV;
+  static constexpr int DQ0 = DFRIC + NV, DKP = DQ0 + NQ;
+  static constexpr int TOTAL = a4(DKP + NU);
+  static_assert(AL < 4 || (XQ % 4 == 0 && XMAT % 4 == 0 && CIN % 4 == 0 && CVEL % 4 == 0 && CDOF % 4 == 0 && M % 4 == 0 &&
+                           COM % 4 == 0 && H % 4 == 0 && (JA + R_CON) % 4 == 0 && (JV + R_CON) % 4 == 0 &&
+                           (RD + R_CON) % 4 == 0 && (AREF + R_CON) % 4 == 0 && CR % 4 == 0 && CFR % 4 == 0 &&
+                           CDIST % 4 == 0 && TOTAL % 4 == 0),
+                "16-byte fields");
+  static_assert(AL < 2 || (XPOS % 2 == 0 && CDD1 % 2 == 0 && KR % 2 == 0 && KLR % 2 == 0 && FL % 2 == 0 && FR % 2 == 0 &&
+                           LSGN % 2 == 0 && AF % 2 == 0 && SENS % 2 == 0),
+                "8-byte fields");
 };
+template <class Md>
+constexpr int lay_rule() {
+  constexpr int keep = lay_keeps<Md>(LayT<Md, 1, false>::TOTAL);
+  if (DUCK_LAY_WIDE) {
+    if (lay_keeps<Md>(LayT<Md, 4, true>::TOTAL) == keep) return 8 + 4;
+    if (lay_keeps<Md>(LayT<Md, 2, true>::TOTAL) == keep) return 8 + 2;
+    if (lay_keeps<Md>(LayT<Md, 1, true>::TOTAL) == keep) return 8 + 1;
+  }
+  return lay_keeps<Md>(LayT<Md, 4, false>::TOTAL) == keep ? 4 : (lay_keeps<Md>(LayT<Md, 2, false>::TOTAL) == keep ? 2 : 1);
+}
+template <class Md>
+struct Lay : LayT<Md, lay_rule<Md>() & 7, (lay_rule<Md>() >> 3) != 0> {};
 
 DK void kbi(const float* solref, const float* solimp, float pos, float dt, float& k, float& b, float& imp) {
   const float timeconst = fmaxf(solref[0], 2.0f * dt);
@@ -240,10 +297,10 @@
     } else {
       float R[9], t[3];
 #pragma unroll
-      for (int k = 0; k < 9; k++) R[k] = L[Ly::XMAT + 9 * b + k];
+      for (int k = 0; k < 9; k++) R[k] = L[Ly::XMAT + Ly::XMS * b + k];
       mulmv3(t, R, Md::geom_pos[g]);
 #pragma unroll
-      for (int k = 0; k < 3; k++) gp[k] = L[Ly::XPOS + 3 * b + k] + t[k];
+      for (int k = 0; k < 3; k++) gp[k] = L[Ly::XPOS + Ly::XPS * b + k] + t[k];
       mulmm3(gR, R, Md::geom_mat[g]);
     }
   }
@@ -251,9 +308,9 @@
   static DK void store_contact(lds_float* L, int slot, float dist, const float* pos, const float* fr) {
     L[Ly::CDIST + slot] = dist;
 #pragma unroll
-    for (int a = 0; a < 3; a++) L[Ly::CR + 3 * slot + a] = pos[a] - L[Ly::COM + a];
-#pragma unroll
-    for (int a = 0; a < 9; a++) L[Ly::CFR + 9 * slot + a] = fr[a];
+    for (int a = 0; a < 3; a++) L[Ly::CR + Ly::CRS * slot + a] = pos[a] - L[Ly::COM + a];
+#pragma unroll
+    for (int a = 0; a < 9; a++) L[Ly::CFR + Ly::CFS * slot + a] = fr[a];
   }
 
   static DK void contact_vel(const float* Sp, const float* r, float* v) {
@@ -272,12 +329,12 @@
     for (int k = 0; k < Md::NSENSORDATA; k++) aux[(o++) * stride] = L[Ly::SENS + k];
     for (int s = 0; s < NCON; s++) aux[(o++) * stride] = L[Ly::CDIST + s];
     for (int s = 0; s < NCON; s++)
-      for (int a = 0; a < 3; a++) aux[(o++) * stride] = L[Ly::CR + 3 * s + a] + L[Ly::COM + a];
+      for (int a = 0; a < 3; a++) aux[(o++) * stride] = L[Ly::CR + Ly::CRS * s + a] + L[Ly::COM + a];
     for (int s = 0; s < NCON; s++)
-      for (int a = 0; a < 3; a++) aux[(o++) * stride] = L[Ly::CFR + 9 * s + a];
+      for (int a = 0; a < 3; a++) aux[(o++) * stride] = L[Ly::CFR + Ly::CFS * s + a];
     for (int k = 0; k < Md::NM; k++) aux[(o++) * stride] = L[Ly::M + k];
 #ifdef DUCK_AUX_LDS
-    for (int k = 0; k < Ly::TOTAL + 12 * Md::MAXCHAIN + 24; k++) aux[(o++) * stride] = L[k];
+    for (int k = 0; k < Ly::TOTAL + SINK_WORDS; k++) aux[(o++) * stride] = L[k];
 #endif
   }
 };
@@ -286,7 +343,7 @@
 constexpr int aux_size() {
   return 4 * Md::NV + Md::NU + Md::NSENSORDATA + 7 * Lay<Md>::NCON + Md::NM
 #ifdef DUCK_AUX_LDS
-         + Lay<Md>::TOTAL + 12 * Md::MAXCHAIN + 24
+         + Lay<Md>::TOTAL + SINK_WORDS
 #endif
       ;
 }
diff --git a/open_duck_playground_amd/csrc/duck_team.h b/open_duck_playground_amd/csrc/duck_team.h
--- a/open_duck_playground_amd/csrc/duck_team.h
+++ b/open_duck_playground_amd/csrc/duck_team.h
@@ -221,11 +221,8 @@
 struct TLay {
   using Ly = Lay<Md>;
   static constexpr int KC = Ly::TOTAL;
-#ifdef DUCK_LS_DUMP
-  static constexpr int USED0 = KC + 136;
-#else
-  static constexpr int USED0 = KC + 2 * TEAM;
-#endif
+  static constexpr int USED0 = KC + SINK_WORDS;
+  static_assert(SINK_WORDS >= 2 * TEAM && SLICES_WG == TEAM_WG, "duck_physics.h lay_keeps");
   static constexpr int HF_SLF = (1 + Md::HF_SILCAP + 3) & ~3;
   static constexpr int HF_SLSZ = HF_SLF + 4 * Md::HF_SILCAP;
   static constexpr int XRNE = LAT ? ((USED0 + 3) & ~3) : Ly::H;
@@ -235,16 +232,20 @@
   static constexpr int XSIL = LAT ? ((XDUM1 + 6 * Md::NB + 3) & ~3) : ((Ly::CIN + 3) & ~3);
   static constexpr int XDIR = LAT ? ((XSIL + (Md::FLOOR_TYPE == 1 ? 2 * HF_SLSZ : 0) + 3) & ~3) : 0;
   static constexpr int USED = LAT ? XDIR + Md::NV + 4 : USED0;
-  static constexpr int STRIDE = ((USED + 15) / 32) * 32 + 16;
+  static constexpr int STRIDE = slice_stride(USED);
   static constexpr int NWG = LAT == 2 ? 2 * LAT_WG : (LAT ? LAT_WG : TEAM_WG);
   static_assert(STRIDE >= USED && STRIDE % 32 == 16, "stride");
+  static_assert(STRIDE % 4 == 0 && (STRIDE * NWG) % 4 == 0, "16-byte slices");
+  static_assert(XRNE % (Ly::ALIGN < 4 ? Ly::ALIGN : 4) == 0 && (!LAT || (XRNE % 4 == 0 && XCIN % 4 == 0 && XDUM0 % 2 == 0 &&
+                XDUM1 % 2 == 0 && XSIL % 4 == 0 && XDIR % 4 == 0)), "16-byte scratch regions");
   static constexpr int SINK = KC;
   static constexpr int TMP = Ly::H;
-  static constexpr int KLOC = TMP;
-  static_assert(7 * Md::NB <= Ly::HSZ + 4 * Ly::NROW, "tree scratch must fit in H + rows");
+  static constexpr int KLOC = TMP, KLS = 8;
+  static_assert(KLS >= 7 && KLS * Md::NB <= Ly::HSZ + 4 * Ly::NROW, "tree scratch must fit in H + rows");
   static constexpr int TAB = STRIDE * NWG;
-  static constexpr int HOT = Md::NQ + 2 * Md::NV + 8 * Md::NU + 77;
-  static constexpr int ESTRIDE = (HOT + 64) | 1;
+  static constexpr int HOT = hot_words<Md>();
+  static constexpr int ESTRIDE = hot_stride(HOT);
+  static_assert(ESTRIDE % 2 == 1, "the staged hot state keeps its odd stride");
   static constexpr int ES_FLOATS = ESTRIDE * NWG;
   static constexpr int NEV_G = LAT ? 10 : 0;
   static constexpr int NEV = LAT == 2 ? 2 * NEV_G : NEV_G;
@@ -258,6 +259,7 @@
   static constexpr int LDS_FLOATS = EV + 4 * NEV;
   static constexpr bool FITS = (size_t)LDS_FLOATS * 4 <= 160 * 1024 && (LAT == 0 || (TAB_LDS && ES_LDS));
   static_assert(LAT || FITS, "LDS budget");
+  static_assert(LAT || lay_keeps<Md>(Ly::TOTAL) == TAB_LDS + 2 * HT_LDS + 4 * ES_LDS, "lay_keeps (duck_physics.h) and TLay agree");
   static_assert(6 * Md::NV <= 4 * Ly::NROW, "crb scratch must fit in the row storage");
   static_assert(LAT || 18 * Md::NB <= Ly::HSZ + 4 * Ly::NROW, "rne scratch must fit in H + rows");
   static_assert(LAT || Md::FLOOR_TYPE != 1 || XSIL + 2 * HF_SLSZ <= Ly::CIN + 10 * Md::NB,
@@ -331,7 +333,7 @@
   static constexpr int R_LIM = Ly::R_LIM, R_CON = Ly::R_CON;
   static DK int ti(int off) {
     if constexpr (TL::TAB_LDS) {
-      extern __shared__ float lds_dyn[];
+      extern __shared__ LDS_ALIGNED float lds_dyn[];
       return ((lds_int*)(lds_dyn + TL::TAB))[off];
     } else {
       return Md::t_blob()[off];
@@ -340,14 +342,14 @@
   static DK float tf(int off) { return __int_as_float(ti(off)); }
   static DK float th(int off) {
     if constexpr (!TL::TAB_LDS && TL::HT_LDS) {
-      extern __shared__ float lds_dyn[];
+      extern __shared__ LDS_ALIGNED float lds_dyn[];
       return ((lds_float*)(lds_dyn + TL::TAB))[off - Md::B_HFACE];
     } else {
       return tf(off);
     }
   }
   static DK f4v ht4(int off) {
-    extern __shared__ __attribute__((aligned(16))) float lds_dyn[];
+    extern __shared__ LDS_ALIGNED float lds_dyn[];
     static_assert(Md::FLOOR_TYPE != 1 || TL::TAB_LDS || TL::HT_LDS, "the hull SAT tables must be in LDS");
     return *(const lds_f4*)((lds_float*)lds_dyn + TL::TAB + (TL::TAB_LDS ? off : off - Md::B_HFACE));
   }
@@ -423,9 +425,9 @@
     q2m(R, q);
   }
   static DK void store_pose(LP L, int b, const float* p, const float* q, const float* R) {
-    for (int k = 0; k < 3; k++) L[Ly::XPOS + 3 * b + k] = p[k];
+    for (int k = 0; k < 3; k++) L[Ly::XPOS + Ly::XPS * b + k] = p[k];
     for (int k = 0; k < 4; k++) L[Ly::XQ + 4 * b + k] = q[k];
-    for (int k = 0; k < 9; k++) L[Ly::XMAT + 9 * b + k] = R[k];
+    for (int k = 0; k < 9; k++) L[Ly::XMAT + Ly::XMS * b + k] = R[k];
   }
 
   static DK void kinematics(LP L, int lane) {
@@ -446,8 +448,8 @@
           qmul(q, q, ql);
         }
       }
-      for (int k = 0; k < 4; k++) L[TL::KLOC + 7 * b + k] = q[k];
-      for (int k = 0; k < 3; k++) L[TL::KLOC + 7 * b + 4 + k] = tf(o + 4 + k);
+      for (int k = 0; k < 4; k++) L[TL::KLOC + TL::KLS * b + k] = q[k];
+      for (int k = 0; k < 3; k++) L[TL::KLOC + TL::KLS * b + 4 + k] = tf(o + 4 + k);
     });
     TSYNC();
     STAGE_MARK(24);
@@ -459,8 +461,8 @@
     if (lane == 0) store_pose(L, 1, p, q, R);
     auto compose = [&](int b) {
       float ql[4], pl[3], t[3], qn[4];
-      for (int k = 0; k < 4; k++) ql[k] = L[TL::KLOC + 7 * b + k];
-      for (int k = 0; k < 3; k++) pl[k] = L[TL::KLOC + 7 * b + 4 + k];
+      for (int k = 0; k < 4; k++) ql[k] = L[TL::KLOC + TL::KLS * b + k];
+      for (int k = 0; k < 3; k++) pl[k] = L[TL::KLOC + TL::KLS * b + 4 + k];
       mulmv3(t, R, pl);
       for (int k = 0; k < 3; k++) p[k] += t[k];
       qmul(qn, q, ql);
@@ -482,7 +484,7 @@
 #pragma unroll
       for (int d = 0; d < BL; d++) {
         const int bc = bb[d] >= 0 ? bb[d] : 1;
-        for (int k = 0; k < 7; k++) kl[d][k] = L[TL::KLOC + 7 * bc + k];
+        for (int k = 0; k < 7; k++) kl[d][k] = L[TL::KLOC + TL::KLS * bc + k];
       }
 #pragma unroll
       for (int d = 0; d < BL; d++) {
@@ -509,7 +511,7 @@
     if (mv) {
       const int ob = Md::B_BINERT + 17 * b;
       float R[9], t[3], ip[3], Ri[9], Bi[9];
-      for (int k = 0; k < 9; k++) R[k] = L[Ly::XMAT + 9 * b + k];
+      for (int k = 0; k < 9; k++) R[k] = L[Ly::XMAT + Ly::XMS * b + k];
       for (int k = 0; k < 3; k++) ip[k] = (b == 1) ? L[Ly::DIPOS + k] : tf(ob + k);
       for (int k = 0; k < 9; k++) Bi[k] = tf(ob + 3 + k);
       mulmv3(t, R, ip);
@@ -518,7 +520,7 @@
       for (int a = 0; a < 3; a++)
         for (int c = 0; c < 3; c++)
           rot[3 * a + c] = Ri[3 * a] * I[0] * Ri[3 * c] + Ri[3 * a + 1] * I[1] * Ri[3 * c + 1] + Ri[3 * a + 2] * I[2] * Ri[3 * c + 2];
-      for (int k = 0; k < 3; k++) xi[k] = L[Ly::XPOS + 3 * b + k] + t[k];
+      for (int k = 0; k < 3; k++) xi[k] = L[Ly::XPOS + Ly::XPS * b + k] + t[k];
       m = L[Ly::DMASS + b];
     }
     const float ms = tsum(m);
@@ -543,12 +545,12 @@
       const int oj = Md::B_JREC + 9 * j;
       const bool jh = Md::B_JAFF && j >= Md::B_JN0;
       const int b = jh ? j + Md::B_JBD : ti(oj), da = jh ? j + Md::B_JDD : ti(oj + 1);
-      const float off[3] = {com[0] - L[Ly::XPOS + 3 * b], com[1] - L[Ly::XPOS + 3 * b + 1], com[2] - L[Ly::XPOS + 3 * b + 2]};
+      const float off[3] = {com[0] - L[Ly::XPOS + Ly::XPS * b], com[1] - L[Ly::XPOS + Ly::XPS * b + 1], com[2] - L[Ly::XPOS + Ly::XPS * b + 2]};
       if (!jh && ti(oj + 3) == 0) {
         for (int k = 0; k < 3; k++)
           for (int q = 0; q < 6; q++) L[Ly::CDOF + 6 * (da + k) + q] = (q == 3 + k) ? 1.0f : 0.0f;
         for (int k = 0; k < 3; k++) {
-          const float ax[3] = {L[Ly::XMAT + 9 * b + k], L[Ly::XMAT + 9 * b + 3 + k], L[Ly::XMAT + 9 * b + 6 + k]};
+          const float ax[3] = {L[Ly::XMAT + Ly::XMS * b + k], L[Ly::XMAT + Ly::XMS * b + 3 + k], L[Ly::XMAT + Ly::XMS * b + 6 + k]};
           float t[3];
           cross3(t, ax, off);
           const int o = Ly::CDOF + 6 * (da + 3 + k);
@@ -557,7 +559,7 @@
       } else {
         float R[9], ax[3], t[3];
         const float ja[3] = {tf(oj + 4), tf(oj + 5), tf(oj + 6)};
-        for (int k = 0; k < 9; k++) R[k] = L[Ly::XMAT + 9 * b + k];
+        for (int k = 0; k < 9; k++) R[k] = L[Ly::XMAT + Ly::XMS * b + k];
         mulmv3(ax, R, ja);
         cross3(t, ax, off);
         const int o = Ly::CDOF + 6 * da;
@@ -1197,8 +1199,8 @@
         const float sg = (e & 1) ? -mu : mu;
         float u[3], r3[3], a[6];
         for (int q = 0; q < 3; q++) {
-          u[q] = L[Ly::CFR + 9 * slot + q] + sg * L[Ly::CFR + 9 * slot + 3 * t + q];
-          r3[q] = L[Ly::CR + 3 * slot + q];
+          u[q] = L[Ly::CFR + Ly::CFS * slot + q] + sg * L[Ly::CFR + Ly::CFS * slot + 3 * t + q];
+          r3[q] = L[Ly::CR + Ly::CRS * slot + q];
         }
         cross3(a, r3, u);
         a[3] = u[0]; a[4] = u[1]; a[5] = u[2];
@@ -1256,8 +1258,8 @@
         const float sg = (e & 1) ? -mu : mu;
         float u[3], r3[3], a[6];
         for (int q = 0; q < 3; q++) {
-          u[q] = L[Ly::CFR + 9 * slot + q] + sg * L[Ly::CFR + 9 * slot + 3 * t + q];
-          r3[q] = L[Ly::CR + 3 * slot + q];
+          u[q] = L[Ly::CFR + Ly::CFS * slot + q] + sg * L[Ly::CFR + Ly::CFS * slot + 3 * t + q];
+          r3[q] = L[Ly::CR + Ly::CRS * slot + q];
         }
         cross3(a, r3, u);
         a[3] = u[0]; a[4] = u[1]; a[5] = u[2];
@@ -1309,10 +1311,10 @@
   static DK void cgeom_frame(LP L, int gs, float* gp, float* gR) {
     const int o = Md::B_CGEOM + 16 * gs, b = ti(o);
     float R[9], t[3], gpos[3], gm[9];
-    for (int k = 0; k < 9; k++) { R[k] = L[Ly::XMAT + 9 * b + k]; gm[k] = tf(o + 4 + k); }
+    for (int k = 0; k < 9; k++) { R[k] = L[Ly::XMAT + Ly::XMS * b + k]; gm[k] = tf(o + 4 + k); }
     for (int k = 0; k < 3; k++) gpos[k] = tf(o + 1 + k);
     mulmv3(t, R, gpos);
-    for (int k = 0; k < 3; k++) gp[k] = L[Ly::XPOS + 3 * b + k] + t[k];
+    for (int k = 0; k < 3; k++) gp[k] = L[Ly::XPOS + Ly::XPS * b + k] + t[k];
     mulmm3(gR, R, gm);
   }
 
@@ -2590,14 +2592,14 @@
     const int o = Md::B_PAIR + PAIRW * p;
     const int s1 = ti(o), s2 = ti(o + 1);
     const float mu = tf(o + 2);
-    const float r[3] = {L[Ly::CR + 3 * slot], L[Ly::CR + 3 * slot + 1], L[Ly::CR + 3 * slot + 2]};
+    const float r[3] = {L[Ly::CR + Ly::CRS * slot], L[Ly::CR + Ly::CRS * slot + 1], L[Ly::CR + Ly::CRS * slot + 2]};
     float v[3] = {0.0f, 0.0f, 0.0f}, t[3];
     if (s2 != 0) { Ph::contact_vel(s2 == 1 ? SL : SR, r, t); v[0] += t[0]; v[1] += t[1]; v[2] += t[2]; }
     if (s1 != 0) { Ph::contact_vel(s1 == 1 ? SL : SR, r, t); v[0] -= t[0]; v[1] -= t[1]; v[2] -= t[2]; }
     float jr[3];
     for (int q = 0; q < 3; q++)
-      jr[q] = L[Ly::CFR + 9 * slot + 3 * q] * v[0] + L[Ly::CFR + 9 * slot + 3 * q + 1] * v[1] +
-              L[Ly::CFR + 9 * slot + 3 * q + 2] * v[2];
+      jr[q] = L[Ly::CFR + Ly::CFS * slot + 3 * q] * v[0] + L[Ly::CFR + Ly::CFS * slot + 3 * q + 1] * v[1] +
+              L[Ly::CFR + Ly::CFS * slot + 3 * q + 2] * v[2];
     out4[0] = jr[0] + mu * jr[1];
     out4[1] = jr[0] - mu * jr[1];
     out4[2] = jr[0] + mu * jr[2];
@@ -3071,9 +3073,9 @@
       const int typ = ti(os), site = ti(os + 1), adr = ti(os + 2), b = ti(os + 3);
       float R[9], sp[3], sR[9], t[3], SM[9];
       const float spos[3] = {tf(os + 4), tf(os + 5), tf(os + 6)};
-      for (int k = 0; k < 9; k++) { R[k] = L[Ly::XMAT + 9 * b + k]; SM[k] = tf(os + 7 + k); }
+      for (int k = 0; k < 9; k++) { R[k] = L[Ly::XMAT + Ly::XMS * b + k]; SM[k] = tf(os + 7 + k); }
       mulmv3(t, R, spos);
-      for (int k = 0; k < 3; k++) sp[k] = L[Ly::XPOS + 3 * b + k] + t[k];
+      for (int k = 0; k < 3; k++) sp[k] = L[Ly::XPOS + Ly::XPS * b + k] + t[k];
       mulmm3(sR, R, SM);
       const float off[3] = {sp[0] - com[0], sp[1] - com[1], sp[2] - com[2]};
       float ang[3] = {L[Ly::CVEL + 6 * b], L[Ly::CVEL + 6 * b + 1], L[Ly::CVEL + 6 * b + 2]}, lin[3];
@@ -3217,12 +3219,12 @@
          EV_TIMEOUT = 9 };
   static_assert(EV_TIMEOUT < TL::NEV_G || !LAT, "event slots");
   static DK lds_int* ev_ptr(int k) {
-    extern __shared__ float lds_dyn[];
+    extern __shared__ LDS_ALIGNED float lds_dyn[];
     const int g = LAT == 2 ? __builtin_amdgcn_readfirstlane((int)threadIdx.x >> 7) : 0;
     return (lds_int*)(lds_dyn + TL::EV) + 4 * (k + TL::NEV_G * g);
   }
   static DK void ev_init(int tid) {
-    extern __shared__ float lds_dyn[];
+    extern __shared__ LDS_ALIGNED float lds_dyn[];
     if (tid < TL::NEV) ((lds_int*)(lds_dyn + TL::EV))[4 * tid] = 0;
   }
   static DK void ev_signal(int k, int v) {
@@ -3246,7 +3248,7 @@
     }
   }
   static DK bool ev_timed_out(int g) {
-    extern __shared__ float lds_dyn[];
+    extern __shared__ LDS_ALIGNED float lds_dyn[];
     return ((lds_int*)(lds_dyn + TL::EV))[4 * (EV_TIMEOUT + TL::NEV_G * g)] != 0;
   }
   static DK void lat_r0(LP L, int lane, int s) {
```

Measured after the change: 21.16 million env-steps/s (median of 6 runs). 1.02x the previous value.
